# ruubhagat/HP-Assignment-2

Hardware: AMD Instinct MI355X
Metric: simulated coherence transactions/sec (whole node) + % HBM roofline, 1/2/4/8 GPU (higher is better)
Workload: dtype u8

## Files before the change

### hp-assignment-2_amd/csrc/dsm_args.h

```cpp
#ifndef DSM_ARGS_H
#define DSM_ARGS_H

#include <hip/hip_runtime.h>
#include <stdint.h>

#include "dsm.h"

struct SimArgs {
    const uint16_t *traces;
    const uint32_t *counts;
    uint32_t stride;
    uint32_t n_instr;
    uint64_t n_sys;
    const unsigned int *d_n;
    const uint32_t *list;
    uint64_t first_sys;
    uint64_t seed;
    int dist;
    dsm_sys_result *results;
    uint4 *recs;
    unsigned long long *counters;
    unsigned int *claim;
    uint32_t *ovf_list;
    unsigned int *ovf_count;
    const uint2 *table;
    uint64_t sched_seed;
    uint32_t sched_thresh;
    uint32_t issue_cap;
    uint32_t *issue;
    uint32_t *issue_n;
    uint32_t rsh;
    uint32_t budget;
    uint32_t resume;
    uint32_t ffsel;
    const uint32_t *scan;
    uint32_t late_rsh;
    uint32_t *susp;
    uint32_t *susp_list;
    unsigned int *susp_count;
    uint32_t *susp_order;
    unsigned int *susp_multi;
    unsigned int *susp_long;
    unsigned int *susp_short;
    uint32_t susp_cap;
    uint32_t lim_rsh;
    uint32_t icap;
    uint32_t susp_ring;
    uint32_t *spill;
    uint32_t thr_ff;
    uint32_t lone;
    uint32_t lone_min;
    uint32_t serfmt;
    uint32_t split;
};
struct SimArgsPack { SimArgs a[3]; };

enum { K_MSGS = 13, K_INSTRS = 14, K_ROUNDS = 15, K_SYSTEMS = 16, K_STATUS = 17, K_DHASH = 22,
       K_FHASH = 23, K_MAXR = 24, K_OVFRERUN = 25, K_WROUNDS = 26, K_RESUMED = 27,
       K_FFPASS = 28, K_FFITER = 29, K_SCANI = 30, K_SCANR = 31, K_N = 32,
       K_SERMAC = 32 ,
       K_SERIT = 33  ,
       K_SERPROBE = 34  };
static_assert(sizeof(dsm_counters) == DSM_NCOUNTERS * 8 && K_SERMAC < DSM_NCOUNTERS, "dsm_counters slots");

#define CTRL_WORDS 2048
#define CTRL_FAST 0
#define CTRL_FB 256
#define CTRL_OVF 512
#define CTRL_RES 1024
#define CTRL_SUSP 1536
#define CTRL_SUSPL 1568
#define CTRL_SUSPS 1600
#define CTRL_SUSPM 1632
#define CTRL_SCAN 1792

#endif
```

### hp-assignment-2_amd/csrc/dsm_internal.h

```cpp
#ifndef DSM_INTERNAL_H
#define DSM_INTERNAL_H

#include <hip/hip_runtime.h>

#include "dsm.h"
#include "dsm_plan.h"
#include "dsm_args.h"

#define DSM_TIMING_RING 64

struct dsm_ctx {
    int device;
    dsm_config cfg;
    int ring;
    hipStream_t stream;
    int cus;
    unsigned int *d_ctrl;
    SimArgs *d_args;
    uint32_t *d_ovf_list;
    size_t ovf_cap;
    uint32_t *d_susp;
    size_t susp_cap;
    uint32_t *d_susp_list;
    size_t susp_list_cap;
    uint32_t *d_susp_order;
    size_t susp_order_cap;
    uint32_t *d_spill;
    size_t spill_cap;
    uint16_t *d_traces;
    size_t traces_cap;
    uint32_t *d_counts;
    size_t counts_cap;
    dsm_sys_result *d_res;
    size_t res_cap;
    dsm_counters *d_cnt;
    uint2 *d_table;
    uint4 *d_recs;
    size_t recs_cap;
    uint64_t recs_n;
    hipEvent_t tev0[DSM_TIMING_RING], tev1[DSM_TIMING_RING];
    uint64_t runs_timed;
    dsmp::Plan plan;
    hipStream_t last_st;
    int last_verdict;
    uint32_t budget_log2, late_log2, round_limit_log2, inbox_limit;
    uint32_t ff_budget_rounds;
    int ff_mode;
    int serial;
    uint32_t lone_rounds;
    uint32_t lone_min;
    int fmt_tile, parse_bpl;
    uint64_t sched_seed;
    uint32_t sched_thresh;
    uint32_t *d_issue;
    size_t issue_cap_total;
    uint32_t *d_issue_n;
    size_t issue_n_cap;
    uint64_t issue_sys;
    uint4 *d_dump_tpl;
    char *d_text_tmp;
    uint32_t *d_len_tmp;
    char *d_parse_buf;
    size_t parse_cap;
    uint64_t *d_parse_off;
    size_t parse_off_cap;
    uint32_t *d_parse_list;
    size_t parse_list_cap;
    uint32_t *d_ev_scratch;
    size_t ev_scratch_cap;
    unsigned char *d_rb_scratch;
    size_t rb_scratch_cap;
    unsigned long long *d_rb_claim;
    uint64_t rb_in_flight;
};

#define HIPCK(x) do { if ((x) != hipSuccess) return DSM_E_DEVICE; } while (0)

extern "C" int dsm_debug_order_state(dsm_ctx *c, uint32_t *counts, uint32_t *list, uint32_t *order,
                                     uint64_t cap, uint64_t sys, uint32_t *rec, uint32_t rec_cap,
                                     uint32_t *rec_words, int *host_long);

extern "C" int dsm_debug_reach_times(double *ms, uint64_t *chunks);

extern "C" int dsm_debug_dist_edges(int np, const uint16_t *trace, const uint32_t *counts, uint32_t stride,
                                    const dsm_reach_opts *opts, uint32_t *src, uint32_t *dst, uint8_t *pk, uint64_t cap,
                                    uint64_t *n);
extern "C" int dsm_debug_dist_edges_device(dsm_ctx *c, const uint16_t *d_trace, const uint32_t *d_counts,
                                           const dsm_reach_opts *opts, uint32_t *src, uint32_t *dst, uint8_t *pk,
                                           uint64_t cap, uint64_t *n, void *stream);
extern "C" int dsm_debug_dist_times(double *ms);
extern "C" int dsm_debug_fate_times(double *ms, uint64_t *sweeps);

extern "C" int dsm_debug_raudit_times(double *ms, uint64_t *bytes);
extern "C" int dsm_debug_raudit_lane(int np, const uint32_t *state, uint32_t cls, uint32_t *word, uint32_t *set);

extern "C" int dsm_debug_reach_batch_state(dsm_ctx *c, uint64_t *in_flight, uint64_t *scratch_bytes);

extern "C" int dsm_debug_exscan_device(dsm_ctx *c, const uint32_t *d_in, uint64_t n, uint64_t *d_out, void *stream);

void dsm_text_release(dsm_ctx *c);
void dsm_events_release(dsm_ctx *c);
void dsm_reach_batch_release(dsm_ctx *c);

#define DSM_LOCAL __attribute__((visibility("hidden")))
typedef void (*sim_fn)(const SimArgs *);
DSM_LOCAL sim_fn dsm_sim_pick(int np, int ring, bool gen, int mode);
DSM_LOCAL sim_fn dsm_sim_pick_rerun(int np, bool gen, int mode);
DSM_LOCAL int dsm_sim_blocks_per_cu(sim_fn f, int threads);
DSM_LOCAL void dsm_sim_launch(sim_fn f, unsigned grid, unsigned threads, hipStream_t st, const SimArgs *a);
DSM_LOCAL int dsm_sim_lds_bytes(int ring, int waves);
DSM_LOCAL void dsm_order_launch(int np, unsigned blocks, hipStream_t st, const SimArgs *a);
DSM_LOCAL void dsm_ser_launch(int np, bool cap, unsigned blocks, hipStream_t st, const SimArgs *a);
DSM_LOCAL void dsm_args_launch(const SimArgsPack &pk, SimArgs *dst, hipStream_t st);
DSM_LOCAL void dsm_scan_launch(int np, unsigned blocks, hipStream_t st, const uint16_t *traces,
                               const uint32_t *counts, uint32_t stride, uint64_t n_sys, uint32_t *scan,
                               unsigned long long *counters);
DSM_LOCAL void dsm_digest_launch(int np, unsigned blocks, hipStream_t st, uint64_t n_sys, const uint4 *recs,
                                 dsm_sys_result *results, unsigned long long *counters);
#define DSM_EXSCAN_TILE 2048
DSM_LOCAL void dsm_exscan_launch(const uint32_t *in, unsigned long long n, unsigned long long *bsum,
                                 unsigned long long *out, hipStream_t st);

static inline int dsm_recs_range(const dsm_ctx *c, uint32_t need, uint64_t first_sys, uint64_t n_sys) {
    if ((c->cfg.flags & need) != need || !c->d_recs) return DSM_E_STATE;
    if (first_sys > c->recs_n || n_sys > c->recs_n - first_sys) return DSM_E_INVAL;
    return DSM_OK;
}

template <typename T>
static inline int dsm_ensure(T **p, size_t *cap, size_t need) {
    if (*cap >= need && *p) return DSM_OK;
    if (*p) { (void)hipFree(*p); *p = nullptr; *cap = 0; }
    if (hipMalloc((void **)p, need * sizeof(T)) != hipSuccess) { *p = nullptr; return DSM_E_NOMEM; }
    *cap = need;
    return DSM_OK;
}

#endif
```

### hp-assignment-2_amd/csrc/dsm_knobs.h

```cpp
#ifndef DSM_KNOBS_H
#define DSM_KNOBS_H

#ifndef TRAFFIC_PROBE
#define TRAFFIC_PROBE 0
#endif
#ifndef REC_PROBE
#define REC_PROBE 0
#endif
#ifndef SIM_TAILPROBE
#define SIM_TAILPROBE 0
#endif
#ifndef SER_PROBE
#define SER_PROBE 0
#endif

#ifndef FF_LONG_U
#define FF_LONG_U 8
#endif

#ifndef SER_HB
#define SER_HB 8
#endif
#ifndef SER_HT
#define SER_HT 32
#endif
#ifndef SER_SOLO_MIN
#define SER_SOLO_MIN 48
#endif
#ifndef SER_SOLO_HW
#define SER_SOLO_HW 2
#endif
#ifndef SER_DEAD_FWD
#define SER_DEAD_FWD 1
#endif
#ifndef SER_NOTICE_HOME
#define SER_NOTICE_HOME 1
#endif
#ifndef SER_DUMP
#define SER_DUMP 0
#endif

#endif
```

### hp-assignment-2_amd/csrc/dsm_runtime.hip

```cpp
#include <hip/hip_runtime.h>

#include <stdint.h>
#include <stdio.h>
#include <stdlib.h>
#include <string.h>

#include "dsm.h"
#include "dsm_knobs.h"
#include "dsm_table.h"
#include "dsm_internal.h"
#include "dsm_serial.h"

using namespace dsmp;


static uint32_t env_u32(const char *name, uint32_t dflt) {
    const char *e = getenv(name);
    if (!e || !*e) return dflt;
    const long v = strtol(e, nullptr, 10);
    return v < 0 ? 0u : (uint32_t)v;
}

extern "C" int dsm_device_count(int *count) {
    if (!count) return DSM_E_INVAL;
    int c = 0;
    if (hipGetDeviceCount(&c) != hipSuccess) c = 0;
    *count = c;
    return DSM_OK;
}

extern "C" int dsm_open(int device, const dsm_config *cfg, dsm_ctx **out) {
    if (!cfg || !out) return DSM_E_INVAL;
    *out = nullptr;
    if (cfg->np != 4 && cfg->np != 8) return DSM_E_INVAL;
    if (cfg->max_instr == 0 || cfg->max_instr > DSM_MAX_INSTR || (cfg->max_instr & 7u)) return DSM_E_INVAL;
    int ring = cfg->ring_cap ? (int)cfg->ring_cap : 12;
    if (ring != 4 && ring != 8 && ring != 12 && ring != 16) return DSM_E_INVAL;
    int ndev = 0;
    if (hipGetDeviceCount(&ndev) != hipSuccess || device < 0 || device >= ndev) return DSM_E_DEVICE;
    hipDeviceProp_t prop;
    if (hipGetDeviceProperties(&prop, device) != hipSuccess) return DSM_E_DEVICE;
    if (strncmp(prop.gcnArchName, "gfx950", 6) != 0) return DSM_E_DEVICE;
    if (hipSetDevice(device) != hipSuccess) return DSM_E_DEVICE;
    dsm_ctx *c = (dsm_ctx *)calloc(1, sizeof(dsm_ctx));
    if (!c) return DSM_E_NOMEM;
    c->device = device;
    c->cfg = *cfg;
    c->sched_thresh = DSM_SCHED_LOCKSTEP;
    c->ring = ring;
    c->cus = prop.multiProcessorCount;
    c->budget_log2 = env_u32("DSM_BUDGET_LOG2", 12);
    if (c->budget_log2 >= RSH_MAX) c->budget_log2 = 0;
    uint32_t ffb_log2 = env_u32("DSM_FF_BUDGET_LOG2", 0);
    if (ffb_log2 >= RSH_MAX) ffb_log2 = 0;
    c->ff_budget_rounds = getenv("DSM_FF_BUDGET_LOG2") ? (ffb_log2 ? 1u << ffb_log2 : 0u)
                                                       : env_u32("DSM_FF_BUDGET_ROUNDS", 448);
    if (c->ff_budget_rounds >= (1u << RSH_MAX)) c->ff_budget_rounds = 0;
    c->late_log2 = env_u32("DSM_LATE_LOG2", 0);
    c->round_limit_log2 = RSH_MAX;
    c->inbox_limit = FB_RING;
    c->ff_mode = DSM_FF_AUTO;
    c->serial = (int)env_u32("DSM_SERIAL", 1);
    c->lone_rounds = env_u32("DSM_LONE", 8);
    c->lone_min = env_u32("DSM_LONE_MIN", 160);

    c->fmt_tile = (int)env_u32("DSM_FMT", 132);
    c->parse_bpl = (int)env_u32("DSM_PARSE_BPL", 32);
    if (hipStreamCreateWithFlags(&c->stream, hipStreamNonBlocking) != hipSuccess ||
        hipMalloc((void **)&c->d_ctrl, CTRL_WORDS * sizeof(unsigned int)) != hipSuccess ||
        hipMalloc((void **)&c->d_args, sizeof(SimArgsPack)) != hipSuccess ||
        hipMalloc((void **)&c->d_cnt, sizeof(dsm_counters)) != hipSuccess ||
        hipMalloc((void **)&c->d_table, DT_TABLE_WORDS * sizeof(uint32_t)) != hipSuccess) {
        dsm_close(c);
        return DSM_E_DEVICE;
    }
    {
        static uint32_t tab[DT_TABLE_WORDS];
        if (dt_build(tab) > DT_ENTRIES || hipMemcpy(c->d_table, tab, sizeof tab, hipMemcpyHostToDevice) != hipSuccess) {
            dsm_close(c);
            return DSM_E_DEVICE;
        }
    }
    if (cfg->flags & DSM_F_TIMING) {
        for (int i = 0; i < DSM_TIMING_RING; ++i)
            if (hipEventCreate(&c->tev0[i]) != hipSuccess || hipEventCreate(&c->tev1[i]) != hipSuccess) {
                dsm_close(c);
                return DSM_E_DEVICE;
            }
    }
    *out = c;
    return DSM_OK;
}

extern "C" void dsm_close(dsm_ctx *c) {
    if (!c) return;
    (void)hipSetDevice(c->device);
    if (c->stream) (void)hipStreamSynchronize(c->stream);
    void *ptrs[] = {c->d_ctrl, c->d_args, c->d_ovf_list, c->d_susp, c->d_susp_list, c->d_susp_order, c->d_spill,
                    c->d_traces, c->d_counts,
                    c->d_res, c->d_cnt, c->d_recs, c->d_table, c->d_issue, c->d_issue_n};
    for (void *p : ptrs) if (p) (void)hipFree(p);
    dsm_text_release(c);
    dsm_events_release(c);
    dsm_reach_batch_release(c);
    for (int i = 0; i < DSM_TIMING_RING; ++i) {
        if (c->tev0[i]) (void)hipEventDestroy(c->tev0[i]);
        if (c->tev1[i]) (void)hipEventDestroy(c->tev1[i]);
    }
    if (c->stream) (void)hipStreamDestroy(c->stream);
    free(c);
}

extern "C" int dsm_launch_info_get(dsm_ctx *c, dsm_launch_info *info) {
    if (!c || !info) return DSM_E_INVAL;
    if (c->plan.pair && c->last_verdict < 0) {
        uint32_t scan[2] = {0, 0};
        HIPCK(hipSetDevice(c->device));
        HIPCK(hipStreamSynchronize(c->last_st));
        HIPCK(hipMemcpy(scan, c->d_ctrl + CTRL_SCAN, sizeof scan, hipMemcpyDeviceToHost));
        c->last_verdict = ff_verdict(scan) ? 1 : 0;
    }
    *info = plan_info(c->plan, c->last_verdict > 0);
    info->lds_bytes_per_block = c->plan.n_launch ? dsm_sim_lds_bytes(c->plan.ring_eff, SIM_WAVES) : 0;
    info->fmt_tile = c->fmt_tile;
    info->parse_bpl = c->parse_bpl;
    return DSM_OK;
}

static const char *build_variant() {
    static char tag[160];
    if (tag[0]) return tag[1] ? tag + 1 : "";
    int n = snprintf(tag, sizeof tag, "#");
    auto add = [&](const char *name, long v, long def) {
        if (v != def && n < (int)sizeof tag) n += snprintf(tag + n, sizeof tag - n, " %s=%ld", name, v);
    };
    add("REC_PROBE", REC_PROBE, 0);
    add("SIM_TAILPROBE", SIM_TAILPROBE, 0);
    add("TRAFFIC_PROBE", TRAFFIC_PROBE, 0);
    add("SER_PROBE", SER_PROBE, 0);
    add("SER_HB", SER_HB, 8);
    add("SER_HT", SER_HT, 32);
    add("SER_SOLO_MIN", SER_SOLO_MIN, 48);
    add("SER_SOLO_HW", SER_SOLO_HW, 2);
    add("FF_LONG_U", FF_LONG_U, 8);
    add("SER_DEAD_FWD", SER_DEAD_FWD, 1);
    add("SER_NOTICE_HOME", SER_NOTICE_HOME, 1);
    add("SER_DUMP", SER_DUMP, 0);
    return tag[1] ? tag + 1 : "";
}

extern "C" int dsm_launch_kernel_names(const dsm_launch_info *info, char *buf, size_t cap) {
    if (!info || !buf) return DSM_E_INVAL;
    char b[2][96];
    auto sim = [&](char *o, int m) {
        snprintf(o, 96, "sim_kernel<%d, %d, %d, %s, %d, %d>", info->np, info->ring_cap,
                 info->block_threads / 64, info->gen ? "true" : "false", m, info->occ);
    };
    int n;
    if (info->budget_mode < 0) {
        n = snprintf(buf, cap, "none");
    } else if (info->resume_form == DSM_RESUME_NONE) {
        sim(b[0], info->budget_mode);
        n = snprintf(buf, cap, "run=%s", b[0]);
    } else {
        sim(b[0], info->budget_mode);
        if (info->resume_mode >= 0) sim(b[1], info->resume_mode);
        else snprintf(b[1], 96, "ser_kernel<%d, %s>", info->np, info->ser_cap ? "true" : "false");
        n = snprintf(buf, cap, "budget=%s resume=%s", b[0], b[1]);
    }
    const char *v = build_variant();
    if (n >= 0 && *v && (size_t)n < cap) n += snprintf(buf + n, cap - n, " [variant:%s]", v);
    return (n < 0 || (size_t)n >= cap) ? DSM_E_INVAL : n;
}

extern "C" int dsm_set_budget(dsm_ctx *c, uint32_t budget_log2, uint32_t late_log2) {
    if (!c || budget_log2 >= RSH_MAX || late_log2 >= RSH_MAX) return DSM_E_INVAL;
    c->budget_log2 = budget_log2;
    c->late_log2 = late_log2;
    return DSM_OK;
}

extern "C" int dsm_set_round_limit(dsm_ctx *c, uint32_t limit_log2) {
    if (!c || limit_log2 > RSH_MAX) return DSM_E_INVAL;
    c->round_limit_log2 = limit_log2 ? limit_log2 : RSH_MAX;
    if (c->round_limit_log2 < 1) return DSM_E_INVAL;
    return DSM_OK;
}

extern "C" int dsm_set_fast_forward(dsm_ctx *c, int mode) {
    if (!c || mode < DSM_FF_OFF || mode > DSM_FF_AUTO) return DSM_E_INVAL;
    c->ff_mode = mode;
    return DSM_OK;
}

extern "C" int dsm_set_inbox_limit(dsm_ctx *c, uint32_t cap) {
    if (!c || cap > (uint32_t)FB_RING) return DSM_E_INVAL;
    c->inbox_limit = cap ? cap : (uint32_t)FB_RING;
    return DSM_OK;
}

namespace {
struct HostRec {
    const uint32_t *p;
    uint32_t ld(uint32_t w) const { return p[w]; }
};
}
extern "C" int dsm_debug_order_state(dsm_ctx *c, uint32_t *counts, uint32_t *list, uint32_t *order,
                                     uint64_t cap, uint64_t sys, uint32_t *rec, uint32_t rec_cap,
                                     uint32_t *rec_words, int *host_long) {
    if (!c || !counts) return DSM_E_INVAL;
    HIPCK(hipSetDevice(c->device));
    HIPCK(hipStreamSynchronize(c->last_st ? c->last_st : c->stream));
    const Plan &pl = c->plan;
    const uint64_t n = pl.in.n_sys;
    counts[0] = counts[1] = counts[2] = counts[3] = 0;
    if (!n || !pl.blog) return 0;
    HIPCK(hipMemcpy(&counts[0], c->d_ctrl + CTRL_SUSP, sizeof(uint32_t), hipMemcpyDeviceToHost));
    HIPCK(hipMemcpy(&counts[1], c->d_ctrl + CTRL_SUSPL, sizeof(uint32_t), hipMemcpyDeviceToHost));
    HIPCK(hipMemcpy(&counts[2], c->d_ctrl + CTRL_SUSPS, sizeof(uint32_t), hipMemcpyDeviceToHost));
    HIPCK(hipMemcpy(&counts[3], c->d_ctrl + CTRL_SUSPM, sizeof(uint32_t), hipMemcpyDeviceToHost));
    counts[1] += counts[3];
    if ((list && cap < n) || (order && cap < 2 * n)) return DSM_E_INVAL;
    if (list) HIPCK(hipMemcpy(list, c->d_susp_list, n * sizeof(uint32_t), hipMemcpyDeviceToHost));
    if (order && pl.order)
        HIPCK(hipMemcpy(order, c->d_susp_order, pl.order_words * sizeof(uint32_t), hipMemcpyDeviceToHost));
    if (rec_words) *rec_words = pl.rec_words;
    if (rec && pl.rec_words) {
        if (sys >= n || rec_cap < pl.rec_words) return DSM_E_INVAL;
        HIPCK(hipMemcpy(rec, c->d_susp + sys * (uint64_t)pl.rec_words,
                        pl.rec_words * sizeof(uint32_t), hipMemcpyDeviceToHost));
        if (host_long) {
            const HostRec m{rec};
            *host_long = (c->cfg.np == 4 ? dsms::ser_long_class<4>(m, rec[121])
                                         : dsms::ser_long_class<8>(m, rec[121])) ? 1 : 0;
        }
    }
    return pl.order ? 1 : 0;
}

static void put_sched(SimArgs &a, const PlanArgs &s) {
    a.rsh = s.rsh; a.budget = s.budget; a.resume = s.resume; a.ffsel = s.ffsel;
    a.late_rsh = s.late_rsh; a.thr_ff = s.thr_ff; a.lone = s.lone; a.lone_min = s.lone_min;
    a.serfmt = s.serfmt; a.split = s.split; a.susp_ring = s.susp_ring; a.lim_rsh = s.lim_rsh;
    a.icap = s.icap;
}

static int run_engine(dsm_ctx *c, bool gen, const dsm_gen *g, uint64_t first_sys,
                      const uint16_t *d_traces, const uint32_t *d_counts, uint64_t n_sys,
                      dsm_sys_result *d_results, dsm_counters *d_counters, hipStream_t st) {
    if (n_sys > 0xFFFFFFFFull) return DSM_E_INVAL;
    const int np = c->cfg.np;
    const bool tr = (c->cfg.flags & DSM_F_ISSUE_TRACE) != 0;
    PlanIn in{};
    in.np = np; in.ring = c->ring; in.gen = gen; in.n_sys = n_sys; in.cus = c->cus;
    in.tc = (c->cfg.flags & DSM_F_TYPE_COUNTS) != 0; in.tr = tr; in.sx = c->sched_thresh < DSM_SCHED_LOCKSTEP;
    in.round_limit_log2 = c->round_limit_log2; in.inbox_limit = c->inbox_limit;
    in.ff_mode = c->ff_mode; in.serial = c->serial; in.ff_budget_rounds = c->ff_budget_rounds;
    in.budget_log2 = c->budget_log2; in.late_log2 = c->late_log2;
    in.lone_rounds = c->lone_rounds; in.lone_min = c->lone_min;
    in.traffic_probe = TRAFFIC_PROBE;
    Plan p = plan_build(in);
    if (n_sys == 0) {
        c->plan = p;
        return DSM_OK;
    }
    HIPCK(hipSetDevice(c->device));
    sim_fn sim[PLAN_MAX_LAUNCHES] = {}, fast = nullptr;
    for (int i = 0; i < p.n_launch; ++i) {
        if (p.launch[i].kernel != PK_SIM) continue;
        if (!(sim[i] = dsm_sim_pick(np, p.ring_eff, gen, p.launch[i].mode))) return DSM_E_INVAL;
        if (!fast) fast = sim[i];
    }
    const sim_fn fb = dsm_sim_pick_rerun(np, gen, p.mode);
    const int nb_fast = dsm_sim_blocks_per_cu(fast, 64 * SIM_WAVES), nb_fb = dsm_sim_blocks_per_cu(fb, 64);
    if (nb_fast < 1 || nb_fb < 1) return DSM_E_DEVICE;
    plan_grids(p, nb_fast, nb_fb);

    int rc;
    if ((rc = dsm_ensure(&c->d_ovf_list, &c->ovf_cap, (size_t)n_sys))) return rc;
    if (p.blog) {
        if ((rc = dsm_ensure(&c->d_susp, &c->susp_cap, (size_t)n_sys * p.susp_words))) return rc;
        if ((rc = dsm_ensure(&c->d_susp_list, &c->susp_list_cap, (size_t)n_sys))) return rc;
    }
    if (p.order && (rc = dsm_ensure(&c->d_susp_order, &c->susp_order_cap, (size_t)p.order_words))) return rc;
    if ((rc = dsm_ensure(&c->d_recs, &c->recs_cap, (size_t)n_sys * np * 8))) return rc;
    if (p.use_ser && (rc = dsm_ensure(&c->d_spill, &c->spill_cap, (size_t)p.spill_lanes * dsms::S_SPILL))) return rc;
    if (!d_results) {
        if ((rc = dsm_ensure(&c->d_res, &c->res_cap, (size_t)n_sys + 1))) return rc;
        d_results = c->d_res;
    }
    if (tr) {
        const size_t cap = (size_t)np * c->cfg.max_instr;
        if ((rc = dsm_ensure(&c->d_issue, &c->issue_cap_total, (size_t)n_sys * cap))) return rc;
        if ((rc = dsm_ensure(&c->d_issue_n, &c->issue_n_cap, (size_t)n_sys))) return rc;
    }
    if (c->cfg.flags & DSM_F_SNAPSHOTS)
        HIPCK(hipMemsetAsync(c->d_recs, 0, (size_t)n_sys * np * 128, st));
    c->recs_n = n_sys;
    HIPCK(hipMemsetAsync(c->d_ctrl, 0, CTRL_WORDS * sizeof(unsigned int), st));

    SimArgsPack pk;
    memset(&pk, 0, sizeof pk);
    SimArgs &A = pk.a[ARGS_FAST];
    A.traces = d_traces;
    A.counts = d_counts;
    A.stride = c->cfg.max_instr;
    A.n_instr = gen ? g->n_instr : 0;
    A.n_sys = n_sys;
    A.first_sys = first_sys;
    A.seed = gen ? g->seed : 0;
    A.dist = gen ? g->dist : 0;
    A.results = d_results;
    A.recs = c->d_recs;
    A.counters = reinterpret_cast<unsigned long long *>(d_counters);
    A.claim = c->d_ctrl + CTRL_FAST;
    A.ovf_list = c->d_ovf_list;
    A.ovf_count = c->d_ctrl + CTRL_OVF;
    A.table = c->d_table;
    A.sched_seed = c->sched_seed;
    A.sched_thresh = c->sched_thresh;
    A.susp = c->d_susp;
    A.susp_list = c->d_susp_list;
    A.susp_count = c->d_ctrl + CTRL_SUSP;
    A.susp_order = p.order ? c->d_susp_order : nullptr;
    A.susp_multi = c->d_ctrl + CTRL_SUSPM;
    A.susp_long = c->d_ctrl + CTRL_SUSPL;
    A.susp_short = c->d_ctrl + CTRL_SUSPS;
    A.susp_cap = (uint32_t)n_sys;
    A.spill = c->d_spill;
    if (tr) {
        A.issue = c->d_issue;
        A.issue_n = c->d_issue_n;
        A.issue_cap = (uint32_t)((size_t)np * c->cfg.max_instr);
        c->issue_sys = n_sys;
    }
    SimArgs &B = pk.a[ARGS_RERUN];
    B = A;
    B.d_n = c->d_ctrl + CTRL_OVF;
    B.list = c->d_ovf_list;
    B.claim = c->d_ctrl + CTRL_FB;
    B.ovf_list = nullptr;
    B.ovf_count = nullptr;
    SimArgs &C = pk.a[ARGS_RESUME];
    C = A;
    C.n_sys = 0;
    C.d_n = c->d_ctrl + CTRL_SUSP;
    C.list = c->d_susp_list;
    C.claim = c->d_ctrl + CTRL_RES;
    A.scan = C.scan = c->d_ctrl + CTRL_SCAN;
    for (int i = 0; i < 3; ++i) put_sched(pk.a[i], p.args[i]);
    dsm_args_launch(pk, c->d_args, st);
    HIPCK(hipGetLastError());

    const bool timed = (c->cfg.flags & DSM_F_TIMING) != 0;
    const int slot = (int)(c->runs_timed % DSM_TIMING_RING);
    if (timed) HIPCK(hipEventRecord(c->tev0[slot], st));
    unsigned long long *dcnt = reinterpret_cast<unsigned long long *>(d_counters);
    for (int i = 0; i < p.n_launch; ++i) {
        const PlanLaunch &L = p.launch[i];
        const SimArgs *a = (const SimArgs *)(c->d_args + L.args);
        switch (L.kernel) {
        case PK_SCAN:
            dsm_scan_launch(np, p.scan_blocks, st, d_traces, d_counts, (uint32_t)c->cfg.max_instr, n_sys,
                            c->d_ctrl + CTRL_SCAN, dcnt);
            break;
        case PK_SIM:
            dsm_sim_launch(sim[i], p.grid_fast, 64 * SIM_WAVES, st, a);
            break;
        case PK_ORDER:
            dsm_order_launch(np, p.order_blocks, st, a);
            break;
        case PK_SER:
            dsm_ser_launch(np, L.mode != 0, p.ser_blocks, st, a);
            break;
        case PK_RERUN:
            if (timed) {
                HIPCK(hipEventRecord(c->tev1[slot], st));
                c->runs_timed++;
            }
            dsm_sim_launch(fb, p.grid_fb, 64, st, a);
            break;
        case PK_DIGEST:
            if (REC_PROBE) break;
            dsm_digest_launch(np, p.digest_blocks, st, n_sys, (const uint4 *)c->d_recs, d_results, dcnt);
            break;
        }
        HIPCK(hipGetLastError());
    }
    c->plan = p;
    c->last_st = st;
    c->last_verdict = -1;
    return DSM_OK;
}


static int validate_host_traces(const dsm_ctx *c, const uint16_t *traces, const uint32_t *counts,
                                 uint64_t n_sys) {
    const int np = c->cfg.np;
    const uint32_t stride = c->cfg.max_instr;
    for (uint64_t s = 0; s < n_sys; ++s)
        for (int nd = 0; nd < np; ++nd) {
            const uint32_t cnt = counts[s * np + nd];
            if (cnt > stride) return DSM_E_INVAL;
            const uint16_t *t = traces + (s * np + nd) * (uint64_t)stride;
            for (uint32_t i = 0; i < cnt; ++i)
                if ((uint32_t)((t[i] >> 12) & 7u) >= (uint32_t)np) return DSM_E_RANGE;
        }
    return DSM_OK;
}

extern "C" int dsm_run_packed_device(dsm_ctx *c, const uint16_t *d_traces, const uint32_t *d_counts,
                                     uint64_t n_sys, dsm_sys_result *d_results,
                                     dsm_counters *d_counters, void *stream) {
    if (!c || (n_sys && (!d_traces || !d_counts)) || !d_counters) return DSM_E_INVAL;
    return run_engine(c, false, nullptr, 0, d_traces, d_counts, n_sys, d_results, d_counters,
                      (hipStream_t)stream);
}

extern "C" int dsm_run_generated_device(dsm_ctx *c, const dsm_gen *g, uint64_t first_sys,
                                        uint64_t n_sys, dsm_sys_result *d_results,
                                        dsm_counters *d_counters, void *stream) {
    if (!c || !g || !d_counters) return DSM_E_INVAL;
    if (g->n_instr > DSM_MAX_INSTR || g->dist < 0 || g->dist > 2) return DSM_E_INVAL;
    return run_engine(c, true, g, first_sys, nullptr, nullptr, n_sys, d_results, d_counters,
                      (hipStream_t)stream);
}

static int finish_host(dsm_ctx *c, uint64_t n_sys, dsm_sys_result *per_sys, dsm_counters *out) {
    if (per_sys && n_sys)
        HIPCK(hipMemcpyAsync(per_sys, c->d_res, n_sys * sizeof(dsm_sys_result), hipMemcpyDeviceToHost, c->stream));
    if (out) HIPCK(hipMemcpyAsync(out, c->d_cnt, sizeof(dsm_counters), hipMemcpyDeviceToHost, c->stream));
    HIPCK(hipStreamSynchronize(c->stream));
    return DSM_OK;
}

extern "C" int dsm_run_packed(dsm_ctx *c, const uint16_t *traces, const uint32_t *counts,
                              uint64_t n_sys, dsm_sys_result *per_sys, dsm_counters *out) {
    if (!c || (n_sys && (!traces || !counts))) return DSM_E_INVAL;
    int rc = validate_host_traces(c, traces, counts, n_sys);
    if (rc) return rc;
    HIPCK(hipSetDevice(c->device));
    const size_t slots = (size_t)n_sys * c->cfg.np;
    if ((rc = dsm_ensure(&c->d_traces, &c->traces_cap, slots * c->cfg.max_instr + 8))) return rc;
    if ((rc = dsm_ensure(&c->d_counts, &c->counts_cap, slots + 1))) return rc;
    if ((rc = dsm_ensure(&c->d_res, &c->res_cap, (size_t)n_sys + 1))) return rc;
    if (n_sys) {
        HIPCK(hipMemcpyAsync(c->d_traces, traces, slots * c->cfg.max_instr * sizeof(uint16_t), hipMemcpyHostToDevice, c->stream));
        HIPCK(hipMemcpyAsync(c->d_counts, counts, slots * sizeof(uint32_t), hipMemcpyHostToDevice, c->stream));
    }
    HIPCK(hipMemsetAsync(c->d_cnt, 0, sizeof(dsm_counters), c->stream));
    if ((rc = run_engine(c, false, nullptr, 0, c->d_traces, c->d_counts, n_sys, c->d_res, c->d_cnt, c->stream))) return rc;
    return finish_host(c, n_sys, per_sys, out);
}

extern "C" int dsm_run_generated(dsm_ctx *c, const dsm_gen *g, uint64_t first_sys, uint64_t n_sys,
                                 dsm_sys_result *per_sys, dsm_counters *out) {
    if (!c || !g) return DSM_E_INVAL;
    int rc;
    HIPCK(hipSetDevice(c->device));
    if ((rc = dsm_ensure(&c->d_res, &c->res_cap, (size_t)n_sys + 1))) return rc;
    HIPCK(hipMemsetAsync(c->d_cnt, 0, sizeof(dsm_counters), c->stream));
    if ((rc = dsm_run_generated_device(c, g, first_sys, n_sys, c->d_res, c->d_cnt, c->stream))) return rc;
    return finish_host(c, n_sys, per_sys, out);
}

extern "C" int dsm_kernel_ms_history(dsm_ctx *c, float *ms, uint32_t cap, uint32_t *n) {
    if (!c || !n || (cap && !ms)) return DSM_E_INVAL;
    if (!(c->cfg.flags & DSM_F_TIMING)) return DSM_E_STATE;
    HIPCK(hipSetDevice(c->device));
    uint64_t k = c->runs_timed < DSM_TIMING_RING ? c->runs_timed : DSM_TIMING_RING;
    if (k > cap) k = cap;
    for (uint64_t i = 0; i < k; ++i) {
        const int slot = (int)((c->runs_timed - k + i) % DSM_TIMING_RING);
        HIPCK(hipEventSynchronize(c->tev1[slot]));
        HIPCK(hipEventElapsedTime(&ms[i], c->tev0[slot], c->tev1[slot]));
    }
    *n = (uint32_t)k;
    return DSM_OK;
}

extern "C" int dsm_last_kernel_ms(dsm_ctx *c, float *ms) {
    if (!c || !ms) return DSM_E_INVAL;
    if (!(c->cfg.flags & DSM_F_TIMING) || c->runs_timed == 0) return DSM_E_STATE;
    uint32_t n = 0;
    return dsm_kernel_ms_history(c, ms, 1, &n);
}

extern "C" int dsm_get_node_state(dsm_ctx *c, uint64_t sys, int node, dsm_node_state *dump,
                                  dsm_node_state *final_state) {
    if (!c || node < 0 || node >= c->cfg.np) return DSM_E_INVAL;
    if (int rc = dsm_recs_range(c, DSM_F_SNAPSHOTS, sys, 1)) return rc;
    HIPCK(hipSetDevice(c->device));
    HIPCK(hipStreamSynchronize(c->stream));
    HIPCK(hipDeviceSynchronize());
    const size_t i = ((size_t)sys * c->cfg.np + node) * 8;
    if (dump) HIPCK(hipMemcpy(dump, c->d_recs + i, sizeof *dump, hipMemcpyDeviceToHost));
    if (final_state) HIPCK(hipMemcpy(final_state, c->d_recs + i + 4, sizeof *final_state, hipMemcpyDeviceToHost));
    return DSM_OK;
}

extern "C" int dsm_set_schedule(dsm_ctx *c, uint64_t seed, uint32_t act_thresh) {
    if (!c) return DSM_E_INVAL;
    c->sched_seed = seed;
    c->sched_thresh = act_thresh >= DSM_SCHED_LOCKSTEP ? DSM_SCHED_LOCKSTEP : act_thresh;
    return DSM_OK;
}

extern "C" int dsm_get_issue_trace(dsm_ctx *c, uint64_t sys, uint32_t *events, uint32_t cap,
                                   uint32_t *n) {
    if (!c || !n || (cap && !events)) return DSM_E_INVAL;
    if (!(c->cfg.flags & DSM_F_ISSUE_TRACE) || !c->d_issue) return DSM_E_STATE;
    if (sys >= c->issue_sys) return DSM_E_INVAL;
    HIPCK(hipSetDevice(c->device));
    HIPCK(hipStreamSynchronize(c->stream));
    HIPCK(hipDeviceSynchronize());
    uint32_t k = 0;
    HIPCK(hipMemcpy(&k, c->d_issue_n + sys, sizeof k, hipMemcpyDeviceToHost));
    const uint32_t per = (uint32_t)(c->cfg.np * c->cfg.max_instr);
    const uint32_t m = k < cap ? k : cap;
    if (m) HIPCK(hipMemcpy(events, c->d_issue + sys * per, m * sizeof(uint32_t), hipMemcpyDeviceToHost));
    *n = k;
    return DSM_OK;
}
```

### hp-assignment-2_amd/csrc/dsm_ser.hip

```cpp
#include <hip/hip_runtime.h>

#include <stdint.h>

#include "dsm.h"
#include "dsm_knobs.h"
#include "dsm_table.h"
#include "dsm_internal.h"
#include "dsm_device.h"
#include "dsm_serial.h"

namespace {

using namespace dsmp;

constexpr int SER_RF = 8;
constexpr int SER_MACRO = 1;
template <int W>
struct LdsCol {
    uint32_t (&s)[W][dsms::S_WORDS][64];
    uint32_t *dum;
    uint32_t wv, lane;
    GU32 *sp;
    DEVI uint32_t ld(uint32_t w) const { return s[wv][w][lane]; }
    DEVI void st(uint32_t w, uint32_t v) const { s[wv][w][lane] = v; }
    DEVI void st_if(bool en, uint32_t w, uint32_t v) const { *(en ? &s[wv][w][lane] : dum) = v; }
    DEVI uint32_t ld8(uint32_t w, uint32_t b) const {
        return reinterpret_cast<const uint8_t *>(&s[wv][w][lane])[b];
    }
    DEVI void st8(uint32_t w, uint32_t b, uint32_t v) const {
        reinterpret_cast<uint8_t *>(&s[wv][w][lane])[b] = (uint8_t)v;
    }
    DEVI uint32_t ld16(uint32_t w, uint32_t h) const {
        return reinterpret_cast<const uint16_t *>(&s[wv][w][lane])[h];
    }
    DEVI void st16(uint32_t w, uint32_t h, uint32_t v) const {
        reinterpret_cast<uint16_t *>(&s[wv][w][lane])[h] = (uint16_t)v;
    }
    DEVI uint32_t sp_ld(uint32_t i) const { return sp[i]; }
    DEVI void sp_st(uint32_t i, uint32_t v) const { sp[i] = v; }
};
struct LdsTab {
    const uint2 (&t)[DT_TABLE_WORDS / 2];
    DEVI uint32_t hdr(uint32_t i) const { return reinterpret_cast<const uint32_t *>(&t[DT_ENTRIES])[i]; }
    DEVI void row(uint32_t i, uint32_t &w0, uint32_t &w1) const {
        const uint2 e = t[i];
        w0 = e.x;
        w1 = e.y;
    }
};

template <int NP, bool CAP>
__global__ void __launch_bounds__(64 * SER_WAVES) __attribute__((amdgpu_waves_per_eu(2)))
ser_kernel(const SimArgs *Ap) {
    using namespace dsms;
    constexpr uint32_t NPM = (1u << NP) - 1u;
    constexpr bool SOLO = !CAP;
    if (DSM_SER_EXITS(Ap)) return;

    __shared__ uint32_t s_ser[SER_WAVES][S_WORDS][64];
    __shared__ uint2 s_tab[DT_TABLE_WORDS / 2];
    __shared__ unsigned long long s_cnt[K_N];
    __shared__ uint32_t s_dum[64];
    const uint32_t lane = threadIdx.x & 63u, wv = threadIdx.x >> 6;
    if (threadIdx.x < K_N) s_cnt[threadIdx.x] = 0;
    for (uint32_t i = threadIdx.x; i < DT_TABLE_WORDS / 2; i += 64 * SER_WAVES) s_tab[i] = Ap->table[i];
    __syncthreads();
#if SIM_TAILPROBE
    const uint64_t tprobe0 = __builtin_amdgcn_s_memrealtime();
#endif

    const LdsCol<SER_WAVES> m{s_ser, &s_dum[lane], wv, lane,
                              (GU32 *)(Ap->spill + ((uint64_t)blockIdx.x * (64 * SER_WAVES) + threadIdx.x) * S_SPILL)};
    const LdsTab T{s_tab};
    const bool ordered = Ap->serfmt != 0u && Ap->susp_order != nullptr;
    const uint32_t nmulti = ordered ? *Ap->susp_multi : 0u;
    const uint32_t nlong = nmulti + (ordered ? *Ap->susp_long : 0u);
    const uint32_t n = uni32(*Ap->d_n);
    const uint32_t lcap = Ap->susp_cap;
    const uint32_t *const list = ordered ? Ap->susp_order : Ap->list;
    auto sel = [&](uint32_t k) -> uint32_t {
        return ((const GU32 *)list)[k < nmulti ? lcap + k : k < nlong ? lcap - 1u - (k - nmulti) : n - 1u - k];
    };

    const uint32_t stride = Ap->stride, lim_rsh = Ap->lim_rsh, SR = Ap->susp_ring;
    const uint32_t cap = Ap->icap;
    const uint16_t *const traces = Ap->traces;

    uint4 *const recs = Ap->recs;
    dsm_sys_result *const results = Ap->results;
    const uint32_t *const susp = Ap->susp;
    uint32_t *const ovf_list = Ap->ovf_list;
    unsigned int *const ovf_count = Ap->ovf_count, *const claim_ctr = Ap->claim;

    SReg r;
    SCache cc;
    ser_cache_clear(cc);
    uint64_t sys = 0;
    uint32_t tn = 0xFFu, tci = 0, pfc = 0;
    bool nxv = false, pfv = false;
    uint4 cur = make_uint4(0, 0, 0, 0), nx = cur, pf = cur;
    auto slot_of = [&](uint32_t nd) { return traces + (sys * NP + nd) * (uint64_t)stride; };

    auto claim_next = [&]() -> uint32_t {
        return gatomic_add((GU32 *)claim_ctr, 1u);
    };


    auto start_ls = [&]() {
        const GU32 *sp = (const GU32 *)(susp + sys * ((uint64_t)susp_words((int)SR) * NP));
        r.rounds = sp[(12u + SR + 6u) * NP];
        for (uint32_t nd = 0; nd < (uint32_t)NP; ++nd) {
            const GU32 *b = sp + nd;
#pragma unroll
            for (uint32_t i = 0; i < 8; ++i) m.st(S_MB + 8u * nd + i, b[i * NP]);
            uint32_t la = 0, lv = 0, ls = 0;
#pragma unroll
            for (uint32_t i = 0; i < 4; ++i) {
                const uint32_t l = b[(8u + i) * NP];
                la |= (l & 0xFFu) << (8 * i);
                lv |= ((l >> 8) & 0xFFu) << (8 * i);
                ls |= ((l >> 16) & 3u) << (2 * i);
            }
            m.st(S_LA + nd, la);
            m.st(S_LV + nd, lv);
            const GU32 *q = b + (12u + SR) * NP;
            const uint32_t ctl = q[NP], ip = q[2 * NP], rh = q[4 * NP];
            m.st(S_DS + nd, q[0]);
            m.st(S_CT + nd, (ctl & 0x3FFu) | (ls << SC_LS) | (ip << SC_IP));
            s_set_ni(r, nd, q[3 * NP]);
            const uint32_t h = rh & 0xFFu, c = rh >> 8;
            for (uint32_t j = 0; j < c; ++j) {
                uint32_t sl = h + j;
                sl = sl >= SR ? sl - SR : sl;
                ser_enqueue<S_QN>(m, r, nd, b[(12u + sl) * NP]);
            }
            s_byte_add(r.cnt0, r.cnt1, nd, c);
            r.nz |= (c ? 1u : 0u) << nd;
            r.msgs += q[5 * NP] - c;
            r.iss |= ((ctl & (C_WAIT | C_DUMPED)) == 0u ? 1u : 0u) << nd;
            r.dmp |= ((ctl & C_DUMPED) ? 1u : 0u) << nd;
        }
    };
    const bool serfmt = Ap->serfmt != 0u;
    v4u32 rr[33];
    auto load_rec = [&](uint64_t s_) {
        const GV4 *sv = (const GV4 *)(susp + s_ * (uint64_t)ssusp_words((int)SR));
#pragma unroll
        for (uint32_t i = 0; i < 33; ++i) rr[i] = sv[i];
    };
    auto start = [&]() -> uint32_t {
        ser_clear(r);
        tn = 0xFFu;
        nxv = pfv = false;
        if (!serfmt) {
            start_ls();
        } else {
        const GU32 *sp = (const GU32 *)(susp + sys * (uint64_t)ssusp_words((int)SR));
#pragma unroll
        for (uint32_t i = 0; i < 24; ++i) {
            const uint32_t w = 4u * i;
            m.st(w, rr[i].x); m.st(w + 1u, rr[i].y); m.st(w + 2u, rr[i].z); m.st(w + 3u, rr[i].w);
        }
        const v4u32 *const hd = rr + 24;
        r.rounds = hd[6].x;
        auto hw = [&](uint32_t k) -> uint32_t {
            const v4u32 &v = hd[k >> 2];
            return (k & 3u) == 0u ? v.x : (k & 3u) == 1u ? v.y : (k & 3u) == 2u ? v.z : v.w;
        };
#pragma unroll
        for (uint32_t nd = 0; nd < (uint32_t)NP; ++nd) {
            const uint32_t rh = hw(nd), c = rh >> 8, ctl = m.ld(S_CT + nd);
            s_set_ni(r, nd, hw(8u + nd));
            for (uint32_t j = 0; j < c; ++j)
                ser_enqueue<S_QN>(m, r, nd, sp[SSUSP_HDR + nd * SR + j]);
            s_byte_add(r.cnt0, r.cnt1, nd, c);
            r.nz |= (c ? 1u : 0u) << nd;
            r.msgs += hw(16u + nd) - c;
            r.iss |= ((ctl & (SC_WAIT | SC_DUMPED)) == 0u ? 1u : 0u) << nd;
            r.dmp |= ((ctl & SC_DUMPED) ? 1u : 0u) << nd;
        }
        if (hd[6].y & 0x100u) {
            tn = hd[6].y & 0xFFu;
            const uint32_t ip0 = m.ld(S_CT + tn) >> SC_IP, j0 = ip0 & 7u;
            const uint32_t rw[4] = {hd[7].x, hd[7].y, hd[7].z, hd[7].w};
            uint32_t al[4] = {0u, 0u, 0u, 0u};
#pragma unroll
            for (uint32_t k = 0; k < 8u; ++k) {
                uint32_t hv = 0u;
#pragma unroll
                for (uint32_t q = 0; q < 8u; ++q)
                    hv = (k >= j0 && k - j0 == q) ? ((rw[q >> 1] >> (16u * (q & 1u))) & 0xFFFFu) : hv;
                al[k >> 1] |= hv << (16u * (k & 1u));
            }
            cur = make_uint4(al[0], al[1], al[2], al[3]);
            nx = make_uint4(hd[8].x, hd[8].y, hd[8].z, hd[8].w);
            tci = ip0 >> 3;
            nxv = true;
            pfc = tci + 2u;
            pfv = pfc * 8u < stride;
            if (pfv) pf = ld16(slot_of(tn) + pfc * 8u);
        }
        }
        r.E = r.nz;
        r.A = r.nz | r.iss;
        ser_cache_clear(cc);
        if (SOLO && serfmt && tn != 0xFFu) {
            cc.ct = m.ld(S_CT + tn); cc.la = m.ld(S_LA + tn); cc.lv = m.ld(S_LV + tn);
            cc.node = tn;
        }
        if (r.A == 0u) {
            r.st = (r.dmp == NPM) ? SS_COMPLETED : SS_DEADLOCKED;
            return SR_DONE;
        }
        return SR_RUN;
    };
    auto store_rec = [&](uint32_t nd, uint32_t flags, uint32_t which) {
        if (REC_PROBE) return;
        GV4 *dst = (GV4 *)(recs + (sys * NP + nd) * 8 + 4u * which);
#pragma unroll
        for (int q = 0; q < 4; ++q) {
            v4u32 x;
            x.x = ser_rec_word(m, nd, flags, 4 * q);
            x.y = ser_rec_word(m, nd, flags, 4 * q + 1);
            x.z = ser_rec_word(m, nd, flags, 4 * q + 2);
            x.w = ser_rec_word(m, nd, flags, 4 * q + 3);
            dst[q] = x;
        }
    };
    auto fetch = [&](uint32_t nd, uint32_t ip, bool iss) -> uint32_t {
        const uint32_t c = ip >> 3;
        const bool tnd = tn == nd;
        const bool rot = iss & tnd & (tci + 1u == c) & nxv;
        const bool miss = iss & !rot & (!tnd | (tci != c));
        cur.x = rot ? nx.x : cur.x; cur.y = rot ? nx.y : cur.y;
        cur.z = rot ? nx.z : cur.z; cur.w = rot ? nx.w : cur.w;
        nxv = nxv & !rot;
        tci = rot ? c : tci;
        if (__ballot(miss)) {
            if (SER_PROBE && lane == 0) atomicAdd(&s_cnt[3], 1ull);
            if (miss) {
                const uint16_t *sl = slot_of(nd);
                cur = ld16(sl + 8u * c);
                nxv = (c + 1u) * 8u < stride;
                nx = ld16(sl + (nxv ? 8u * (c + 1u) : 8u * c));
                pfv = false;
                tn = nd;
                tci = c;
            }
            wait_vmcnt0();
        }
        const uint32_t j = ip & 7u;
        const uint32_t m2 = 0u - ((j >> 1) & 1u), m4 = 0u - ((j >> 2) & 1u);
        const uint32_t lo = (cur.x & ~m2) | (cur.y & m2), hi = (cur.z & ~m2) | (cur.w & m2);
        const uint32_t wd = (lo & ~m4) | (hi & m4);
        return (wd >> (16u * (j & 1u))) & 0xFFFFu;
    };
    auto fetch_reg = [&](uint32_t nd, uint32_t ip, uint32_t &ins) -> bool {
        const uint32_t c = ip >> 3;
        const bool tnd = tn == nd;
        const bool rot = tnd & (tci + 1u == c) & nxv;
        const bool have = tnd & ((tci == c) | rot);
        cur.x = rot ? nx.x : cur.x; cur.y = rot ? nx.y : cur.y;
        cur.z = rot ? nx.z : cur.z; cur.w = rot ? nx.w : cur.w;
        nxv = nxv & !rot;
        tci = rot ? c : tci;
        const uint32_t j = ip & 7u;
        const uint32_t m2 = 0u - ((j >> 1) & 1u), m4 = 0u - ((j >> 2) & 1u);
        const uint32_t lo = (cur.x & ~m2) | (cur.y & m2), hi = (cur.z & ~m2) | (cur.w & m2);
        const uint32_t wd = (lo & ~m4) | (hi & m4);
        ins = (wd >> (16u * (j & 1u))) & 0xFFFFu;
        return have;
    };
    bool live = false;
    uint32_t v = SR_RUN;
    auto refill = [&]() {
        if (pfv && !nxv && pfc == tci + 1u) {
            nx = pf;
            nxv = true;
            pfv = false;
        }
        if (pfv && (pfc <= tci || pfc > tci + 2u)) pfv = false;
        const uint32_t want = nxv ? tci + 2u : tci + 1u;
        if (tn != 0xFFu && !pfv && want * 8u < stride && v == SR_RUN) {
            pf = ld16(slot_of(tn) + want * 8u);
            pfc = want;
            pfv = true;
        }
    };
    auto on_dump = [&](uint32_t nd) { store_rec(nd, 2u, 0u); };
    auto finish = [&](uint32_t v) {
        if (v == SR_OVF) {
            const uint32_t pos = gatomic_add((GU32 *)ovf_count, 1u);
            ((GU32 *)ovf_list)[pos] = (uint32_t)sys;
            atomicAdd(&s_cnt[K_OVFRERUN], 1ull);
            return;
        }
        uint32_t ins = 0;
#pragma unroll
        for (uint32_t nd = 0; nd < (uint32_t)NP; ++nd) {
            ins += m.ld(S_CT + nd) >> SC_IP;
            store_rec(nd, ser_final_flags(m, nd), 1u);
        }
        v4u32 res;
        res.x = r.st | (r.dmp << 8); res.y = r.rounds; res.z = r.msgs; res.w = ins;
        ((GV4 *)results)[2 * sys] = res;
        atomicAdd(&s_cnt[K_MSGS], (unsigned long long)r.msgs);
        atomicAdd(&s_cnt[K_INSTRS], (unsigned long long)ins);
        atomicAdd(&s_cnt[K_ROUNDS], (unsigned long long)r.rounds);
        atomicAdd(&s_cnt[K_SYSTEMS], 1ull);
        atomicAdd(&s_cnt[K_STATUS + r.st], 1ull);
        atomicMax(&s_cnt[K_MAXR], (unsigned long long)r.rounds);
    };

    {
        const uint32_t k = claim_next();
        live = k < n;
        if (live) sys = sel(k);
        if (live && serfmt) load_rec(sys);
    }
    v = live ? start() : SR_RUN;
    uint32_t iters = 0, nmac = 0;
    uint32_t tclaim = 0, now_it = 0;
    bool lone0 = false;
    [[maybe_unused]] uint64_t pr_long = 0, pr_last = 0, pr_n4k = 0, pr_nl_it = 0, pr_it = 0, pr_nl_n = 0;
    if constexpr (SIM_TAILPROBE == 2) lone0 = live && serfmt && (rr[30].y & 0x100u);
    uint32_t hwait = 0;
    uint64_t pb_runs = 0, pb_steps = 0, pb_idle = 0, pb_cyc = 0;
    for (;;) {
        bool taken = false, rest = false;
#pragma unroll 1
        for (int k = 0; k < SER_RF; ++k) {
            bool ran_now = false, gen = true;
            if (SOLO) {
                if (k == 0) {
                    uint64_t ts0 = 0;
                    if (SER_PROBE >= 2) ts0 = __builtin_amdgcn_s_memtime();
                    const bool run = live && v == SR_RUN;
                    const bool ql = run && ser_quiet_lone(r, lim_rsh);
                    const uint32_t sn = ql ? dsms::s_ctz(r.A) : 0xFEu;
                    const uint32_t c = cc.ct >> (SC_IP + 3u);
                    const bool hotq = ql & (cc.node == sn) & (tn == sn);
                    const bool rot = hotq & (tci + 1u == c) & nxv;
                    cur.x = rot ? nx.x : cur.x; cur.y = rot ? nx.y : cur.y;
                    cur.z = rot ? nx.z : cur.z; cur.w = rot ? nx.w : cur.w;
                    nxv = nxv & !rot;
                    tci = rot ? c : tci;
                    const bool elig = hotq & (tci == c);
                    const uint32_t ne = (uint32_t)__builtin_popcountll(__ballot(elig));
                    const uint32_t nr = (uint32_t)__builtin_popcountll(__ballot(run));
                    if (ne != 0u && ne * 64u >= nr * (uint32_t)SER_SOLO_MIN) {
                        uint32_t ns = 0;
                        if (elig) ns = ser_solo<NP>(m, r, cc, cur.x, cur.y, cur.z, cur.w, lim_rsh);
                        nmac += ns;
                        taken = ran_now = true;
                        rest = elig & (ns != 0u) & (((cc.ct >> SC_IP) & 7u) == 0u);
                        iters += 1u;
                        if (SER_PROBE) {
                            uint32_t t = ns;
                            for (int o = 1; o < 64; o <<= 1) t += __shfl_xor(t, o, 64);
                            pb_runs += 1u; pb_steps += t; pb_idle += 8u * nr - t;
                            if (SER_PROBE >= 2) pb_cyc += __builtin_amdgcn_s_memtime() - ts0;
                        }
                    }
                }
                if (taken) {
                    gen = __ballot(live && v == SR_RUN && !rest) != 0ull;
                    if (!gen && !ran_now) break;
                }
                iters += gen ? 1u : 0u;
            }
            bool mac = false;
            uint64_t tp0 = 0, tp1 = 0, tp2 = 0;
            if (SER_PROBE >= 2) tp0 = __builtin_amdgcn_s_memtime();
            if (!CAP && gen) {
#pragma unroll
                for (int j = 0; j < SER_MACRO; ++j) {
                    const bool q = live && v == SR_RUN && !rest && ser_quiet_lone(r, lim_rsh) && (j == 0 || mac);
                    bool did = false;
                    bool nohave = false;
                    if (SER_PROBE && q) {
                        const uint32_t n0 = dsms::s_ctz(r.A), ip0 = m.ld(S_CT + n0) >> SC_IP, c0 = ip0 >> 3;
                        nohave = !((tn == n0) & ((tci == c0) | ((tci + 1u == c0) & nxv)));
                    }
                    if (SER_PROBE >= 4) {
                        uint64_t ts[5] = {0, 0, 0, 0, 0};
                        auto stamp = [&](int i) { __builtin_amdgcn_s_waitcnt(0); ts[i + 1] = __builtin_amdgcn_s_memtime(); };
                        __builtin_amdgcn_s_waitcnt(0);
                        ts[0] = __builtin_amdgcn_s_memtime();
                        if (__ballot(q) && q) did = ser_macro<NP>(m, r, cc, fetch_reg, on_dump, stamp);
                        const uint64_t okb = __ballot(did);
                        if (okb && lane == (uint32_t)__builtin_ctzll(okb)) {
                            atomicAdd(&s_cnt[13], ts[1] - ts[0]);
                            atomicAdd(&s_cnt[14], ts[2] - ts[1]);
                            atomicAdd(&s_cnt[15], ts[3] - ts[2]);
                            atomicAdd(&s_cnt[16], ts[4] - ts[3]);
                        }
                    } else if (__ballot(q) && q) {
                        did = ser_macro<NP>(m, r, cc, fetch_reg, on_dump, [](int) {});
                    }
                    if (SER_PROBE && j == 0) {
                        const uint64_t nh = __ballot(nohave);
                        if (lane == 0) atomicAdd(&s_cnt[8 + 3], 0ull + __builtin_popcountll(nh));
                    }
                    if (SER_PROBE && j == 0) {
                        const bool nq_ = live && v == SR_RUN && !q;
                        const uint64_t nq = __ballot(nq_), qn = __ballot(q && !did);
                        const uint64_t mi = __ballot(nq_ && (r.iss & (r.iss - 1u)) != 0u);
                        if (lane == 0) {
                            atomicAdd(&s_cnt[9], (unsigned long long)__builtin_popcountll(nq));
                            atomicAdd(&s_cnt[10], (unsigned long long)__builtin_popcountll(qn));
                            (void)mi;
                        }
                    }
                    mac = mac || did;
                    nmac += did ? 1u : 0u;
                }
                if (mac && r.A == 0u) v = SR_DONE;
                if (SOLO) rest = rest | (taken & mac);
            }
            if (SER_PROBE) {
                const uint64_t gm = __ballot(live && v == SR_RUN && !mac), mm = __ballot(mac);
                const uint64_t lv = __ballot(live);
                if (lane == 0) {
                    atomicAdd(&s_cnt[8], (unsigned long long)__builtin_popcountll(lv));
                    if (__builtin_popcountll(lv) < 32) atomicAdd(&s_cnt[12], 1ull);
                    atomicAdd(&s_cnt[0], 1ull);
                    if (mm) atomicAdd(&s_cnt[1], 1ull);
                    if (gm) atomicAdd(&s_cnt[2], 1ull);
                }
            }
            if (SER_PROBE >= 2) tp1 = __builtin_amdgcn_s_memtime();
            if (live && v == SR_RUN && !mac && gen && !rest) {
                v = ser_step<NP, S_QN, CAP>(m, r, T, fetch, on_dump, lim_rsh, cap);
                ser_cache_clear(cc);
            }
            if (SER_PROBE >= 2) tp2 = __builtin_amdgcn_s_memtime();
            if (SER_PROBE) {
                const uint64_t hm = __ballot(live && v != SR_RUN);
                if (lane == 0 && hm) atomicAdd(&s_cnt[4], 1ull);
            }
            bool hgo = false;
            const uint64_t fin = __ballot(live && v != SR_RUN);
            if (fin) {
                hgo = (uint32_t)__builtin_popcountll(fin) >= (uint32_t)SER_HB ||
                      hwait >= (uint32_t)SER_HT || fin == __ballot(live);
                hwait = hgo ? 0u : hwait + (gen ? 1u : 0u) + (ran_now ? (uint32_t)SER_SOLO_HW : 0u);
            }
            if (hgo && live && v != SR_RUN) {
                if constexpr (SIM_TAILPROBE == 2) now_it = iters + (uint32_t)k;
                uint64_t th0 = 0, th1 = 0, th2 = 0;
                if (SER_PROBE >= 3) th0 = __builtin_amdgcn_s_memtime();
                wait_vmcnt0();
                const uint32_t k = claim_next();
                const bool nl = k < n;
                const uint32_t ns = nl ? sel(k) : 0u;
                if (nl && serfmt) load_rec(ns);
                if (SER_PROBE >= 3) { __builtin_amdgcn_s_waitcnt(0); th1 = __builtin_amdgcn_s_memtime(); }
                if constexpr (SIM_TAILPROBE == 2) {
                    const uint64_t dur = (uint64_t)(now_it - tclaim);
                    const uint64_t a = (dur << 32) | (uint64_t)sys;
                    const uint64_t b = ((uint64_t)now_it << 32) | ((uint64_t)lone0 << 31) | dur;
                    pr_long = a > pr_long ? a : pr_long;
                    pr_last = b > pr_last ? b : pr_last;
                    pr_n4k += dur > 4000u ? 1u : 0u;
                    pr_nl_it += lone0 ? 0u : dur;
                    pr_it += dur;
                    pr_nl_n += lone0 ? 0u : 1u;
                    tclaim = now_it;
                    lone0 = nl && serfmt && (rr[30].y & 0x100u);
                }
                finish(v);
                if (SER_PROBE >= 3) { __builtin_amdgcn_s_waitcnt(0); th2 = __builtin_amdgcn_s_memtime(); }
                live = nl;
                sys = ns;
                rest = false;
                v = live ? start() : SR_RUN;
                if (SER_PROBE >= 3) {
                    __builtin_amdgcn_s_waitcnt(0);
                    const uint64_t th3 = __builtin_amdgcn_s_memtime();
                    const uint64_t fl = __ballot(true);
                    if (lane == (uint32_t)__builtin_ctzll(fl)) {
                        atomicAdd(&s_cnt[13], th1 - th0);
                        atomicAdd(&s_cnt[14], th2 - th1);
                        atomicAdd(&s_cnt[15], th3 - th2);
                    }
                }
            }
            if (SER_PROBE >= 2 && lane == 0) {
                const uint64_t tp3 = __builtin_amdgcn_s_memtime();
                atomicAdd(&s_cnt[5], tp1 - tp0);
                atomicAdd(&s_cnt[6], tp2 - tp1);
                atomicAdd(&s_cnt[7], tp3 - tp2);
            }
            if (!gen) break;
        }
        uint64_t tr0 = 0;
        if (SER_PROBE >= 2) tr0 = __builtin_amdgcn_s_memtime();
        refill();
        (void)tr0;
        if (!SOLO) iters += SER_RF;
        if (__ballot(live) == 0) break;
    }
#if SIM_TAILPROBE == 2
    {
        uint64_t v6[6] = {pr_long, pr_last, pr_n4k, pr_nl_it, pr_it, pr_nl_n};
#pragma unroll
        for (int q = 0; q < 6; ++q) {
            uint64_t x = v6[q];
            for (int o = 1; o < 64; o <<= 1) {
                const uint32_t lo = __shfl_xor((uint32_t)x, o, 64), hi = __shfl_xor((uint32_t)(x >> 32), o, 64);
                const uint64_t y = ((uint64_t)hi << 32) | lo;
                x = q < 2 ? (y > x ? y : x) : x + y;
            }
            if (lane == 0) {
                if (q < 2) atomicMax(&Ap->counters[q], (unsigned long long)x);
                else atomicAdd(&Ap->counters[q], (unsigned long long)x);
            }
        }
    }
#endif
    if (lane == 0) {
        atomicAdd(&s_cnt[K_WROUNDS], (unsigned long long)iters);
        atomicAdd(&Ap->counters[K_SERIT], (unsigned long long)iters);
        if (SER_PROBE && SOLO && !SIM_TAILPROBE) {
            atomicAdd(&Ap->counters[K_SERPROBE], (unsigned long long)pb_runs);
            atomicAdd(&Ap->counters[K_SERPROBE + 1], (unsigned long long)pb_steps);
            atomicAdd(&Ap->counters[K_SERPROBE + 2], (unsigned long long)pb_idle);
            atomicAdd(&Ap->counters[K_SERPROBE + 3], (unsigned long long)pb_cyc);
        }
#if SIM_TAILPROBE
        const uint64_t ms = (__builtin_amdgcn_s_memrealtime() - tprobe0) / 100000u;
        atomicAdd(&Ap->counters[K_SERPROBE + (ms < 11u ? 0u : (ms - 10u < 5u ? ms - 10u : 5u))], 1ull);
#endif
    }
    if (!CAP) {
        uint32_t t = nmac;
        for (int o = 1; o < 64; o <<= 1) t += __shfl_xor(t, o, 64);
        if (lane == 0 && t) atomicAdd(&Ap->counters[K_SERMAC], (unsigned long long)t);
    }
    __syncthreads();
    if (threadIdx.x < K_N) {
        const unsigned long long x = s_cnt[threadIdx.x];
        if (x) {
            if (threadIdx.x == K_MAXR) atomicMax(&Ap->counters[K_MAXR], x);
            else atomicAdd(&Ap->counters[threadIdx.x], x);
        }
    }
}

struct RecCol {
    const GU32 *sp;
    DEVI uint32_t ld(uint32_t w) const { return sp[w]; }
};
template <int NP>
__global__ void __launch_bounds__(ORD_THREADS) order_kernel(const SimArgs *Ap) {
    constexpr uint32_t SPB = ORD_THREADS / NP, NW = ORD_THREADS / 64;
    constexpr uint64_t NPM = (1ull << NP) - 1ull;
    if (DSM_SER_EXITS(Ap)) return;
    const uint32_t n = *Ap->d_n, first = blockIdx.x * SPB;
    if (first >= n) return;
    __shared__ uint32_t s_nm[NW], s_nl[NW], s_ns[NW], s_base[3];
    const uint32_t lane = threadIdx.x & 63u, wv = threadIdx.x >> 6;
    const uint32_t h = lane & (uint32_t)(NP - 1), gbase = lane & ~(uint32_t)(NP - 1);
    const uint32_t k = first + threadIdx.x / NP;
    const bool have = k < n;
    uint32_t sys = 0;
    bool lone = false, stale = false;
    if (have) {
        sys = ((const GU32 *)Ap->list)[k];
        const RecCol m{(const GU32 *)(Ap->susp + sys * (uint64_t)ssusp_words((int)Ap->susp_ring))};
        const uint32_t hd = m.sp[121];
        lone = (hd & 0x100u) != 0u;
        stale = dsms::ser_stale_home(m, h, hd & 7u);
    }
    const bool gstale = ((__ballot(stale) >> gbase) & NPM) != 0ull;
    const bool lead = have && h == 0u;
    const uint32_t cls = !lone ? 0u : (gstale ? 2u : 1u);
    const uint64_t mb = __ballot(lead && cls == 0u), lb = __ballot(lead && cls == 1u), sb = __ballot(lead && cls == 2u);
    if (lane == 0) {
        s_nm[wv] = (uint32_t)__builtin_popcountll(mb);
        s_nl[wv] = (uint32_t)__builtin_popcountll(lb);
        s_ns[wv] = (uint32_t)__builtin_popcountll(sb);
    }
    __syncthreads();
    if (threadIdx.x == 0) {
        uint32_t nm = 0, nl = 0, ns = 0;
        for (uint32_t w = 0; w < NW; ++w) { nm += s_nm[w]; nl += s_nl[w]; ns += s_ns[w]; }
        s_base[0] = nm ? atomicAdd(Ap->susp_multi, nm) : 0u;
        s_base[1] = nl ? atomicAdd(Ap->susp_long, nl) : 0u;
        s_base[2] = ns ? atomicAdd(Ap->susp_short, ns) : 0u;
    }
    __syncthreads();
    if (lead) {
        const uint64_t below = (1ull << lane) - 1ull;
        const uint32_t *const cw = cls == 0u ? s_nm : (cls == 1u ? s_nl : s_ns);
        uint32_t r = s_base[cls] + (uint32_t)__builtin_popcountll((cls == 0u ? mb : (cls == 1u ? lb : sb)) & below);
        for (uint32_t w = 0; w < wv; ++w) r += cw[w];
        const uint32_t cap = Ap->susp_cap;
        Ap->susp_order[cls == 0u ? cap + r : (cls == 1u ? cap - 1u - r : r)] = sys;
    }
}

}

void dsm_order_launch(int np, unsigned blocks, hipStream_t st, const SimArgs *a) {
    hipLaunchKernelGGL(np == 4 ? order_kernel<4> : order_kernel<8>, dim3(blocks), dim3(ORD_THREADS), 0, st, a);
}
void dsm_ser_launch(int np, bool cap, unsigned blocks, hipStream_t st, const SimArgs *a) {
    hipLaunchKernelGGL(np == 4 ? (cap ? ser_kernel<4, true> : ser_kernel<4, false>)
                               : (cap ? ser_kernel<8, true> : ser_kernel<8, false>),
                       dim3(blocks), dim3(64 * SER_WAVES), 0, st, a);
}
```

### hp-assignment-2_amd/pydsm.py

```python
import ctypes
import os

import numpy as np

HERE = os.path.dirname(os.path.abspath(__file__))
LIB_PATH = os.environ.get("DSM_LIB") or os.path.join(HERE, "libdsm.so")
CLI_PATH = os.path.join(HERE, "cache_simulator")

NTYPES = 13
TYPE_NAMES = ["READ_REQUEST", "WRITE_REQUEST", "REPLY_RD", "REPLY_WR", "REPLY_ID", "INV",
              "UPGRADE", "WRITEBACK_INV", "WRITEBACK_INT", "FLUSH", "FLUSH_INVACK",
              "EVICT_SHARED", "EVICT_MODIFIED"]
STATUS_NAMES = ["COMPLETED", "DEADLOCKED", "RING_OVERFLOW", "ASSERT_FAILED", "ROUND_LIMIT"]
DIST = {"uniform": 0, "hot": 1, "evict": 2}
FF_OFF, FF_ON, FF_AUTO = 0, 1, 2
F_SNAPSHOTS = 1
F_TIMING = 2
F_TYPE_COUNTS = 4
F_ISSUE_TRACE = 8
SCHED_LOCKSTEP = 0x10000

RESULT_DTYPE = np.dtype([("status", "<u4"), ("rounds", "<u4"), ("msgs", "<u4"),
                         ("instrs", "<u4"), ("dump_hash", "<u8"), ("final_hash", "<u8")])
COUNTER_FIELDS = ([f"msgs_{t}" for t in TYPE_NAMES] +
                  ["msgs", "instrs", "rounds", "systems"] +
                  [f"status_{s}" for s in STATUS_NAMES] +
                  ["sum_dump_hash", "sum_final_hash", "max_rounds", "overflow_reruns",
                   "wave_rounds", "resumed", "ff_passes", "ff_steps", "ff_sample_instrs",
                   "ff_sample_runs", "ser_macro_steps", "ser_iterations"] +
                  [f"reserved_{i}" for i in range(6)])
NCOUNTERS = 40
assert len(COUNTER_FIELDS) == NCOUNTERS
MAX_SLOT = COUNTER_FIELDS.index("max_rounds")

DUMP_BASE, DUMP_MAX, DUMP_SLOT = 1954, 1958, 1968
DUMP_ABSENT = 1
VIEW_DUMP, VIEW_FINAL = 0, 1
E_INVAL, E_DEVICE, E_NOMEM, E_IO, E_FORMAT, E_STATE, E_RANGE = -1, -2, -3, -4, -5, -6, -7


class DsmError(RuntimeError):
    def __init__(self, code, what):
        self.code = code
        super().__init__(f"{what}: {strerror(code)} ({code})")


class Config(ctypes.Structure):
    _fields_ = [("np", ctypes.c_int), ("max_instr", ctypes.c_uint32),
                ("ring_cap", ctypes.c_uint32), ("flags", ctypes.c_uint32)]


class Gen(ctypes.Structure):
    _fields_ = [("seed", ctypes.c_uint64), ("dist", ctypes.c_int), ("n_instr", ctypes.c_uint32)]


class LaunchInfo(ctypes.Structure):
    _fields_ = [("grid_blocks", ctypes.c_int), ("block_threads", ctypes.c_int),
                ("waves_per_cu", ctypes.c_int), ("cus", ctypes.c_int),
                ("ring_cap", ctypes.c_int), ("lds_bytes_per_block", ctypes.c_int),
                ("resume_blocks", ctypes.c_int), ("budget_log2", ctypes.c_int),
                ("late_log2", ctypes.c_int), ("round_limit_log2", ctypes.c_int),
                ("fmt_tile", ctypes.c_int), ("parse_bpl", ctypes.c_int),
                ("resume_form", ctypes.c_int), ("budget_rounds", ctypes.c_int),
                ("ff_picked", ctypes.c_int), ("np", ctypes.c_int), ("gen", ctypes.c_int),
                ("occ", ctypes.c_int), ("budget_mode", ctypes.c_int),
                ("resume_mode", ctypes.c_int), ("ser_cap", ctypes.c_int)]


class EventOpts(ctypes.Structure):
    _fields_ = [("sched_seed", ctypes.c_uint64), ("sched_thresh", ctypes.c_uint32),
                ("round_limit_log2", ctypes.c_uint32), ("inbox_limit", ctypes.c_uint32)]


class ReachOpts(ctypes.Structure):
    _fields_ = [("inbox_limit", ctypes.c_uint32), ("kind", ctypes.c_uint32),
                ("max_states", ctypes.c_uint64), ("max_depth", ctypes.c_uint32),
                ("chunk", ctypes.c_uint32)]


class FateOpts(ctypes.Structure):
    _fields_ = [("status_mask", ctypes.c_uint32), ("max_sweeps", ctypes.c_uint32), ("key", ctypes.c_uint64)]


RESUME_FORMS = {0: "none", 1: "lock-step", 2: "serial", 3: "fast-forward lock-step"}


_lib = None


def lib():
    global _lib
    if _lib is None:
        if not os.path.exists(LIB_PATH):
            raise OSError(f"{LIB_PATH} not built (run `make -C hp-assignment-2_amd`)")
        try:
            import torch
        except ImportError:
            pass
        L = ctypes.CDLL(LIB_PATH)
        vp, u64, u32, i32 = ctypes.c_void_p, ctypes.c_uint64, ctypes.c_uint32, ctypes.c_int
        sig = {
            "dsm_abi_version": (i32, []),
            "dsm_strerror": (ctypes.c_char_p, [i32]),
            "dsm_device_count": (i32, [ctypes.POINTER(i32)]),
            "dsm_open": (i32, [i32, ctypes.POINTER(Config), ctypes.POINTER(vp)]),
            "dsm_close": (None, [vp]),
            "dsm_launch_info_get": (i32, [vp, ctypes.POINTER(LaunchInfo)]),
            "dsm_launch_kernel_names": (i32, [ctypes.POINTER(LaunchInfo), ctypes.c_char_p,
                                              ctypes.c_size_t]),
            "dsm_run_packed": (i32, [vp, vp, vp, u64, vp, vp]),
            "dsm_run_packed_device": (i32, [vp, vp, vp, u64, vp, vp, vp]),
            "dsm_generate_device": (i32, [vp, ctypes.POINTER(Gen), u64, u64, vp, vp, vp]),
            "dsm_run_generated_device": (i32, [vp, ctypes.POINTER(Gen), u64, u64, vp, vp, vp]),
            "dsm_run_generated": (i32, [vp, ctypes.POINTER(Gen), u64, u64, vp, vp]),
            "dsm_get_node_state": (i32, [vp, u64, i32, vp, vp]),
            "dsm_last_kernel_ms": (i32, [vp, ctypes.POINTER(ctypes.c_float)]),
            "dsm_kernel_ms_history": (i32, [vp, vp, u32, ctypes.POINTER(u32)]),
            "dsm_set_budget": (i32, [vp, u32, u32]),
            "dsm_set_round_limit": (i32, [vp, u32]),
            "dsm_set_inbox_limit": (i32, [vp, u32]),
            "dsm_set_fast_forward": (i32, [vp, i32]),
            "dsm_parse_trace_file": (i32, [ctypes.c_char_p, vp, u32, ctypes.POINTER(u32)]),
            "dsm_load_test_dir": (i32, [ctypes.c_char_p, i32, u32, vp, u32, vp]),
            "dsm_format_dump": (i32, [i32, vp, ctypes.c_char_p, ctypes.c_size_t]),
            "dsm_write_dump": (i32, [i32, vp, ctypes.c_char_p]),
            "dsm_node_hash": (u64, [i32, vp, i32]),
            "dsm_format_dumps_device": (i32, [vp, vp, u32, u64, vp, vp, vp]),
            "dsm_format_run_dumps_device": (i32, [vp, i32, u64, u64, vp, vp, vp]),
            "dsm_write_run_dumps": (i32, [vp, u64, u32, ctypes.c_char_p]),
            "dsm_set_schedule": (i32, [vp, u64, u32]),
            "dsm_get_issue_trace": (i32, [vp, u64, vp, u32, ctypes.POINTER(u32)]),
            "dsm_format_issue_trace": (i32, [vp, u32, ctypes.c_char_p, ctypes.c_size_t]),
            "dsm_parse_traces_device": (i32, [vp, vp, vp, u64, u32, vp, vp, vp, vp]),
            "dsm_parse_traces": (i32, [vp, vp, vp, u64, u32, vp, vp, vp]),
            "dsm_generate_text_device": (i32, [vp, ctypes.POINTER(Gen), u64, u64, vp, vp, vp]),
            "dsm_aggregate_device": (i32, [vp, vp, u64, u64, vp, vp]),
            "dsm_aggregate_results": (i32, [vp, u64, u64, vp]),
            "dsm_result_digest": (u64, [u64, vp]),
            "dsm_group_unique_id": (i32, [vp]),
            "dsm_group_init_rank": (i32, [i32, i32, i32, vp, ctypes.POINTER(vp)]),
            "dsm_group_init_all": (i32, [i32, vp, vp]),
            "dsm_group_info": (i32, [vp, ctypes.POINTER(i32), ctypes.POINTER(i32), ctypes.POINTER(i32)]),
            "dsm_group_close": (i32, [vp]),
            "dsm_group_allreduce": (i32, [vp, vp, ctypes.c_size_t, i32, vp]),
            "dsm_group_allreduce_counters": (i32, [vp, vp, vp]),
            "dsm_group_allreduce_aggregate": (i32, [vp, vp, vp]),
            "dsm_group_barrier": (i32, [vp, vp]),
            "dsm_outcome_key": (u64, [i32, vp]),
            "dsm_census_device": (i32, [vp, vp, u64, u64, i32, vp, u32, vp]),
            "dsm_census_run_nodes_device": (i32, [vp, u64, u64, vp, u32, vp]),
            "dsm_census_results": (i32, [vp, u64, u64, i32, vp, u32]),
            "dsm_census_merge": (i32, [vp, vp, u32]),
            "dsm_census_sorted": (i32, [vp, u32, vp, u64, ctypes.POINTER(u64)]),
            "dsm_audit_states_device": (i32, [vp, vp, u32, u64, u64, vp, vp, vp]),
            "dsm_audit_run_device": (i32, [vp, u64, u64, vp, vp, vp]),
            "dsm_audit_states": (i32, [i32, vp, u32, u64, u64, vp, vp]),
            "dsm_audit_merge": (i32, [vp, vp]),
            "dsm_audit_class_name": (ctypes.c_char_p, [i32]),
            "dsm_parse_dump": (i32, [vp, ctypes.c_size_t, ctypes.POINTER(i32), vp]),
            "dsm_read_dump": (i32, [i32, ctypes.c_char_p, vp]),
            "dsm_census_find": (i32, [vp, u32, u64, vp]),
            "dsm_parse_dumps_device": (i32, [vp, vp, vp, u64, vp, u32, vp, vp]),
            "dsm_trace_events_device": (i32, [vp, vp, vp, u64, vp, u64, vp, u32, vp, vp, vp, vp]),
            "dsm_trace_events": (i32, [i32, vp, vp, u32, u64, vp, u64, ctypes.POINTER(EventOpts), vp, u32,
                                       vp, vp, vp]),
            "dsm_event_trace_hash": (u64, [vp, u64]),
            "dsm_format_event_trace": (i32, [vp, u64, i32, ctypes.c_char_p, ctypes.c_size_t]),
            "dsm_reach": (i32, [i32, vp, vp, u32, ctypes.POINTER(ReachOpts), vp, vp, vp, vp, vp, vp, u64]),
            "dsm_reach_device": (i32, [vp, vp, vp, ctypes.POINTER(ReachOpts), vp, vp, vp, vp, vp, vp, u64, vp]),
            "dsm_reach_batch_slab_bytes": (u64, [i32, ctypes.POINTER(ReachOpts)]),
            "dsm_reach_batch": (i32, [i32, vp, vp, u32, u64, ctypes.POINTER(ReachOpts), vp, vp, u64, vp, vp]),
            "dsm_reach_batch_device": (i32, [vp, vp, vp, u64, ctypes.POINTER(ReachOpts), u64, vp, vp, u64, vp, vp, vp]),
            "dsm_debug_reach_batch_state": (i32, [vp, ctypes.POINTER(u64), ctypes.POINTER(u64)]),
            "dsm_reach_path": (i32, [vp, vp, u64, vp, u64, ctypes.POINTER(u64)]),
            "dsm_reach_replay": (i32, [i32, vp, vp, u32, u32, vp, u64, vp, vp, vp]),
            "dsm_census_insert": (i32, [vp, u32, u64, u64]),
            "dsm_sched_prob": (u64, [u32, u32, u32]),
            "dsm_reach_dist": (i32, [i32, vp, vp, u32, ctypes.POINTER(ReachOpts), vp, u32, u32, vp, vp, vp, vp, u64, vp]),
            "dsm_reach_dist_device": (i32, [vp, vp, vp, ctypes.POINTER(ReachOpts), vp, u32, u32, vp, vp, vp, vp, u64,
                                            vp, vp]),
            "dsm_reach_fate": (i32, [i32, vp, vp, u32, ctypes.POINTER(ReachOpts), ctypes.POINTER(FateOpts), vp, u32,
                                     vp, vp, vp, vp, vp, vp, vp, u64, vp, vp, vp]),
            "dsm_reach_fate_device": (i32, [vp, vp, vp, ctypes.POINTER(ReachOpts), ctypes.POINTER(FateOpts), vp, u32,
                                            vp, vp, vp, vp, vp, vp, vp, u64, vp, vp, vp, vp]),
            "dsm_fate_seal_point": (i32, [vp, vp, u64, ctypes.POINTER(u64), ctypes.POINTER(u64)]),
            "dsm_reach_audit": (i32, [i32, vp, vp, u32, ctypes.POINTER(ReachOpts), vp, vp, vp, vp, vp, vp, u64, vp, vp,
                                      vp]),
            "dsm_reach_audit_device": (i32, [vp, vp, vp, ctypes.POINTER(ReachOpts), vp, vp, vp, vp, vp, vp, u64, vp, vp,
                                             vp, vp]),
            "dsm_debug_raudit_times": (i32, [vp, ctypes.POINTER(u64)]),
            "dsm_debug_raudit_lane": (i32, [i32, vp, u32, ctypes.POINTER(u32), ctypes.POINTER(u32)]),
            "dsm_debug_fate_times": (i32, [vp, vp]),
            "dsm_debug_dist_edges": (i32, [i32, vp, vp, u32, ctypes.POINTER(ReachOpts), vp, vp, vp, u64,
                                           ctypes.POINTER(u64)]),
            "dsm_debug_dist_edges_device": (i32, [vp, vp, vp, ctypes.POINTER(ReachOpts), vp, vp, vp, u64,
                                                  ctypes.POINTER(u64), vp]),
            "dsm_debug_dist_times": (i32, [vp]),
            "dsm_debug_reach_times": (i32, [vp, ctypes.POINTER(u64)]),
            "dsm_debug_exscan_device": (i32, [vp, vp, u64, vp, vp]),
            "dsm_debug_order_state": (i32, [vp, vp, vp, vp, u64, u64, vp, u32, ctypes.POINTER(u32),
                                            ctypes.POINTER(i32)]),
        }
        for name, (res, args) in sig.items():
            if os.environ.get("DSM_LIB") and not hasattr(L, name):
                continue
            f = getattr(L, name)
            f.restype, f.argtypes = res, args
        _lib = L
    return _lib


def strerror(code):
    try:
        return lib().dsm_strerror(code).decode()
    except OSError:
        return "libdsm.so unavailable"


def _check(rc, what):
    if rc != 0:
        raise DsmError(rc, what)


def _ptr(a):
    return ctypes.c_void_p(a.ctypes.data) if a is not None else None


COUNTERS_BYTES = NCOUNTERS * 8
NAGG = 16
AGG_FIELDS = ("systems", "msgs", "instrs", "rounds", "max_rounds", "st0", "st1", "st2", "st3",
              "st4", "sum_dump_hash", "sum_final_hash", "result_digest", "reserved0",
              "reserved1", "reserved2")
assert len(AGG_FIELDS) == NAGG
RED_SUM, RED_MAX = 0, 1


def _dptr(x, min_bytes=0):
    if x is None:
        return None
    if hasattr(x, "data_ptr"):
        nb = x.numel() * x.element_size()
        if nb < min_bytes:
            raise DsmError(-1, f"device buffer of {nb} bytes, needs {min_bytes}")
        return ctypes.c_void_p(x.data_ptr())
    return ctypes.c_void_p(x)


def agg_vec_to_dict(v):
    v = [int(x) for x in np.asarray(v, dtype=np.uint64).reshape(-1)]
    a = dict(zip(AGG_FIELDS, v))
    out = {k: a[k] for k in ("systems", "msgs", "instrs", "rounds", "max_rounds")}
    out["status"] = [a[f"st{i}"] for i in range(5)]
    out.update({k: "0x%016x" % a[k] for k in ("sum_dump_hash", "sum_final_hash", "result_digest")})
    return out


def aggregate_results_c(res, first_idx=0):
    res = np.ascontiguousarray(res).view(RESULT_DTYPE).reshape(-1)
    out = np.zeros(NAGG, dtype=np.uint64)
    _check(lib().dsm_aggregate_results(_ptr(res), len(res), first_idx, _ptr(out)),
           "dsm_aggregate_results")
    return agg_vec_to_dict(out)


CENSUS_DUMPS, CENSUS_FINAL, CENSUS_FULL = 0, 1, 2
CENSUS_KINDS = {"dumps": CENSUS_DUMPS, "final": CENSUS_FINAL, "full": CENSUS_FULL}
CENSUS_MIN_CAP, CENSUS_MAX_CAP = 16, 1 << 20
OUTCOME_MISSING = 1
OUTCOME_DTYPE = np.dtype([("key", "<u8"), ("count", "<u8"), ("first_sys", "<u8")])


def _census_cap_ok(cap):
    return CENSUS_MIN_CAP <= cap <= CENSUS_MAX_CAP and cap & (cap - 1) == 0


def CENSUS_WORDS(cap):
    return 4 + 4 * cap


def outcome_key(kind, res):
    rec = np.ascontiguousarray(res).view(RESULT_DTYPE).reshape(-1)[:1].copy()
    return int(lib().dsm_outcome_key(CENSUS_KINDS.get(kind, kind), _ptr(rec)))


def census_results(res, kind=CENSUS_DUMPS, cap=256, first_sys=0):
    res = np.ascontiguousarray(res).view(RESULT_DTYPE).reshape(-1)
    out = np.zeros(CENSUS_WORDS(cap) if _census_cap_ok(cap) else 4, dtype=np.uint64)
    _check(lib().dsm_census_results(_ptr(res), len(res), first_sys, CENSUS_KINDS.get(kind, kind),
                                    _ptr(out), cap), "dsm_census_results")
    return out


def census_merge(dst, src, cap):
    assert dst.dtype == np.uint64 and dst.flags.c_contiguous and dst.size >= 4
    src = np.ascontiguousarray(src, dtype=np.uint64)
    if _census_cap_ok(cap):
        assert dst.size == src.size == CENSUS_WORDS(cap)
    _check(lib().dsm_census_merge(_ptr(dst), _ptr(src), cap), "dsm_census_merge")
    return dst


def census_header(census):
    c = np.asarray(census, dtype=np.uint64).reshape(-1)
    return {"systems": int(c[0]), "distinct": int(c[1]), "dropped": int(c[2])}


def census_sorted(census, cap):
    census = np.ascontiguousarray(census, dtype=np.uint64).reshape(-1)
    if _census_cap_ok(cap):
        assert census.size == CENSUS_WORDS(cap)
    n = ctypes.c_uint64(0)
    _check(lib().dsm_census_sorted(_ptr(census), cap, None, 0, ctypes.byref(n)), "dsm_census_sorted")
    out = np.zeros(n.value, dtype=OUTCOME_DTYPE)
    _check(lib().dsm_census_sorted(_ptr(census), cap, _ptr(out), n.value, ctypes.byref(n)),
           "dsm_census_sorted")
    return out


def census_find(census, cap, key):
    census = np.ascontiguousarray(census, dtype=np.uint64).reshape(-1)
    if _census_cap_ok(cap):
        assert census.size == CENSUS_WORDS(cap)
    out = np.zeros(1, dtype=OUTCOME_DTYPE)
    rc = lib().dsm_census_find(_ptr(census), cap, key, _ptr(out))
    if rc < 0:
        raise DsmError(rc, "dsm_census_find")
    return (int(out[0]["count"]), int(out[0]["first_sys"])) if rc else None


(AUDIT_MULTI_OWNER, AUDIT_OWNER_AND_SHARER, AUDIT_DIR_EM, AUDIT_DIR_S, AUDIT_DIR_U,
 AUDIT_STALE_VALUE, AUDIT_BAD_RECORD) = range(7)
AUDIT_NCLASS = 7
AUDIT_CLASS_NAMES = ["MULTI_OWNER", "OWNER_AND_SHARER", "DIR_EM", "DIR_S", "DIR_U", "STALE_VALUE",
                     "BAD_RECORD"]
AUDIT_COHERENT = 0x00FF0000
NAUDIT = 32
AUDIT_DTYPE = np.dtype([("systems", "<u8"), ("violating", "<u8"), ("lines", "<u8"),
                        ("bad_items", "<u8"), ("by_class", "<u8", (8,)), ("inv_first", "<u8", (8,)),
                        ("reserved", "<u8", (12,))])
assert AUDIT_DTYPE.itemsize == 8 * NAUDIT


def audit_class_name(bit):
    s = lib().dsm_audit_class_name(bit)
    return s.decode() if s is not None else None


def audit_word_fields(word):
    w = int(word)
    return w & 0xFF, (w >> 8) & 0xFF, (w >> 16) & 0xFF, w >> 24


def audit_states(np_, states, state_stride=1, first_sys=0, n_sys=None, words=True, summary=True):
    st = np.ascontiguousarray(states).view(np.uint8).reshape(-1)
    if n_sys is None:
        n_sys = st.size // (64 * np_ * state_stride) if np_ > 0 and state_stride > 0 else 0
    w = np.zeros(n_sys, dtype=np.uint32) if words else None
    a = np.zeros(1, dtype=AUDIT_DTYPE) if summary else None
    _check(lib().dsm_audit_states(np_, _ptr(st) if st.size else None, state_stride, n_sys, first_sys,
                                  _ptr(w), _ptr(a)), "dsm_audit_states")
    return w, (a[0] if summary else None)


def audit_merge(dst, src):
    assert dst.dtype == AUDIT_DTYPE and dst.size == 1 and dst.flags.c_contiguous
    src = np.ascontiguousarray(src, dtype=AUDIT_DTYPE).reshape(1)
    _check(lib().dsm_audit_merge(_ptr(dst), _ptr(src)), "dsm_audit_merge")
    return dst


def audit_to_dict(a):
    v = [int(x) for x in np.ascontiguousarray(a).view(np.uint64).reshape(-1)]
    assert len(v) == NAUDIT
    inv = lambda x: (~x) & 0xFFFFFFFFFFFFFFFF
    return {"systems": v[0], "violating": v[1], "lines": v[2], "bad_items": v[3],
            "first": inv(v[19]) if v[19] else None,
            "classes": {AUDIT_CLASS_NAMES[b]: (v[4 + b], inv(v[12 + b]))
                        for b in range(AUDIT_NCLASS) if v[4 + b]}}


EV_RECV, EV_SEND, EV_ISSUE, EV_ACCESS, EV_REPLACE, EV_FINISHED = range(6)
EV_KIND_NAMES = ["RECV", "SEND", "ISSUE", "ACCESS", "REPLACE", "FINISHED"]
EV_FMT_INSTR, EV_FMT_MSG = 1, 2
EV_FMT_ALL = EV_FMT_INSTR | EV_FMT_MSG
EV_FMT = {"instr": EV_FMT_INSTR, "msg": EV_FMT_MSG, "all": EV_FMT_ALL}
EVENTS_MAX_LANES = 65536


def event_fields(events):
    e = np.asarray(events, dtype=np.uint64)
    f = lambda lo, w: ((e >> np.uint64(lo)) & np.uint64((1 << w) - 1)).astype(np.int64)
    return {"addr": f(0, 8), "value": f(8, 8), "type": f(16, 4), "node": f(20, 3), "peer": f(23, 3),
            "aux": f(26, 3), "kind": f(29, 3), "round": f(32, 23), "flag": f(55, 1)}


def trace_events(np_, traces, counts, ids=None, cap=0, sched=(0, SCHED_LOCKSTEP), round_limit_log2=0,
                 inbox_limit=0):
    traces = np.ascontiguousarray(traces, dtype=np.uint16)
    counts = np.ascontiguousarray(counts, dtype=np.uint32)
    n_sys, _, stride = traces.shape
    assert traces.shape[1] == np_ and counts.shape == (n_sys, np_)
    if ids is not None:
        ids = np.ascontiguousarray(ids, dtype=np.uint64)
    n = n_sys if ids is None else len(ids)
    ev = np.zeros((n, cap), dtype=np.uint64) if cap else None
    cnt = np.zeros(n, dtype=np.uint32)
    hs = np.zeros(n, dtype=np.uint64)
    res = np.zeros(n, dtype=RESULT_DTYPE)
    opts = EventOpts(sched[0], sched[1], round_limit_log2, inbox_limit)
    _check(lib().dsm_trace_events(np_, _ptr(traces), _ptr(counts), stride, n_sys, _ptr(ids), n,
                                  ctypes.byref(opts), _ptr(ev), cap, _ptr(cnt), _ptr(hs), _ptr(res)),
           "dsm_trace_events")
    return ev, cnt, hs, res


def event_trace_hash(events):
    events = np.ascontiguousarray(events, dtype=np.uint64).reshape(-1)
    return int(lib().dsm_event_trace_hash(_ptr(events) if events.size else None, events.size))


def format_event_trace_rc(events, what=EV_FMT_ALL, cap=None):
    events = np.ascontiguousarray(events, dtype=np.uint64).reshape(-1)
    if cap is None:
        cap = 160 * max(events.size, 1) + 1
    buf = ctypes.create_string_buffer(max(cap, 1))
    n = lib().dsm_format_event_trace(_ptr(events) if events.size else None, events.size,
                                     EV_FMT.get(what, what), buf, cap)
    return n, (buf.raw[:n] if n >= 0 else b"")


def format_event_trace(events, what=EV_FMT_ALL):
    n, text = format_event_trace_rc(events, what)
    if n < 0:
        raise DsmError(n, "dsm_format_event_trace")
    return text


REACH_F_STATES, REACH_F_DEPTH, REACH_F_COLLISION = 1, 2, 4
REACH_MAX_LEVELS = 4096
REACH_INFO_FIELDS = ("states", "transitions", "terminals", "levels", "max_frontier", "max_fill",
                     "st0", "st1", "st2", "st3", "st4", "fp_collisions", "flags", "reserved")
REACH_TERMINAL_DTYPE = np.dtype([("state", "<u8"), ("status", "<u4"), ("rounds", "<u4"), ("msgs", "<u4"),
                                 ("instrs", "<u4"), ("dump_hash", "<u8"), ("final_hash", "<u8")])
assert REACH_TERMINAL_DTYPE.itemsize == 40


def reach_info_to_dict(v):
    a = dict(zip(REACH_INFO_FIELDS, (int(x) for x in v)))
    out = {k: a[k] for k in REACH_INFO_FIELDS if not k.startswith("st") or k == "states"}
    out["by_status"] = [a[f"st{i}"] for i in range(5)]
    return out


def reach_census(terminals, kind=CENSUS_DUMPS, cap=None):
    terminals = np.ascontiguousarray(terminals).view(REACH_TERMINAL_DTYPE).reshape(-1)
    if cap is None:
        cap = min(CENSUS_MAX_CAP, max(CENSUS_MIN_CAP, 1 << (2 * max(len(terminals), 1) - 1).bit_length()))
    table = np.zeros(CENSUS_WORDS(cap), dtype=np.uint64)
    res = np.zeros(1, dtype=RESULT_DTYPE)
    for t in terminals:
        for f in RESULT_DTYPE.names:
            res[0][f] = t[f]
        key = int(lib().dsm_outcome_key(CENSUS_KINDS.get(kind, kind), _ptr(res)))
        _check(lib().dsm_census_insert(_ptr(table), cap, key, int(t["state"])), "dsm_census_insert")
    return table, cap


def _reach_result(info, parents, masks, fps, level_off, terms, kind):
    d = reach_info_to_dict(info)
    n, nt = d["states"], min(d["terminals"], len(terms))
    table, cap = reach_census(terms[:nt], kind)
    return {"info": d, "parents": parents[:n], "masks": masks[:n], "fps": fps[:n],
            "level_off": level_off[:d["levels"] + 1], "terminals": terms[:nt], "census": table,
            "census_cap": cap, "outcomes": census_sorted(table, cap)}


def reach(np_, traces, counts, inbox_limit=16, kind=CENSUS_DUMPS, max_states=1 << 22, max_depth=0, term_cap=None):
    traces = np.ascontiguousarray(traces, dtype=np.uint16)
    counts = np.ascontiguousarray(counts, dtype=np.uint32).reshape(-1)
    assert traces.ndim == 2 and traces.shape[0] == np_ and counts.shape == (np_,)
    kind = CENSUS_KINDS.get(kind, kind)
    opts = ReachOpts(inbox_limit, kind, max_states, max_depth, 0)
    ok = 0 < max_states <= 1 << 31
    n = max_states if ok else 1
    term_cap = min(n, 1 << 20) if term_cap is None else term_cap
    info = np.zeros(len(REACH_INFO_FIELDS), dtype=np.uint64)
    parents, masks, fps = np.zeros(n, np.uint32), np.zeros(n, np.uint8), np.zeros(n, np.uint64)
    level_off = np.zeros(REACH_MAX_LEVELS + 1, dtype=np.uint64)
    terms = np.zeros(max(term_cap, 1), dtype=REACH_TERMINAL_DTYPE)
    _check(lib().dsm_reach(np_, _ptr(traces), _ptr(counts), traces.shape[1], ctypes.byref(opts), _ptr(info),
                           _ptr(parents), _ptr(masks), _ptr(fps), _ptr(level_off), _ptr(terms), term_cap),
           "dsm_reach")
    return _reach_result(info, parents, masks, fps, level_off, terms, kind)


REACH_BATCH_MAX_STATES = 1 << 20
REACH_BATCH_MAX_CHUNK = 1 << 16
REACH_INFO_DTYPE = np.dtype([("states", "<u8"), ("transitions", "<u8"), ("terminals", "<u8"), ("levels", "<u8"),
                             ("max_frontier", "<u8"), ("max_fill", "<u8"), ("by_status", "<u8", (5,)),
                             ("fp_collisions", "<u8"), ("flags", "<u8"), ("reserved", "<u8")])
assert REACH_INFO_DTYPE.itemsize == 8 * len(REACH_INFO_FIELDS)


def reach_batch_slab_bytes(np_, inbox_limit=16, kind=CENSUS_DUMPS, max_states=1 << 16, max_depth=0, chunk=0):
    opts = ReachOpts(inbox_limit, CENSUS_KINDS.get(kind, kind), max_states, max_depth, chunk)
    return int(lib().dsm_reach_batch_slab_bytes(np_, ctypes.byref(opts)))


def _reach_many_result(info, terms, term_cap, parents, masks, max_states):
    n = len(info)
    terms = terms[:n * term_cap].reshape(n, term_cap)
    out = {"info": info,
           "terminals": [terms[s, :min(term_cap, int(info["terminals"][s]))] for s in range(n)],
           "can_deadlock": info["by_status"][:, 1] > 0 if n else np.zeros(0, bool),
           "exhaustive": (info["flags"] & (REACH_F_STATES | REACH_F_DEPTH)) == 0}
    if parents is not None:
        out["parents"] = [parents[s * max_states: s * max_states + int(info["states"][s])] for s in range(n)]
        out["masks"] = [masks[s * max_states: s * max_states + int(info["states"][s])] for s in range(n)]
    return out


def reach_many(np_, traces, counts, inbox_limit=16, kind=CENSUS_DUMPS, max_states=1 << 16, max_depth=0, term_cap=None,
               witnesses=False):
    traces = np.ascontiguousarray(traces, dtype=np.uint16)
    counts = np.ascontiguousarray(counts, dtype=np.uint32)
    assert traces.ndim == 3 and traces.shape[1] == np_ and counts.shape == traces.shape[:2]
    n = traces.shape[0]
    opts = ReachOpts(inbox_limit, CENSUS_KINDS.get(kind, kind), max_states, max_depth, 0)
    ok = 0 < max_states <= REACH_BATCH_MAX_STATES
    cap = max_states if ok else 1
    term_cap = min(cap, 4096) if term_cap is None else term_cap
    info = np.zeros(n, dtype=REACH_INFO_DTYPE)
    terms = np.zeros(max(n * term_cap, 1), dtype=REACH_TERMINAL_DTYPE)
    parents = np.zeros(max(n * cap, 1), np.uint32) if witnesses else None
    masks = np.zeros(max(n * cap, 1), np.uint8) if witnesses else None
    _check(lib().dsm_reach_batch(np_, _ptr(traces), _ptr(counts), traces.shape[2], n, ctypes.byref(opts), _ptr(info),
                                 _ptr(terms), term_cap, _ptr(parents), _ptr(masks)), "dsm_reach_batch")
    return _reach_many_result(info, terms[:n * term_cap], term_cap, parents, masks, cap)


def reach_path(parents, masks, state):
    parents = np.ascontiguousarray(parents, dtype=np.uint32)
    masks = np.ascontiguousarray(masks, dtype=np.uint8)
    if not 0 <= state < len(parents):
        raise DsmError(E_INVAL, "reach_path: state")
    out = np.zeros(REACH_MAX_LEVELS, dtype=np.uint8)
    n = ctypes.c_uint64(0)
    _check(lib().dsm_reach_path(_ptr(parents), _ptr(masks), state, _ptr(out), len(out), ctypes.byref(n)),
           "dsm_reach_path")
    return out[:n.value].copy()


def reach_replay(np_, traces, counts, masks, inbox_limit=16):
    traces = np.ascontiguousarray(traces, dtype=np.uint16)
    counts = np.ascontiguousarray(counts, dtype=np.uint32).reshape(-1)
    masks = np.ascontiguousarray(masks, dtype=np.uint8).reshape(-1)
    assert traces.ndim == 2 and traces.shape[0] == np_ and counts.shape == (np_,)
    dump, fin = np.zeros((np_, 64), np.uint8), np.zeros((np_, 64), np.uint8)
    res = np.zeros(1, dtype=RESULT_DTYPE)
    _check(lib().dsm_reach_replay(np_, _ptr(traces), _ptr(counts), traces.shape[1], inbox_limit,
                                  _ptr(masks) if masks.size else None, masks.size, _ptr(dump), _ptr(fin), _ptr(res)),
           "dsm_reach_replay")
    return dump, fin, res[0]


DIST_ONE = 1 << 63
DIST_MAX_THRESH, DIST_MAX_ROUNDS = 16, 65536
DIST_F_RESIDUAL, DIST_F_ESCAPED, DIST_F_INEXACT = 1, 2, 4
DIST_INFO_FIELDS = ("thresh", "rounds", "absorbed", "escaped", "residual", "lost", "st0", "st1", "st2", "st3",
                    "st4", "edges", "missing_edges", "flags", "reserved0", "reserved1")


def sched_prob(thresh, k, m):
    if not all(0 <= x < 1 << 32 for x in (thresh, k, m)):
        return 0
    return int(lib().dsm_sched_prob(thresh, k, m))


def dist_info_to_dict(v):
    a = dict(zip(DIST_INFO_FIELDS, (int(x) for x in v)))
    out = {k: a[k] for k in DIST_INFO_FIELDS if not (k.startswith("st") or k.startswith("reserved"))}
    out["by_status"] = [a[f"st{i}"] for i in range(5)]
    out["reserved"] = [a["reserved0"], a["reserved1"]]
    return out


def _dist_rounds(max_rounds):
    return max_rounds if 0 < max_rounds <= DIST_MAX_ROUNDS else 4096


def _dist_result(r, kind, dinfo, term_mass, round_mass):
    terms = r["terminals"]
    res = np.zeros(1, dtype=RESULT_DTYPE)
    keys = []
    for t in terms:
        for f in RESULT_DTYPE.names:
            res[0][f] = t[f]
        keys.append(int(lib().dsm_outcome_key(kind, _ptr(res))))
    r["dist"] = []
    for j in range(len(dinfo)):
        d = dist_info_to_dict(dinfo[j])
        tm = term_mass[j, :len(terms)].copy()
        by_key = {}
        for k, v in zip(keys, tm):
            by_key[k] = by_key.get(k, 0) + int(v)
        d["term_mass"] = tm
        d["round_mass"] = round_mass[j, :d["rounds"] + 1].copy()
        d["outcomes"] = [{"key": int(o["key"]), "count": int(o["count"]), "first_sys": int(o["first_sys"]),
                          "mass": by_key.get(int(o["key"]), 0), "p": by_key.get(int(o["key"]), 0) / DIST_ONE}
                         for o in r["outcomes"]]
        r["dist"].append(d)
    return r


def reach_dist(np_, traces, counts, thresh=(0x8000,), max_rounds=0, inbox_limit=16, kind=CENSUS_DUMPS,
               max_states=1 << 22, max_depth=0, term_cap=None):
    traces = np.ascontiguousarray(traces, dtype=np.uint16)
    counts = np.ascontiguousarray(counts, dtype=np.uint32).reshape(-1)
    assert traces.ndim == 2 and traces.shape[0] == np_ and counts.shape == (np_,)
    kind = CENSUS_KINDS.get(kind, kind)
    th = np.ascontiguousarray(thresh, dtype=np.uint32).reshape(-1)
    opts = ReachOpts(inbox_limit, kind, max_states, max_depth, 0)
    n = max_states if 0 < max_states <= 1 << 31 else 1
    term_cap = min(n, 1 << 20) if term_cap is None else term_cap
    R = _dist_rounds(max_rounds)
    info = np.zeros(len(REACH_INFO_FIELDS), dtype=np.uint64)
    dinfo = np.zeros((max(len(th), 1), len(DIST_INFO_FIELDS)), dtype=np.uint64)
    terms = np.zeros(max(term_cap, 1), dtype=REACH_TERMINAL_DTYPE)
    term_mass = np.zeros((max(len(th), 1), max(term_cap, 1)), dtype=np.uint64)
    round_mass = np.zeros((max(len(th), 1), R + 1), dtype=np.uint64)
    _check(lib().dsm_reach_dist(np_, _ptr(traces), _ptr(counts), traces.shape[1], ctypes.byref(opts), _ptr(th), len(th),
                                max_rounds, _ptr(info), _ptr(dinfo), _ptr(terms), _ptr(term_mass), max(term_cap, 1),
                                _ptr(round_mass)), "dsm_reach_dist")
    return _dist_result(_reach_terminals_result(info, terms, kind), kind, dinfo, term_mass, round_mass)


FATE_CAN_TARGET, FATE_CAN_OTHER = 1, 2
FATE_NONE, FATE_DOOMED, FATE_SAFE, FATE_OPEN = 0, 1, 2, 3
FATE_CLASS_NAMES = ["NONE", "DOOMED", "SAFE", "OPEN"]
FATE_F_TRUNCATED, FATE_F_INEXACT, FATE_F_UNCONVERGED = 1, 2, 4
FATE_STATUS_ALL = 0x1F
FATE_NO_EDGE = (1 << 64) - 1
FATE_INFO_FIELDS = ("targets", "cls0", "cls1", "cls2", "cls3", "seal_edges", "avert_edges",
                    "seal_src", "seal_rank", "seal_mask", "seal_dst", "avert_src", "avert_rank", "avert_mask",
                    "avert_dst", "edges", "missing_edges", "sweeps", "flags", "reserved0", "reserved1")
FATE_VALUE_FIELDS = ("thresh", "root_lo", "root_hi", "max_slack", "sweeps", "flags", "reserved0", "reserved1")


def fate_info_to_dict(v):
    a = dict(zip(FATE_INFO_FIELDS, (int(x) for x in v)))
    out = {k: a[k] for k in ("targets", "seal_edges", "avert_edges", "edges", "missing_edges", "sweeps", "flags")}
    out["by_class"] = [a[f"cls{i}"] for i in range(4)]
    for kind in ("seal", "avert"):
        out[f"first_{kind}"] = {f: a[f"{kind}_{f}"] for f in ("src", "rank", "mask", "dst")}
    out["reserved"] = [a["reserved0"], a["reserved1"]]
    return out


def fate_value_to_dict(v):
    a = dict(zip(FATE_VALUE_FIELDS, (int(x) for x in v)))
    a["reserved"] = [a.pop("reserved0"), a.pop("reserved1")]
    return a


def fate_target(target):
    if isinstance(target, str):
        return 1 << [n.lower() for n in STATUS_NAMES].index(target.lower()), 0
    if isinstance(target, int):
        return target, 0
    if len(target) and target[0] == "key":
        return (target[2] if len(target) > 2 else FATE_STATUS_ALL), int(target[1])
    m = 0
    for t in target:
        m |= fate_target(t)[0]
    return m, 0


def _fate_result(info, finfo, values, parents, masks, level_off, terms, kind, cls, lo, hi, nth):
    d = reach_info_to_dict(info)
    n, nt = d["states"], min(d["terminals"], len(terms))
    return {"info": d, "fate": fate_info_to_dict(finfo), "values": [fate_value_to_dict(values[j]) for j in range(nth)],
            "parents": parents[:n], "masks": masks[:n], "level_off": level_off[:d["levels"] + 1], "terminals": terms[:nt],
            "cls": cls[:n], "lo": lo[:nth, :n], "hi": hi[:nth, :n]}


def reach_fate(np_, traces, counts, target="deadlocked", thresh=(0x8000,), max_sweeps=0, inbox_limit=16,
               kind=CENSUS_DUMPS, max_states=1 << 22, max_depth=0, term_cap=None):
    traces = np.ascontiguousarray(traces, dtype=np.uint16)
    counts = np.ascontiguousarray(counts, dtype=np.uint32).reshape(-1)
    assert traces.ndim == 2 and traces.shape[0] == np_ and counts.shape == (np_,)
    kind = CENSUS_KINDS.get(kind, kind)
    th = np.ascontiguousarray(thresh, dtype=np.uint32).reshape(-1)
    mask, key = fate_target(target)
    opts = ReachOpts(inbox_limit, kind, max_states, max_depth, 0)
    fopts = FateOpts(mask, max_sweeps, key)
    n = max_states if 0 < max_states <= 1 << 31 else 1
    term_cap = min(n, 1 << 20) if term_cap is None else term_cap
    nth = len(th)
    info = np.zeros(len(REACH_INFO_FIELDS), dtype=np.uint64)
    finfo = np.zeros(len(FATE_INFO_FIELDS), dtype=np.uint64)
    values = np.zeros((max(nth, 1), len(FATE_VALUE_FIELDS)), dtype=np.uint64)
    parents, masks, cls = np.zeros(n, np.uint32), np.zeros(n, np.uint8), np.zeros(n, np.uint8)
    level_off = np.zeros(REACH_MAX_LEVELS + 1, dtype=np.uint64)
    terms = np.zeros(max(term_cap, 1), dtype=REACH_TERMINAL_DTYPE)
    lo, hi = np.zeros((max(nth, 1), n), np.uint64), np.zeros((max(nth, 1), n), np.uint64)
    _check(lib().dsm_reach_fate(np_, _ptr(traces), _ptr(counts), traces.shape[1], ctypes.byref(opts), ctypes.byref(fopts),
                                _ptr(th) if nth else None, nth, _ptr(info), _ptr(finfo), _ptr(values), _ptr(parents),
                                _ptr(masks), _ptr(level_off), _ptr(terms), term_cap, _ptr(cls), _ptr(lo), _ptr(hi)),
           "dsm_reach_fate")
    return _fate_result(info, finfo, values, parents, masks, level_off, terms, kind, cls, lo, hi, nth)


def fate_seal_point(parents, cls, state):
    parents = np.ascontiguousarray(parents, dtype=np.uint32)
    cls = np.ascontiguousarray(cls, dtype=np.uint8)
    if not 0 <= state < min(len(parents), len(cls)):
        raise DsmError(E_INVAL, "fate_seal_point: state")
    s, d = ctypes.c_uint64(0), ctypes.c_uint64(0)
    _check(lib().dsm_fate_seal_point(_ptr(parents), _ptr(cls), state, ctypes.byref(s), ctypes.byref(d)),
           "dsm_fate_seal_point")
    return (None if s.value == FATE_NO_EDGE else s.value), d.value


RAUDIT_ALL, RAUDIT_QUIESCENT, RAUDIT_TERMINAL, RAUDIT_COMPLETED = range(4)
RAUDIT_NSETS = 4
RAUDIT_SET_NAMES = ["all", "quiescent", "terminal", "completed"]
RAUDIT_F_TRUNCATED, RAUDIT_F_INEXACT = 1, 2
RAUDIT_NONE = (1 << 64) - 1
RAUDIT_INFO_DTYPE = np.dtype([("set", AUDIT_DTYPE, (RAUDIT_NSETS,)), ("first_depth", "<u8", (RAUDIT_NSETS, 8)),
                              ("flags", "<u8"), ("reserved", "<u8", (3,))])
assert RAUDIT_INFO_DTYPE.itemsize == RAUDIT_NSETS * NAUDIT * 8 + RAUDIT_NSETS * 64 + 32


def _raudit_result(info, ainfo, parents, masks, level_off, terms, words, sets, term_words, term_cap):
    d = reach_info_to_dict(info)
    n, nt = d["states"], min(d["terminals"], term_cap)
    a = ainfo[0]
    return {"info": d, "parents": parents[:n], "masks": masks[:n], "level_off": level_off[:d["levels"] + 1],
            "terminals": terms[:nt], "words": words[:n], "sets": sets[:n], "term_words": term_words[:nt],
            "audit": a["set"].copy(), "flags": int(a["flags"]), "reserved": [int(x) for x in a["reserved"]],
            "first_depth": a["first_depth"].copy(),
            **{name: audit_to_dict(a["set"][k]) for k, name in enumerate(RAUDIT_SET_NAMES)}}


def reach_audit(np_, traces, counts, inbox_limit=16, kind=CENSUS_DUMPS, max_states=1 << 22, max_depth=0, term_cap=None):
    traces = np.ascontiguousarray(traces, dtype=np.uint16)
    counts = np.ascontiguousarray(counts, dtype=np.uint32).reshape(-1)
    assert traces.ndim == 2 and traces.shape[0] == np_ and counts.shape == (np_,)
    kind = CENSUS_KINDS.get(kind, kind)
    opts = ReachOpts(inbox_limit, kind, max_states, max_depth, 0)
    n = max_states if 0 < max_states <= 1 << 31 else 1
    term_cap = min(n, 1 << 20) if term_cap is None else term_cap
    info = np.zeros(len(REACH_INFO_FIELDS), dtype=np.uint64)
    ainfo = np.zeros(1, dtype=RAUDIT_INFO_DTYPE)
    parents, masks = np.zeros(n, np.uint32), np.zeros(n, np.uint8)
    words, sets = np.zeros(n, np.uint32), np.zeros(n, np.uint8)
    level_off = np.zeros(REACH_MAX_LEVELS + 1, dtype=np.uint64)
    terms = np.zeros(max(term_cap, 1), dtype=REACH_TERMINAL_DTYPE)
    term_words = np.zeros(max(term_cap, 1), np.uint32)
    _check(lib().dsm_reach_audit(np_, _ptr(traces), _ptr(counts), traces.shape[1], ctypes.byref(opts), _ptr(info),
                                 _ptr(ainfo), _ptr(parents), _ptr(masks), _ptr(level_off), _ptr(terms), term_cap,
                                 _ptr(words), _ptr(sets), _ptr(term_words)), "dsm_reach_audit")
    return _raudit_result(info, ainfo, parents, masks, level_off, terms, words, sets, term_words, term_cap)


def _reach_terminals_result(info, terms, kind):
    d = reach_info_to_dict(info)
    nt = min(d["terminals"], len(terms))
    table, cap = reach_census(terms[:nt], kind)
    return {"info": d, "terminals": terms[:nt], "census": table, "census_cap": cap, "outcomes": census_sorted(table, cap)}


class Group:

    @staticmethod
    def unique_id():
        b = (ctypes.c_ubyte * 128)()
        _check(lib().dsm_group_unique_id(b), "dsm_group_unique_id")
        return bytes(b)

    def __init__(self, device, nranks, rank, uid):
        assert len(uid) == 128
        self.g = ctypes.c_void_p()
        b = (ctypes.c_ubyte * 128).from_buffer_copy(uid)
        _check(lib().dsm_group_init_rank(device, nranks, rank, b, ctypes.byref(self.g)),
               "dsm_group_init_rank")

    def info(self):
        r, n, d = ctypes.c_int(), ctypes.c_int(), ctypes.c_int()
        _check(lib().dsm_group_info(self.g, ctypes.byref(r), ctypes.byref(n), ctypes.byref(d)),
               "dsm_group_info")
        return r.value, n.value, d.value

    def allreduce(self, d_buf, n, op=RED_SUM, stream=0):
        _check(lib().dsm_group_allreduce(self.g, _dptr(d_buf, 8 * n), n, op, ctypes.c_void_p(stream)),
               "dsm_group_allreduce")

    def allreduce_counters(self, d_counters, stream=0):
        _check(lib().dsm_group_allreduce_counters(self.g, _dptr(d_counters, COUNTERS_BYTES),
                                                  ctypes.c_void_p(stream)),
               "dsm_group_allreduce_counters")

    def allreduce_aggregate(self, d_agg, stream=0):
        _check(lib().dsm_group_allreduce_aggregate(self.g, _dptr(d_agg, NAGG * 8),
                                                   ctypes.c_void_p(stream)),
               "dsm_group_allreduce_aggregate")

    def barrier(self, stream=0):
        _check(lib().dsm_group_barrier(self.g, ctypes.c_void_p(stream)), "dsm_group_barrier")

    def close(self):
        if self.g:
            lib().dsm_group_close(self.g)
            self.g = ctypes.c_void_p()

    def __del__(self):
        try:
            self.close()
        except Exception:
            pass


def counters_to_dict(c):
    c = np.asarray(c, dtype=np.uint64).reshape(-1)
    return {k: int(v) for k, v in zip(COUNTER_FIELDS, c) if not k.startswith("reserved")}


def device_count():
    n = ctypes.c_int(0)
    _check(lib().dsm_device_count(ctypes.byref(n)), "dsm_device_count")
    return n.value


class Engine:

    def __init__(self, np_=8, max_instr=4096, ring_cap=0, snapshots=False, device=0, timing=False,
                 type_counts=False, issue_trace=False):
        self.np = np_
        self.max_instr = max_instr
        self.device = device
        self._sched = (0, SCHED_LOCKSTEP)
        self.cfg = Config(np_, max_instr, ring_cap,
                          (F_SNAPSHOTS if snapshots else 0) | (F_TIMING if timing else 0) |
                          (F_TYPE_COUNTS if type_counts else 0) |
                          (F_ISSUE_TRACE if issue_trace else 0))
        self.ctx = ctypes.c_void_p()
        _check(lib().dsm_open(device, ctypes.byref(self.cfg), ctypes.byref(self.ctx)), "dsm_open")

    def close(self):
        if self.ctx:
            lib().dsm_close(self.ctx)
            self.ctx = ctypes.c_void_p()

    def __enter__(self):
        return self

    def __exit__(self, *a):
        self.close()

    def __del__(self):
        try:
            self.close()
        except Exception:
            pass

    def run_packed(self, traces, counts):
        traces = np.ascontiguousarray(traces, dtype=np.uint16)
        counts = np.ascontiguousarray(counts, dtype=np.uint32)
        n = counts.shape[0]
        assert traces.shape == (n, self.np, self.max_instr), traces.shape
        assert counts.shape == (n, self.np)
        res = np.zeros(n, dtype=RESULT_DTYPE)
        cnt = np.zeros(NCOUNTERS, dtype=np.uint64)
        _check(lib().dsm_run_packed(self.ctx, _ptr(traces), _ptr(counts), n, _ptr(res), _ptr(cnt)),
               "dsm_run_packed")
        return res, counters_to_dict(cnt)

    def run_generated(self, dist, seed, n_instr, first_sys, n_sys):
        g = Gen(seed, DIST.get(dist, dist), n_instr)
        res = np.zeros(n_sys, dtype=RESULT_DTYPE)
        cnt = np.zeros(NCOUNTERS, dtype=np.uint64)
        _check(lib().dsm_run_generated(self.ctx, ctypes.byref(g), first_sys, n_sys, _ptr(res),
                                       _ptr(cnt)), "dsm_run_generated")
        return res, counters_to_dict(cnt)

    def generate_device(self, dist, seed, n_instr, first_sys, n_sys, d_traces, d_counts, stream=0):
        g = Gen(seed, DIST.get(dist, dist), n_instr)
        _check(lib().dsm_generate_device(self.ctx, ctypes.byref(g), first_sys, n_sys,
                                         ctypes.c_void_p(d_traces), ctypes.c_void_p(d_counts),
                                         ctypes.c_void_p(stream)), "dsm_generate_device")

    def run_packed_device(self, d_traces, d_counts, n_sys, d_results, d_counters, stream=0):
        _check(lib().dsm_run_packed_device(self.ctx, _dptr(d_traces), _dptr(d_counts), n_sys,
                                           _dptr(d_results), _dptr(d_counters, COUNTERS_BYTES),
                                           ctypes.c_void_p(stream)), "dsm_run_packed_device")

    def run_generated_device(self, dist, seed, n_instr, first_sys, n_sys, d_results, d_counters,
                             stream=0):
        g = Gen(seed, DIST.get(dist, dist), n_instr)
        _check(lib().dsm_run_generated_device(self.ctx, ctypes.byref(g), first_sys, n_sys,
                                              _dptr(d_results), _dptr(d_counters, COUNTERS_BYTES),
                                              ctypes.c_void_p(stream)), "dsm_run_generated_device")

    def aggregate_device(self, d_results, n_sys, first_sys, d_agg, stream=0):
        _check(lib().dsm_aggregate_device(self.ctx, _dptr(d_results), n_sys, first_sys,
                                          _dptr(d_agg, NAGG * 8), ctypes.c_void_p(stream)),
               "dsm_aggregate_device")

    def census_device(self, d_results, n_sys, first_sys, kind, d_census, cap, stream=0):
        nb = 8 * CENSUS_WORDS(cap) if _census_cap_ok(cap) else 0
        _check(lib().dsm_census_device(self.ctx, _dptr(d_results, 32 * n_sys), n_sys, first_sys,
                                       CENSUS_KINDS.get(kind, kind), _dptr(d_census, nb), cap,
                                       ctypes.c_void_p(stream)), "dsm_census_device")

    def census_run_nodes_device(self, first_sys, n_sys, d_census, cap, stream=0):
        nb = 8 * self.np * CENSUS_WORDS(cap) if _census_cap_ok(cap) else 0
        _check(lib().dsm_census_run_nodes_device(self.ctx, first_sys, n_sys, _dptr(d_census, nb),
                                                 cap, ctypes.c_void_p(stream)),
               "dsm_census_run_nodes_device")

    def audit_states_device(self, d_states, n_sys, first_sys, d_words, d_audit, state_stride=1,
                            stream=0):
        _check(lib().dsm_audit_states_device(self.ctx, _dptr(d_states), state_stride, n_sys,
                                             first_sys, _dptr(d_words, 4 * n_sys),
                                             _dptr(d_audit, 8 * NAUDIT), ctypes.c_void_p(stream)),
               "dsm_audit_states_device")

    def audit_run_device(self, first_sys, n_sys, d_words, d_audit, stream=0):
        _check(lib().dsm_audit_run_device(self.ctx, first_sys, n_sys, _dptr(d_words, 4 * n_sys),
                                          _dptr(d_audit, 8 * NAUDIT), ctypes.c_void_p(stream)),
               "dsm_audit_run_device")

    def debug_exscan_device(self, d_in, n, d_out, stream=0):
        _check(lib().dsm_debug_exscan_device(self.ctx, _dptr(d_in, 4 * n), n, _dptr(d_out, 8 * (n + 1)),
                                             ctypes.c_void_p(stream)), "dsm_debug_exscan_device")

    def trace_events_device(self, d_traces, d_counts, n_sys, d_ids, n_ids, d_events, event_cap,
                            d_n_events, d_hash, d_results, stream=0):
        _check(lib().dsm_trace_events_device(self.ctx, _dptr(d_traces), _dptr(d_counts), n_sys,
                                             _dptr(d_ids, 8 * n_ids), n_ids,
                                             _dptr(d_events, 8 * n_ids * event_cap), event_cap,
                                             _dptr(d_n_events, 4 * n_ids), _dptr(d_hash, 8 * n_ids),
                                             _dptr(d_results, 32 * n_ids), ctypes.c_void_p(stream)),
               "dsm_trace_events_device")

    def event_trace(self, traces, counts, ids=None, cap=0):
        import torch
        traces = np.ascontiguousarray(traces, dtype=np.uint16)
        counts = np.ascontiguousarray(counts, dtype=np.uint32)
        n_sys = counts.shape[0]
        assert traces.shape == (n_sys, self.np, self.max_instr), traces.shape
        assert counts.shape == (n_sys, self.np)
        dev = torch.device("cuda", self.device)
        d_tr = torch.from_numpy(traces.view(np.int16).reshape(-1)).to(dev)
        d_cn = torch.from_numpy(counts.view(np.int32).reshape(-1)).to(dev)
        d_ids = None
        if ids is not None:
            ids = np.ascontiguousarray(ids, dtype=np.uint64)
            d_ids = torch.from_numpy(ids.view(np.int64)).to(dev)
        n = n_sys if ids is None else len(ids)
        d_ev = torch.zeros(max(n * cap, 1), dtype=torch.int64, device=dev) if cap else None
        d_n = torch.zeros(max(n, 1), dtype=torch.int32, device=dev)
        d_h = torch.zeros(max(n, 1), dtype=torch.int64, device=dev)
        d_res = torch.zeros(4 * max(n, 1), dtype=torch.int64, device=dev)
        st = torch.cuda.current_stream(dev).cuda_stream
        self.trace_events_device(d_tr, d_cn, n_sys, d_ids, n, d_ev, cap, d_n, d_h, d_res, st)
        torch.cuda.synchronize(dev)
        ev = d_ev.cpu().numpy().view(np.uint64)[:n * cap].reshape(n, cap) if cap else None
        return (ev, d_n.cpu().numpy().view(np.uint32)[:n], d_h.cpu().numpy().view(np.uint64)[:n],
                d_res.cpu().numpy().view(RESULT_DTYPE)[:n])

    def reach_device(self, d_trace, d_counts, opts, info, d_parents, d_masks, d_fps, level_off, d_terminals,
                     term_cap, stream=0):
        return lib().dsm_reach_device(self.ctx, _dptr(d_trace), _dptr(d_counts), ctypes.byref(opts), _ptr(info),
                                      _dptr(d_parents), _dptr(d_masks), _dptr(d_fps), _ptr(level_off),
                                      _dptr(d_terminals), term_cap, ctypes.c_void_p(stream))

    def reach(self, traces, counts, inbox_limit=16, kind=CENSUS_DUMPS, max_states=1 << 22, max_depth=0, chunk=0,
              term_cap=None):
        import torch
        tr, cn = np.array(traces, dtype=np.uint16), np.array(counts, dtype=np.uint32)
        if tr.shape != (self.np, self.max_instr) or cn.shape != (self.np,):
            raise DsmError(E_INVAL, "reach: one system of the engine's np and max_instr")
        kind = CENSUS_KINDS.get(kind, kind)
        dev = torch.device("cuda", self.device)
        d_tr = torch.from_numpy(tr.view(np.int16).reshape(-1)).to(dev)
        d_cn = torch.from_numpy(cn.view(np.int32)).to(dev)
        ok = 0 < max_states <= 1 << 31
        n = max_states if ok else 1
        term_cap = min(n, 1 << 20) if term_cap is None else term_cap
        d_par = torch.zeros(n, dtype=torch.int32, device=dev)
        d_msk = torch.zeros(n, dtype=torch.uint8, device=dev)
        d_fps = torch.zeros(n, dtype=torch.int64, device=dev)
        d_term = torch.zeros(5 * max(term_cap, 1), dtype=torch.int64, device=dev)
        info = np.zeros(len(REACH_INFO_FIELDS), dtype=np.uint64)
        level_off = np.zeros(REACH_MAX_LEVELS + 1, dtype=np.uint64)
        opts = ReachOpts(inbox_limit, kind, max_states, max_depth, chunk)
        st = torch.cuda.current_stream(dev).cuda_stream
        _check(self.reach_device(d_tr, d_cn, opts, info, d_par, d_msk, d_fps, level_off, d_term, term_cap, st),
               "dsm_reach_device")
        return _reach_result(info, d_par.cpu().numpy().view(np.uint32), d_msk.cpu().numpy(),
                             d_fps.cpu().numpy().view(np.uint64),
                             level_off, d_term.cpu().numpy().view(REACH_TERMINAL_DTYPE), kind)

    def reach_batch_device(self, d_traces, d_counts, n_sys, opts, d_info, d_terminals, term_cap, d_parents, d_masks,
                           scratch_bytes=0, stream=0):
        return lib().dsm_reach_batch_device(self.ctx, _dptr(d_traces), _dptr(d_counts), n_sys, ctypes.byref(opts),
                                            scratch_bytes, _dptr(d_info), _dptr(d_terminals), term_cap,
                                            _dptr(d_parents), _dptr(d_masks), ctypes.c_void_p(stream))

    def reach_batch_state(self):
        w, b = ctypes.c_uint64(0), ctypes.c_uint64(0)
        _check(lib().dsm_debug_reach_batch_state(self.ctx, ctypes.byref(w), ctypes.byref(b)), "dsm_debug_reach_batch_state")
        return w.value, b.value

    def reach_many(self, traces, counts, inbox_limit=16, kind=CENSUS_DUMPS, max_states=1 << 16, max_depth=0, chunk=0,
                   term_cap=None, witnesses=False, scratch_bytes=0):
        import torch
        tr, cn = np.ascontiguousarray(traces, dtype=np.uint16), np.ascontiguousarray(counts, dtype=np.uint32)
        if tr.ndim != 3 or tr.shape[1:] != (self.np, self.max_instr) or cn.shape != tr.shape[:2]:
            raise DsmError(E_INVAL, "reach_many: systems of the engine's np and max_instr")
        n = tr.shape[0]
        dev = torch.device("cuda", self.device)
        d_tr = torch.from_numpy(tr.view(np.int16).reshape(-1)).to(dev)
        d_cn = torch.from_numpy(cn.view(np.int32).reshape(-1)).to(dev)
        ok = 0 < max_states <= REACH_BATCH_MAX_STATES
        cap = max_states if ok else 1
        term_cap = min(cap, 4096) if term_cap is None else term_cap
        nw = len(REACH_INFO_FIELDS)
        d_info = torch.zeros(max(n, 1) * nw, dtype=torch.int64, device=dev)
        d_term = torch.zeros(5 * max(n * term_cap, 1), dtype=torch.int64, device=dev)
        d_par = torch.zeros(max(n * cap, 1), dtype=torch.int32, device=dev) if witnesses else None
        d_msk = torch.zeros(max(n * cap, 1), dtype=torch.uint8, device=dev) if witnesses else None
        opts = ReachOpts(inbox_limit, CENSUS_KINDS.get(kind, kind), max_states, max_depth, chunk)
        st = torch.cuda.current_stream(dev).cuda_stream
        _check(self.reach_batch_device(d_tr, d_cn, n, opts, d_info, d_term, term_cap, d_par, d_msk, scratch_bytes, st),
               "dsm_reach_batch_device")
        info = d_info.cpu().numpy().view(REACH_INFO_DTYPE)[:n]
        terms = d_term.cpu().numpy().view(REACH_TERMINAL_DTYPE)[:n * term_cap]
        return _reach_many_result(info, terms, term_cap,
                                  d_par.cpu().numpy().view(np.uint32) if witnesses else None,
                                  d_msk.cpu().numpy() if witnesses else None, cap)

    def reach_dist_device(self, d_trace, d_counts, opts, thresh, max_rounds, rinfo, dinfo, d_terminals, d_term_mass,
                          term_cap, round_mass, stream=0):
        n = 0 if thresh is None else len(thresh)
        return lib().dsm_reach_dist_device(self.ctx, _dptr(d_trace), _dptr(d_counts), ctypes.byref(opts), _ptr(thresh), n,
                                           max_rounds, _ptr(rinfo), _ptr(dinfo), _dptr(d_terminals), _dptr(d_term_mass),
                                           term_cap, _ptr(round_mass), ctypes.c_void_p(stream))

    def reach_dist(self, traces, counts, thresh=(0x8000,), max_rounds=0, inbox_limit=16, kind=CENSUS_DUMPS,
                   max_states=1 << 22, max_depth=0, chunk=0, term_cap=None):
        import torch
        tr, cn = np.array(traces, dtype=np.uint16), np.array(counts, dtype=np.uint32)
        if tr.shape != (self.np, self.max_instr) or cn.shape != (self.np,):
            raise DsmError(E_INVAL, "reach_dist: one system of the engine's np and max_instr")
        kind = CENSUS_KINDS.get(kind, kind)
        th = np.ascontiguousarray(thresh, dtype=np.uint32).reshape(-1)
        dev = torch.device("cuda", self.device)
        d_tr = torch.from_numpy(tr.view(np.int16).reshape(-1)).to(dev)
        d_cn = torch.from_numpy(cn.view(np.int32)).to(dev)
        n = max_states if 0 < max_states <= 1 << 31 else 1
        term_cap = max(min(n, 1 << 20) if term_cap is None else term_cap, 1)
        R, nth = _dist_rounds(max_rounds), max(len(th), 1)
        d_term = torch.zeros(5 * term_cap, dtype=torch.int64, device=dev)
        d_tm = torch.zeros(nth * term_cap, dtype=torch.int64, device=dev)
        info = np.zeros(len(REACH_INFO_FIELDS), dtype=np.uint64)
        dinfo = np.zeros((nth, len(DIST_INFO_FIELDS)), dtype=np.uint64)
        round_mass = np.zeros((nth, R + 1), dtype=np.uint64)
        opts = ReachOpts(inbox_limit, kind, max_states, max_depth, chunk)
        st = torch.cuda.current_stream(dev).cuda_stream
        _check(self.reach_dist_device(d_tr, d_cn, opts, th, max_rounds, info, dinfo, d_term, d_tm, term_cap, round_mass, st),
               "dsm_reach_dist_device")
        terms = d_term.cpu().numpy().view(REACH_TERMINAL_DTYPE)
        term_mass = d_tm.cpu().numpy().view(np.uint64).reshape(nth, term_cap)
        return _dist_result(_reach_terminals_result(info, terms, kind), kind, dinfo, term_mass, round_mass)

    def reach_fate_device(self, d_trace, d_counts, opts, fopts, thresh, rinfo, finfo, values, d_parents, d_masks,
                          level_off, d_terminals, term_cap, d_cls, d_lo, d_hi, stream=0):
        n = 0 if thresh is None else len(thresh)
        return lib().dsm_reach_fate_device(self.ctx, _dptr(d_trace), _dptr(d_counts),
                                           None if opts is None else ctypes.byref(opts),
                                           None if fopts is None else ctypes.byref(fopts),
                                           _ptr(thresh) if n else None, n, _ptr(rinfo), _ptr(finfo),
                                           _ptr(values), _dptr(d_parents), _dptr(d_masks), _ptr(level_off),
                                           _dptr(d_terminals), term_cap, _dptr(d_cls), _dptr(d_lo), _dptr(d_hi),
                                           ctypes.c_void_p(stream))

    def reach_fate(self, traces, counts, target="deadlocked", thresh=(0x8000,), max_sweeps=0, inbox_limit=16,
                   kind=CENSUS_DUMPS, max_states=1 << 22, max_depth=0, chunk=0, term_cap=None):
        import torch
        tr, cn = np.array(traces, dtype=np.uint16), np.array(counts, dtype=np.uint32)
        if tr.shape != (self.np, self.max_instr) or cn.shape != (self.np,):
            raise DsmError(E_INVAL, "reach_fate: one system of the engine's np and max_instr")
        kind = CENSUS_KINDS.get(kind, kind)
        th = np.ascontiguousarray(thresh, dtype=np.uint32).reshape(-1)
        mask, key = fate_target(target)
        dev = torch.device("cuda", self.device)
        d_tr = torch.from_numpy(tr.view(np.int16).reshape(-1)).to(dev)
        d_cn = torch.from_numpy(cn.view(np.int32)).to(dev)
        n = max_states if 0 < max_states <= 1 << 31 else 1
        term_cap = max(min(n, 1 << 20) if term_cap is None else term_cap, 1)
        nth = len(th)
        d_par = torch.zeros(n, dtype=torch.int32, device=dev)
        d_msk = torch.zeros(n, dtype=torch.uint8, device=dev)
        d_cls = torch.zeros(n, dtype=torch.uint8, device=dev)
        d_lo = torch.zeros(max(nth, 1) * n, dtype=torch.int64, device=dev)
        d_hi = torch.zeros(max(nth, 1) * n, dtype=torch.int64, device=dev)
        d_term = torch.zeros(5 * term_cap, dtype=torch.int64, device=dev)
        info = np.zeros(len(REACH_INFO_FIELDS), dtype=np.uint64)
        finfo = np.zeros(len(FATE_INFO_FIELDS), dtype=np.uint64)
        values = np.zeros((max(nth, 1), len(FATE_VALUE_FIELDS)), dtype=np.uint64)
        level_off = np.zeros(REACH_MAX_LEVELS + 1, dtype=np.uint64)
        opts = ReachOpts(inbox_limit, kind, max_states, max_depth, chunk)
        fopts = FateOpts(mask, max_sweeps, key)
        st = torch.cuda.current_stream(dev).cuda_stream
        _check(self.reach_fate_device(d_tr, d_cn, opts, fopts, th, info, finfo, values, d_par, d_msk, level_off, d_term,
                                      term_cap, d_cls, d_lo, d_hi, st), "dsm_reach_fate_device")
        return _fate_result(info, finfo, values, d_par.cpu().numpy().view(np.uint32), d_msk.cpu().numpy(), level_off,
                            d_term.cpu().numpy().view(REACH_TERMINAL_DTYPE), kind, d_cls.cpu().numpy(),
                            d_lo.cpu().numpy().view(np.uint64).reshape(max(nth, 1), n),
                            d_hi.cpu().numpy().view(np.uint64).reshape(max(nth, 1), n), nth)

    def reach_audit_device(self, d_trace, d_counts, opts, rinfo, ainfo, d_parents, d_masks, level_off, d_terminals,
                           term_cap, d_words, d_sets, d_term_words, stream=0):
        return lib().dsm_reach_audit_device(self.ctx, _dptr(d_trace), _dptr(d_counts),
                                            None if opts is None else ctypes.byref(opts), _ptr(rinfo), _ptr(ainfo),
                                            _dptr(d_parents), _dptr(d_masks), _ptr(level_off), _dptr(d_terminals),
                                            term_cap, _dptr(d_words), _dptr(d_sets), _dptr(d_term_words),
                                            ctypes.c_void_p(stream))

    def reach_audit(self, traces, counts, inbox_limit=16, kind=CENSUS_DUMPS, max_states=1 << 22, max_depth=0, chunk=0,
                    term_cap=None):
        import torch
        tr, cn = np.array(traces, dtype=np.uint16), np.array(counts, dtype=np.uint32)
        if tr.shape != (self.np, self.max_instr) or cn.shape != (self.np,):
            raise DsmError(E_INVAL, "reach_audit: one system of the engine's np and max_instr")
        kind = CENSUS_KINDS.get(kind, kind)
        dev = torch.device("cuda", self.device)
        d_tr = torch.from_numpy(tr.view(np.int16).reshape(-1)).to(dev)
        d_cn = torch.from_numpy(cn.view(np.int32)).to(dev)
        n = max_states if 0 < max_states <= 1 << 31 else 1
        term_cap = min(n, 1 << 20) if term_cap is None else term_cap
        d_par = torch.zeros(n, dtype=torch.int32, device=dev)
        d_msk = torch.zeros(n, dtype=torch.uint8, device=dev)
        d_words = torch.zeros(n, dtype=torch.int32, device=dev)
        d_sets = torch.zeros(n, dtype=torch.uint8, device=dev)
        d_term = torch.zeros(5 * max(term_cap, 1), dtype=torch.int64, device=dev)
        d_tw = torch.zeros(max(term_cap, 1), dtype=torch.int32, device=dev)
        info = np.zeros(len(REACH_INFO_FIELDS), dtype=np.uint64)
        ainfo = np.zeros(1, dtype=RAUDIT_INFO_DTYPE)
        level_off = np.zeros(REACH_MAX_LEVELS + 1, dtype=np.uint64)
        opts = ReachOpts(inbox_limit, kind, max_states, max_depth, chunk)
        st = torch.cuda.current_stream(dev).cuda_stream
        _check(self.reach_audit_device(d_tr, d_cn, opts, info, ainfo, d_par, d_msk, level_off, d_term, term_cap, d_words,
                                       d_sets, d_tw, st), "dsm_reach_audit_device")
        return _raudit_result(info, ainfo, d_par.cpu().numpy().view(np.uint32), d_msk.cpu().numpy(), level_off,
                              d_term.cpu().numpy().view(REACH_TERMINAL_DTYPE), d_words.cpu().numpy().view(np.uint32),
                              d_sets.cpu().numpy(), d_tw.cpu().numpy().view(np.uint32), term_cap)

    def explore(self, traces, counts, k, seed, thresh=0x8000, kind=CENSUS_DUMPS, audit=False):
        import torch
        if not 1 <= k <= CENSUS_MAX_CAP:
            raise DsmError(E_INVAL, "explore: k")
        if audit and not self.cfg.flags & F_SNAPSHOTS:
            raise DsmError(E_STATE, "explore: audit needs an engine with snapshots")
        cap, dev, d_tr, d_cn, d_res, d_cnt, st = self._stage_variants(traces, counts, k)
        d_cen = torch.zeros(CENSUS_WORDS(cap), dtype=torch.int64, device=dev)
        prev = self._sched
        self.set_schedule(seed, thresh)
        try:
            self.run_packed_device(d_tr, d_cn, k, d_res, d_cnt, st)
            self.census_device(d_res, k, 0, kind, d_cen, cap, st)
            if audit:
                d_words = torch.zeros(k, dtype=torch.int32, device=dev)
                d_aud = torch.zeros(NAUDIT, dtype=torch.int64, device=dev)
                self.audit_run_device(0, k, d_words, d_aud, st)
            table = d_cen.cpu().numpy().view(np.uint64)
        finally:
            self.set_schedule(*prev)
        outcomes = census_sorted(table, cap)
        if not audit:
            return outcomes
        words = d_words.cpu().numpy().view(np.uint32)[outcomes["first_sys"].astype(np.int64)]
        return outcomes, words, d_aud.cpu().numpy().view(AUDIT_DTYPE)[0]

    def _stage_variants(self, traces, counts, k):
        import torch
        tr = np.ascontiguousarray(traces, dtype=np.uint16).reshape(1, self.np, self.max_instr)
        cn = np.ascontiguousarray(counts, dtype=np.uint32).reshape(1, self.np)
        cap = max(CENSUS_MIN_CAP, 1 << (k - 1).bit_length())
        dev = torch.device("cuda", self.device)
        d_tr = torch.zeros(k * tr.size + 8, dtype=torch.int16, device=dev)
        d_tr[:k * tr.size].view(k, tr.size)[:] = torch.from_numpy(tr.view(np.int16).reshape(-1)).to(dev)
        d_cn = torch.zeros(k * self.np + 1, dtype=torch.int32, device=dev)
        d_cn[:k * self.np].view(k, self.np)[:] = torch.from_numpy(cn.view(np.int32).reshape(-1)).to(dev)
        d_res = torch.zeros(4 * k, dtype=torch.int64, device=dev)
        d_cnt = torch.zeros(NCOUNTERS, dtype=torch.int64, device=dev)
        return cap, dev, d_tr, d_cn, d_res, d_cnt, torch.cuda.current_stream(dev).cuda_stream

    def check_dumps(self, traces, counts, k, seed, thresh, dumps):
        import torch
        if not 1 <= k <= CENSUS_MAX_CAP:
            raise DsmError(E_INVAL, "check_dumps: k")
        if not self.cfg.flags & F_SNAPSHOTS:
            raise DsmError(E_STATE, "check_dumps: needs an engine with snapshots")
        if len(dumps) != self.np:
            raise DsmError(E_INVAL, "check_dumps: one item per core")
        target, keys = [], []
        for c, text in enumerate(dumps):
            if text is None:
                target.append(None)
                keys.append(OUTCOME_MISSING)
                continue
            node, rec = parse_dump(text)
            if node != c:
                raise DsmError(E_FORMAT, f"check_dumps: core {c}'s text prints node {node}")
            target.append(rec[:60].tobytes())
            keys.append(max(node_hash(c, rec, 15), 2))
        cap, dev, d_tr, d_cn, d_res, d_cnt, st = self._stage_variants(traces, counts, k)
        words = CENSUS_WORDS(cap)
        d_cen = torch.zeros((1 + self.np) * words, dtype=torch.int64, device=dev)
        prev = self._sched
        self.set_schedule(seed, thresh)
        try:
            self.run_packed_device(d_tr, d_cn, k, d_res, d_cnt, st)
            self.census_device(d_res, k, 0, CENSUS_DUMPS, d_cen[:words], cap, st)
            self.census_run_nodes_device(0, k, d_cen[words:], cap, st)
            tables = d_cen.cpu().numpy().view(np.uint64).reshape(1 + self.np, words)
        finally:
            self.set_schedule(*prev)
        out = {"k": k, "cores": [], "dropped": int(tables[:, 2].sum())}
        for c in range(self.np):
            hit = census_find(tables[1 + c], cap, keys[c])
            out["cores"].append({"key": keys[c], "count": hit[0] if hit else 0,
                                 "first": hit[1] if hit else None})
        by_agree = {}
        for o in census_sorted(tables[0], cap):
            rep, agree = int(o["first_sys"]), 0
            for c in range(self.np):
                d, f = self.node_state(rep, c)
                mine = d[:60].tobytes() if f[61] & 2 else None
                agree += mine == target[c]
            cnt, first = by_agree.get(agree, (0, rep))
            by_agree[agree] = (cnt + int(o["count"]), min(first, rep))
        cnt, first = by_agree.pop(self.np, (0, None))
        out["joint"] = {"count": cnt, "first": first}
        out["closest"] = None
        if by_agree:
            a = max(by_agree)
            out["closest"] = {"agree": a, "count": by_agree[a][0], "first": by_agree[a][1]}
        return out

    def node_state(self, sys, node):
        d = np.zeros(64, dtype=np.uint8)
        f = np.zeros(64, dtype=np.uint8)
        _check(lib().dsm_get_node_state(self.ctx, sys, node, _ptr(d), _ptr(f)), "dsm_get_node_state")
        return d, f

    def parse_traces(self, files, cap):
        n = len(files)
        assert n % self.np == 0
        text = np.frombuffer(b"".join(files) + b"\0" * 16, dtype=np.uint8)
        off = np.zeros(n + 1, dtype=np.uint64)
        off[1:] = np.cumsum([len(f) for f in files])
        tr = np.zeros((n // self.np, self.np, self.max_instr), dtype=np.uint16)
        cn = np.zeros((n // self.np, self.np), dtype=np.uint32)
        st = np.zeros((n // self.np, self.np), dtype=np.int32)
        _check(lib().dsm_parse_traces(self.ctx, _ptr(text), _ptr(off), n, cap, _ptr(tr), _ptr(cn),
                                      _ptr(st)), "dsm_parse_traces")
        return tr, cn, st

    def parse_traces_device(self, d_text, d_offsets, n_files, cap, d_traces, d_counts, d_status,
                            stream=0):
        _check(lib().dsm_parse_traces_device(self.ctx, ctypes.c_void_p(d_text),
                                             ctypes.c_void_p(d_offsets), n_files, cap,
                                             ctypes.c_void_p(d_traces), ctypes.c_void_p(d_counts),
                                             ctypes.c_void_p(d_status), ctypes.c_void_p(stream)),
               "dsm_parse_traces_device")

    def generate_text_device(self, dist, seed, n_instr, first_sys, n_sys, d_text, d_offsets,
                             stream=0):
        g = Gen(seed, DIST.get(dist, dist), n_instr)
        _check(lib().dsm_generate_text_device(self.ctx, ctypes.byref(g), first_sys, n_sys,
                                              ctypes.c_void_p(d_text), ctypes.c_void_p(d_offsets),
                                              ctypes.c_void_p(stream)), "dsm_generate_text_device")

    def format_dumps_device(self, d_states, n_states, d_text, d_len, state_stride=1, stream=0):
        _check(lib().dsm_format_dumps_device(self.ctx, ctypes.c_void_p(d_states), state_stride,
                                             n_states, ctypes.c_void_p(d_text),
                                             ctypes.c_void_p(d_len), ctypes.c_void_p(stream)),
               "dsm_format_dumps_device")

    def format_run_dumps_device(self, view, first_sys, n_sys, d_text, d_len, stream=0):
        _check(lib().dsm_format_run_dumps_device(self.ctx, view, first_sys, n_sys,
                                                 ctypes.c_void_p(d_text), ctypes.c_void_p(d_len),
                                                 ctypes.c_void_p(stream)),
               "dsm_format_run_dumps_device")

    def parse_dumps_device(self, d_text, d_len, n, d_states, d_status=None, state_stride=1, stream=0):
        _check(lib().dsm_parse_dumps_device(self.ctx, _dptr(d_text, DUMP_SLOT * n), _dptr(d_len, 4 * n), n,
                                            _dptr(d_states, 64 * ((n - 1) * state_stride + 1) if n else 0),
                                            state_stride, _dptr(d_status, 4 * n), ctypes.c_void_p(stream)),
               "dsm_parse_dumps_device")

    def write_run_dumps(self, sys, node_mask, out_dir=None):
        _check(lib().dsm_write_run_dumps(self.ctx, sys, node_mask,
                                         out_dir.encode() if out_dir else None),
               "dsm_write_run_dumps")

    def set_schedule(self, seed, act_thresh=SCHED_LOCKSTEP):
        _check(lib().dsm_set_schedule(self.ctx, seed, act_thresh), "dsm_set_schedule")
        self._sched = (seed, act_thresh)

    def issue_trace(self, sys):
        cap = self.np * self.max_instr
        ev = np.zeros(cap, dtype=np.uint32)
        n = ctypes.c_uint32(0)
        _check(lib().dsm_get_issue_trace(self.ctx, sys, _ptr(ev), cap, ctypes.byref(n)),
               "dsm_get_issue_trace")
        return ev[:min(n.value, cap)].copy()

    def last_kernel_ms(self):
        ms = ctypes.c_float(0)
        _check(lib().dsm_last_kernel_ms(self.ctx, ctypes.byref(ms)), "dsm_last_kernel_ms")
        return float(ms.value)

    def kernel_ms_history(self, cap=64):
        ms = np.zeros(max(cap, 1), dtype=np.float32)
        n = ctypes.c_uint32(0)
        _check(lib().dsm_kernel_ms_history(self.ctx, _ptr(ms), cap, ctypes.byref(n)),
               "dsm_kernel_ms_history")
        return [float(x) for x in ms[:n.value]]

    def set_budget(self, budget_log2, late_log2=9):
        _check(lib().dsm_set_budget(self.ctx, budget_log2, late_log2), "dsm_set_budget")

    def set_round_limit(self, limit_log2):
        _check(lib().dsm_set_round_limit(self.ctx, limit_log2), "dsm_set_round_limit")

    def set_inbox_limit(self, cap):
        _check(lib().dsm_set_inbox_limit(self.ctx, cap), "dsm_set_inbox_limit")

    def set_fast_forward(self, mode):
        _check(lib().dsm_set_fast_forward(self.ctx, mode), "dsm_set_fast_forward")

    def order_state(self, n_sys, sys=None):
        counts = np.zeros(4, dtype=np.uint32)
        rw, hl = ctypes.c_uint32(0), ctypes.c_int(-1)
        if sys is not None:
            rec = np.zeros(512, dtype=np.uint32)
            rc = lib().dsm_debug_order_state(self.ctx, _ptr(counts), None, None, 0, sys, _ptr(rec),
                                             rec.size, ctypes.byref(rw), ctypes.byref(hl))
            _check(min(rc, 0), "dsm_debug_order_state")
            return (rec[:rw.value].copy(), bool(hl.value)) if rw.value else (None, None)
        n = n_sys
        lst = np.zeros(max(n, 1), dtype=np.uint32)
        order = np.zeros(max(2 * n, 1), dtype=np.uint32)
        rc = lib().dsm_debug_order_state(self.ctx, _ptr(counts), _ptr(lst), _ptr(order), order.size,
                                         0, None, 0, ctypes.byref(rw), ctypes.byref(hl))
        _check(min(rc, 0), "dsm_debug_order_state")
        nl, ns, nm = int(counts[1]), int(counts[2]), int(counts[3])
        d = {"launched": rc == 1, "suspended": int(counts[0]), "long": nl, "short": ns, "multi": nm,
             "list": lst[:int(counts[0])].copy(), "order_long": None, "order_short": None}
        if rc == 1:
            d["order_long"] = np.concatenate([order[n:n + nm], order[n - (nl - nm):n][::-1]])
            d["order_short"] = order[:ns][::-1].copy()
        return d

    def launch_info(self):
        li = LaunchInfo()
        _check(lib().dsm_launch_info_get(self.ctx, ctypes.byref(li)), "dsm_launch_info_get")
        d = {k: getattr(li, k) for k, _ in LaunchInfo._fields_}
        buf = ctypes.create_string_buffer(256)
        n = lib().dsm_launch_kernel_names(ctypes.byref(li), buf, 256)
        if n < 0:
            raise DsmError(n, "dsm_launch_kernel_names")
        d["kernels"] = buf.raw[:n].decode()
        return d


def parse_trace_file(path, cap=32):
    out = np.zeros(max(cap, 1), dtype=np.uint16)
    n = ctypes.c_uint32(0)
    rc = lib().dsm_parse_trace_file(path.encode(), _ptr(out), cap, ctypes.byref(n))
    _check(rc, f"dsm_parse_trace_file({path})")
    return out[:n.value].copy()


def format_dump(node, rec):
    rec = np.ascontiguousarray(rec, dtype=np.uint8)
    assert rec.size == 64
    buf = ctypes.create_string_buffer(4096)
    n = lib().dsm_format_dump(node, _ptr(rec), buf, 4096)
    if n < 0:
        raise DsmError(n, "dsm_format_dump")
    return buf.raw[:n].decode()


def parse_dump_rc(text, length=None):
    raw = text.encode("latin-1") if isinstance(text, str) else bytes(text)
    length = len(raw) if length is None else length
    assert 0 <= length <= len(raw)
    buf = np.frombuffer(raw, dtype=np.uint8) if raw else np.zeros(1, dtype=np.uint8)
    rec = np.full(64, 0xEE, dtype=np.uint8)
    node = ctypes.c_int(-2)
    rc = lib().dsm_parse_dump(_ptr(buf), length, ctypes.byref(node), _ptr(rec))
    return rc, node.value, rec


def parse_dump(text):
    rc, node, rec = parse_dump_rc(text)
    _check(rc, "dsm_parse_dump")
    return node, rec


def read_dump(node, dump_dir=None):
    rec = np.zeros(64, dtype=np.uint8)
    _check(lib().dsm_read_dump(node, dump_dir.encode() if dump_dir else None, _ptr(rec)),
           f"dsm_read_dump({node})")
    return rec


def split_dumps(text, lens):
    text = np.asarray(text, dtype=np.uint8).reshape(-1, DUMP_SLOT)
    return [bytes(text[k, :int(n)]).decode() for k, n in enumerate(np.asarray(lens))]


def format_issue_trace(events):
    events = np.ascontiguousarray(events, dtype=np.uint32)
    cap = 64 * max(len(events), 1) + 1
    buf = ctypes.create_string_buffer(cap)
    n = lib().dsm_format_issue_trace(_ptr(events), len(events), buf, cap)
    if n < 0:
        raise DsmError(n, "dsm_format_issue_trace")
    return buf.raw[:n].decode()


def node_hash(node, rec, nwords):
    rec = np.ascontiguousarray(rec, dtype=np.uint8)
    return int(lib().dsm_node_hash(node, _ptr(rec), nwords))


def pack_instr(op, addr, value=0):
    wr = 1 if op in ("W", "WR") else 0
    return (wr << 15) | ((addr & 0x7F) << 8) | ((value & 0xFF) if wr else 0)


_M64 = np.uint64(0xFFFFFFFFFFFFFFFF)


def _fmix64(z):
    z = z ^ (z >> np.uint64(33))
    z = z * np.uint64(0xff51afd7ed558ccd)
    z = z ^ (z >> np.uint64(33))
    z = z * np.uint64(0xc4ceb9fe1a85ec53)
    return z ^ (z >> np.uint64(33))


def result_digest(res, first_idx=0):
    res = np.ascontiguousarray(res).view(RESULT_DTYPE).reshape(-1)
    with np.errstate(over="ignore"):
        idx = np.arange(first_idx, first_idx + len(res), dtype=np.uint64)
        h = _fmix64(idx * np.uint64(0x9E3779B97F4A7C15) + np.uint64(1))
        h = _fmix64(h ^ (res["status"].astype(np.uint64) | (res["rounds"].astype(np.uint64) << np.uint64(32))))
        h = _fmix64(h ^ (res["msgs"].astype(np.uint64) | (res["instrs"].astype(np.uint64) << np.uint64(32))))
        h = _fmix64(h ^ res["dump_hash"])
        h = _fmix64(h ^ res["final_hash"])
        return int(h.sum(dtype=np.uint64))


def aggregate(res, first_idx=0):
    res = np.ascontiguousarray(res).view(RESULT_DTYPE).reshape(-1)
    st = np.bincount((res["status"] & 0xFF).astype(np.int64), minlength=5)
    with np.errstate(over="ignore"):
        return {"systems": int(len(res)), "msgs": int(res["msgs"].sum(dtype=np.uint64)),
                "instrs": int(res["instrs"].sum(dtype=np.uint64)),
                "rounds": int(res["rounds"].sum(dtype=np.uint64)),
                "max_rounds": int(res["rounds"].max()) if len(res) else 0,
                "status": [int(x) for x in st[:5]],
                "sum_dump_hash": "0x%016x" % int(res["dump_hash"].sum(dtype=np.uint64)),
                "sum_final_hash": "0x%016x" % int(res["final_hash"].sum(dtype=np.uint64)),
                "result_digest": "0x%016x" % result_digest(res, first_idx)}


AGG_KEYS = ("systems", "msgs", "instrs", "rounds", "max_rounds", "status", "sum_dump_hash",
            "sum_final_hash", "result_digest")


def aggregate_diff(mine, gold):
    return [k for k in AGG_KEYS if mine.get(k) != gold.get(k)]
```

Before: 105.7 billion.

## Split serial-tail kernel claims across a multi-wave share path with separate args

```diff
diff --git a/hp-assignment-2_amd/csrc/dsm_args.h b/hp-assignment-2_amd/csrc/dsm_args.h
--- a/hp-assignment-2_amd/csrc/dsm_args.h
+++ b/hp-assignment-2_amd/csrc/dsm_args.h
@@ -53,7 +53,8 @@
     uint32_t serfmt;
     uint32_t split;
 };
-struct SimArgsPack { SimArgs a[3]; };
+struct SimArgsPack { SimArgs a[4]; };
+#define ARGS_SERX 3
 
 enum { K_MSGS = 13, K_INSTRS = 14, K_ROUNDS = 15, K_SYSTEMS = 16, K_STATUS = 17, K_DHASH = 22,
        K_FHASH = 23, K_MAXR = 24, K_OVFRERUN = 25, K_WROUNDS = 26, K_RESUMED = 27,
@@ -72,6 +73,7 @@
 #define CTRL_SUSPL 1568
 #define CTRL_SUSPS 1600
 #define CTRL_SUSPM 1632
+#define CTRL_SERX 1664
 #define CTRL_SCAN 1792
 
 #endif
diff --git a/hp-assignment-2_amd/csrc/dsm_internal.h b/hp-assignment-2_amd/csrc/dsm_internal.h
--- a/hp-assignment-2_amd/csrc/dsm_internal.h
+++ b/hp-assignment-2_amd/csrc/dsm_internal.h
@@ -80,6 +80,8 @@
                                      uint64_t cap, uint64_t sys, uint32_t *rec, uint32_t rec_cap,
                                      uint32_t *rec_words, int *host_long);
 
+extern "C" int dsm_debug_ser_claims(dsm_ctx *c, uint32_t *out);
+
 extern "C" int dsm_debug_reach_times(double *ms, uint64_t *chunks);
 
 extern "C" int dsm_debug_dist_edges(int np, const uint16_t *trace, const uint32_t *counts, uint32_t stride,
@@ -110,7 +112,8 @@
 DSM_LOCAL void dsm_sim_launch(sim_fn f, unsigned grid, unsigned threads, hipStream_t st, const SimArgs *a);
 DSM_LOCAL int dsm_sim_lds_bytes(int ring, int waves);
 DSM_LOCAL void dsm_order_launch(int np, unsigned blocks, hipStream_t st, const SimArgs *a);
-DSM_LOCAL void dsm_ser_launch(int np, bool cap, unsigned blocks, hipStream_t st, const SimArgs *a);
+DSM_LOCAL void dsm_ser_launch(int np, bool cap, unsigned blocks, hipStream_t st, const SimArgs *a,
+                              const SimArgs *ax, uint32_t *took);
 DSM_LOCAL void dsm_args_launch(const SimArgsPack &pk, SimArgs *dst, hipStream_t st);
 DSM_LOCAL void dsm_scan_launch(int np, unsigned blocks, hipStream_t st, const uint16_t *traces,
                                const uint32_t *counts, uint32_t stride, uint64_t n_sys, uint32_t *scan,
diff --git a/hp-assignment-2_amd/csrc/dsm_knobs.h b/hp-assignment-2_amd/csrc/dsm_knobs.h
--- a/hp-assignment-2_amd/csrc/dsm_knobs.h
+++ b/hp-assignment-2_amd/csrc/dsm_knobs.h
@@ -30,6 +30,9 @@
 #ifndef SER_SOLO_HW
 #define SER_SOLO_HW 2
 #endif
+#ifndef SER_MW_SHARE
+#define SER_MW_SHARE 8
+#endif
 #ifndef SER_DEAD_FWD
 #define SER_DEAD_FWD 1
 #endif
diff --git a/hp-assignment-2_amd/csrc/dsm_runtime.hip b/hp-assignment-2_amd/csrc/dsm_runtime.hip
--- a/hp-assignment-2_amd/csrc/dsm_runtime.hip
+++ b/hp-assignment-2_amd/csrc/dsm_runtime.hip
@@ -238,6 +238,16 @@
     return pl.order ? 1 : 0;
 }
 
+extern "C" int dsm_debug_ser_claims(dsm_ctx *c, uint32_t *out) {
+    if (!c || !out) return DSM_E_INVAL;
+    HIPCK(hipSetDevice(c->device));
+    HIPCK(hipStreamSynchronize(c->last_st ? c->last_st : c->stream));
+    const unsigned int at[4] = {CTRL_SERX, CTRL_RES, CTRL_RES + 32, CTRL_RES + 64};
+    for (int i = 0; i < 4; ++i)
+        HIPCK(hipMemcpy(&out[i], c->d_ctrl + at[i], sizeof(uint32_t), hipMemcpyDeviceToHost));
+    return DSM_OK;
+}
+
 static void put_sched(SimArgs &a, const PlanArgs &s) {
     a.rsh = s.rsh; a.budget = s.budget; a.resume = s.resume; a.ffsel = s.ffsel;
     a.late_rsh = s.late_rsh; a.thr_ff = s.thr_ff; a.lone = s.lone; a.lone_min = s.lone_min;
@@ -349,6 +359,10 @@
     C.claim = c->d_ctrl + CTRL_RES;
     A.scan = C.scan = c->d_ctrl + CTRL_SCAN;
     for (int i = 0; i < 3; ++i) put_sched(pk.a[i], p.args[i]);
+    SimArgs &X = pk.a[ARGS_SERX];
+    X = C;
+    X.ffsel = 1;
+    X.scan = c->d_ctrl + CTRL_SERX;
     dsm_args_launch(pk, c->d_args, st);
     HIPCK(hipGetLastError());
 
@@ -371,7 +385,7 @@
             dsm_order_launch(np, p.order_blocks, st, a);
             break;
         case PK_SER:
-            dsm_ser_launch(np, L.mode != 0, p.ser_blocks, st, a);
+            dsm_ser_launch(np, L.mode != 0, p.ser_blocks, st, a, c->d_args + ARGS_SERX, c->d_ctrl + CTRL_SERX);
             break;
         case PK_RERUN:
             if (timed) {
diff --git a/hp-assignment-2_amd/csrc/dsm_ser.hip b/hp-assignment-2_amd/csrc/dsm_ser.hip
--- a/hp-assignment-2_amd/csrc/dsm_ser.hip
+++ b/hp-assignment-2_amd/csrc/dsm_ser.hip
@@ -52,500 +52,15 @@
 template <int NP, bool CAP>
 __global__ void __launch_bounds__(64 * SER_WAVES) __attribute__((amdgpu_waves_per_eu(2)))
 ser_kernel(const SimArgs *Ap) {
-    using namespace dsms;
-    constexpr uint32_t NPM = (1u << NP) - 1u;
-    constexpr bool SOLO = !CAP;
-    if (DSM_SER_EXITS(Ap)) return;
-
-    __shared__ uint32_t s_ser[SER_WAVES][S_WORDS][64];
-    __shared__ uint2 s_tab[DT_TABLE_WORDS / 2];
-    __shared__ unsigned long long s_cnt[K_N];
-    __shared__ uint32_t s_dum[64];
-    const uint32_t lane = threadIdx.x & 63u, wv = threadIdx.x >> 6;
-    if (threadIdx.x < K_N) s_cnt[threadIdx.x] = 0;
-    for (uint32_t i = threadIdx.x; i < DT_TABLE_WORDS / 2; i += 64 * SER_WAVES) s_tab[i] = Ap->table[i];
-    __syncthreads();
-#if SIM_TAILPROBE
-    const uint64_t tprobe0 = __builtin_amdgcn_s_memrealtime();
-#endif
-
-    const LdsCol<SER_WAVES> m{s_ser, &s_dum[lane], wv, lane,
-                              (GU32 *)(Ap->spill + ((uint64_t)blockIdx.x * (64 * SER_WAVES) + threadIdx.x) * S_SPILL)};
-    const LdsTab T{s_tab};
-    const bool ordered = Ap->serfmt != 0u && Ap->susp_order != nullptr;
-    const uint32_t nmulti = ordered ? *Ap->susp_multi : 0u;
-    const uint32_t nlong = nmulti + (ordered ? *Ap->susp_long : 0u);
-    const uint32_t n = uni32(*Ap->d_n);
-    const uint32_t lcap = Ap->susp_cap;
-    const uint32_t *const list = ordered ? Ap->susp_order : Ap->list;
-    auto sel = [&](uint32_t k) -> uint32_t {
-        return ((const GU32 *)list)[k < nmulti ? lcap + k : k < nlong ? lcap - 1u - (k - nmulti) : n - 1u - k];
-    };
-
-    const uint32_t stride = Ap->stride, lim_rsh = Ap->lim_rsh, SR = Ap->susp_ring;
-    const uint32_t cap = Ap->icap;
-    const uint16_t *const traces = Ap->traces;
-
-    uint4 *const recs = Ap->recs;
-    dsm_sys_result *const results = Ap->results;
-    const uint32_t *const susp = Ap->susp;
-    uint32_t *const ovf_list = Ap->ovf_list;
-    unsigned int *const ovf_count = Ap->ovf_count, *const claim_ctr = Ap->claim;
-
-    SReg r;
-    SCache cc;
-    ser_cache_clear(cc);
-    uint64_t sys = 0;
-    uint32_t tn = 0xFFu, tci = 0, pfc = 0;
-    bool nxv = false, pfv = false;
-    uint4 cur = make_uint4(0, 0, 0, 0), nx = cur, pf = cur;
-    auto slot_of = [&](uint32_t nd) { return traces + (sys * NP + nd) * (uint64_t)stride; };
-
-    auto claim_next = [&]() -> uint32_t {
-        return gatomic_add((GU32 *)claim_ctr, 1u);
-    };
-
-
-    auto start_ls = [&]() {
-        const GU32 *sp = (const GU32 *)(susp + sys * ((uint64_t)susp_words((int)SR) * NP));
-        r.rounds = sp[(12u + SR + 6u) * NP];
-        for (uint32_t nd = 0; nd < (uint32_t)NP; ++nd) {
-            const GU32 *b = sp + nd;
-#pragma unroll
-            for (uint32_t i = 0; i < 8; ++i) m.st(S_MB + 8u * nd + i, b[i * NP]);
-            uint32_t la = 0, lv = 0, ls = 0;
-#pragma unroll
-            for (uint32_t i = 0; i < 4; ++i) {
-                const uint32_t l = b[(8u + i) * NP];
-                la |= (l & 0xFFu) << (8 * i);
-                lv |= ((l >> 8) & 0xFFu) << (8 * i);
-                ls |= ((l >> 16) & 3u) << (2 * i);
-            }
-            m.st(S_LA + nd, la);
-            m.st(S_LV + nd, lv);
-            const GU32 *q = b + (12u + SR) * NP;
-            const uint32_t ctl = q[NP], ip = q[2 * NP], rh = q[4 * NP];
-            m.st(S_DS + nd, q[0]);
-            m.st(S_CT + nd, (ctl & 0x3FFu) | (ls << SC_LS) | (ip << SC_IP));
-            s_set_ni(r, nd, q[3 * NP]);
-            const uint32_t h = rh & 0xFFu, c = rh >> 8;
-            for (uint32_t j = 0; j < c; ++j) {
-                uint32_t sl = h + j;
-                sl = sl >= SR ? sl - SR : sl;
-                ser_enqueue<S_QN>(m, r, nd, b[(12u + sl) * NP]);
-            }
-            s_byte_add(r.cnt0, r.cnt1, nd, c);
-            r.nz |= (c ? 1u : 0u) << nd;
-            r.msgs += q[5 * NP] - c;
-            r.iss |= ((ctl & (C_WAIT | C_DUMPED)) == 0u ? 1u : 0u) << nd;
-            r.dmp |= ((ctl & C_DUMPED) ? 1u : 0u) << nd;
-        }
-    };
-    const bool serfmt = Ap->serfmt != 0u;
-    v4u32 rr[33];
-    auto load_rec = [&](uint64_t s_) {
-        const GV4 *sv = (const GV4 *)(susp + s_ * (uint64_t)ssusp_words((int)SR));
-#pragma unroll
-        for (uint32_t i = 0; i < 33; ++i) rr[i] = sv[i];
-    };
-    auto start = [&]() -> uint32_t {
-        ser_clear(r);
-        tn = 0xFFu;
-        nxv = pfv = false;
-        if (!serfmt) {
-            start_ls();
-        } else {
-        const GU32 *sp = (const GU32 *)(susp + sys * (uint64_t)ssusp_words((int)SR));
-#pragma unroll
-        for (uint32_t i = 0; i < 24; ++i) {
-            const uint32_t w = 4u * i;
-            m.st(w, rr[i].x); m.st(w + 1u, rr[i].y); m.st(w + 2u, rr[i].z); m.st(w + 3u, rr[i].w);
-        }
-        const v4u32 *const hd = rr + 24;
-        r.rounds = hd[6].x;
-        auto hw = [&](uint32_t k) -> uint32_t {
-            const v4u32 &v = hd[k >> 2];
-            return (k & 3u) == 0u ? v.x : (k & 3u) == 1u ? v.y : (k & 3u) == 2u ? v.z : v.w;
-        };
-#pragma unroll
-        for (uint32_t nd = 0; nd < (uint32_t)NP; ++nd) {
-            const uint32_t rh = hw(nd), c = rh >> 8, ctl = m.ld(S_CT + nd);
-            s_set_ni(r, nd, hw(8u + nd));
-            for (uint32_t j = 0; j < c; ++j)
-                ser_enqueue<S_QN>(m, r, nd, sp[SSUSP_HDR + nd * SR + j]);
-            s_byte_add(r.cnt0, r.cnt1, nd, c);
-            r.nz |= (c ? 1u : 0u) << nd;
-            r.msgs += hw(16u + nd) - c;
-            r.iss |= ((ctl & (SC_WAIT | SC_DUMPED)) == 0u ? 1u : 0u) << nd;
-            r.dmp |= ((ctl & SC_DUMPED) ? 1u : 0u) << nd;
-        }
-        if (hd[6].y & 0x100u) {
-            tn = hd[6].y & 0xFFu;
-            const uint32_t ip0 = m.ld(S_CT + tn) >> SC_IP, j0 = ip0 & 7u;
-            const uint32_t rw[4] = {hd[7].x, hd[7].y, hd[7].z, hd[7].w};
-            uint32_t al[4] = {0u, 0u, 0u, 0u};
-#pragma unroll
-            for (uint32_t k = 0; k < 8u; ++k) {
-                uint32_t hv = 0u;
-#pragma unroll
-                for (uint32_t q = 0; q < 8u; ++q)
-                    hv = (k >= j0 && k - j0 == q) ? ((rw[q >> 1] >> (16u * (q & 1u))) & 0xFFFFu) : hv;
-                al[k >> 1] |= hv << (16u * (k & 1u));
-            }
-            cur = make_uint4(al[0], al[1], al[2], al[3]);
-            nx = make_uint4(hd[8].x, hd[8].y, hd[8].z, hd[8].w);
-            tci = ip0 >> 3;
-            nxv = true;
-            pfc = tci + 2u;
-            pfv = pfc * 8u < stride;
-            if (pfv) pf = ld16(slot_of(tn) + pfc * 8u);
-        }
-        }
-        r.E = r.nz;
-        r.A = r.nz | r.iss;
-        ser_cache_clear(cc);
-        if (SOLO && serfmt && tn != 0xFFu) {
-            cc.ct = m.ld(S_CT + tn); cc.la = m.ld(S_LA + tn); cc.lv = m.ld(S_LV + tn);
-            cc.node = tn;
-        }
-        if (r.A == 0u) {
-            r.st = (r.dmp == NPM) ? SS_COMPLETED : SS_DEADLOCKED;
-            return SR_DONE;
-        }
-        return SR_RUN;
-    };
-    auto store_rec = [&](uint32_t nd, uint32_t flags, uint32_t which) {
-        if (REC_PROBE) return;
-        GV4 *dst = (GV4 *)(recs + (sys * NP + nd) * 8 + 4u * which);
-#pragma unroll
-        for (int q = 0; q < 4; ++q) {
-            v4u32 x;
-            x.x = ser_rec_word(m, nd, flags, 4 * q);
-            x.y = ser_rec_word(m, nd, flags, 4 * q + 1);
-            x.z = ser_rec_word(m, nd, flags, 4 * q + 2);
-            x.w = ser_rec_word(m, nd, flags, 4 * q + 3);
-            dst[q] = x;
-        }
-    };
-    auto fetch = [&](uint32_t nd, uint32_t ip, bool iss) -> uint32_t {
-        const uint32_t c = ip >> 3;
-        const bool tnd = tn == nd;
-        const bool rot = iss & tnd & (tci + 1u == c) & nxv;
-        const bool miss = iss & !rot & (!tnd | (tci != c));
-        cur.x = rot ? nx.x : cur.x; cur.y = rot ? nx.y : cur.y;
-        cur.z = rot ? nx.z : cur.z; cur.w = rot ? nx.w : cur.w;
-        nxv = nxv & !rot;
-        tci = rot ? c : tci;
-        if (__ballot(miss)) {
-            if (SER_PROBE && lane == 0) atomicAdd(&s_cnt[3], 1ull);
-            if (miss) {
-                const uint16_t *sl = slot_of(nd);
-                cur = ld16(sl + 8u * c);
-                nxv = (c + 1u) * 8u < stride;
-                nx = ld16(sl + (nxv ? 8u * (c + 1u) : 8u * c));
-                pfv = false;
-                tn = nd;
-                tci = c;
-            }
-            wait_vmcnt0();
-        }
-        const uint32_t j = ip & 7u;
-        const uint32_t m2 = 0u - ((j >> 1) & 1u), m4 = 0u - ((j >> 2) & 1u);
-        const uint32_t lo = (cur.x & ~m2) | (cur.y & m2), hi = (cur.z & ~m2) | (cur.w & m2);
-        const uint32_t wd = (lo & ~m4) | (hi & m4);
-        return (wd >> (16u * (j & 1u))) & 0xFFFFu;
-    };
-    auto fetch_reg = [&](uint32_t nd, uint32_t ip, uint32_t &ins) -> bool {
-        const uint32_t c = ip >> 3;
-        const bool tnd = tn == nd;
-        const bool rot = tnd & (tci + 1u == c) & nxv;
-        const bool have = tnd & ((tci == c) | rot);
-        cur.x = rot ? nx.x : cur.x; cur.y = rot ? nx.y : cur.y;
-        cur.z = rot ? nx.z : cur.z; cur.w = rot ? nx.w : cur.w;
-        nxv = nxv & !rot;
-        tci = rot ? c : tci;
-        const uint32_t j = ip & 7u;
-        const uint32_t m2 = 0u - ((j >> 1) & 1u), m4 = 0u - ((j >> 2) & 1u);
-        const uint32_t lo = (cur.x & ~m2) | (cur.y & m2), hi = (cur.z & ~m2) | (cur.w & m2);
-        const uint32_t wd = (lo & ~m4) | (hi & m4);
-        ins = (wd >> (16u * (j & 1u))) & 0xFFFFu;
-        return have;
-    };
-    bool live = false;
-    uint32_t v = SR_RUN;
-    auto refill = [&]() {
-        if (pfv && !nxv && pfc == tci + 1u) {
-            nx = pf;
-            nxv = true;
-            pfv = false;
-        }
-        if (pfv && (pfc <= tci || pfc > tci + 2u)) pfv = false;
-        const uint32_t want = nxv ? tci + 2u : tci + 1u;
-        if (tn != 0xFFu && !pfv && want * 8u < stride && v == SR_RUN) {
-            pf = ld16(slot_of(tn) + want * 8u);
-            pfc = want;
-            pfv = true;
-        }
-    };
-    auto on_dump = [&](uint32_t nd) { store_rec(nd, 2u, 0u); };
-    auto finish = [&](uint32_t v) {
-        if (v == SR_OVF) {
-            const uint32_t pos = gatomic_add((GU32 *)ovf_count, 1u);
-            ((GU32 *)ovf_list)[pos] = (uint32_t)sys;
-            atomicAdd(&s_cnt[K_OVFRERUN], 1ull);
-            return;
-        }
-        uint32_t ins = 0;
-#pragma unroll
-        for (uint32_t nd = 0; nd < (uint32_t)NP; ++nd) {
-            ins += m.ld(S_CT + nd) >> SC_IP;
-            store_rec(nd, ser_final_flags(m, nd), 1u);
-        }
-        v4u32 res;
-        res.x = r.st | (r.dmp << 8); res.y = r.rounds; res.z = r.msgs; res.w = ins;
-        ((GV4 *)results)[2 * sys] = res;
-        atomicAdd(&s_cnt[K_MSGS], (unsigned long long)r.msgs);
-        atomicAdd(&s_cnt[K_INSTRS], (unsigned long long)ins);
-        atomicAdd(&s_cnt[K_ROUNDS], (unsigned long long)r.rounds);
-        atomicAdd(&s_cnt[K_SYSTEMS], 1ull);
-        atomicAdd(&s_cnt[K_STATUS + r.st], 1ull);
-        atomicMax(&s_cnt[K_MAXR], (unsigned long long)r.rounds);
-    };
-
-    {
-        const uint32_t k = claim_next();
-        live = k < n;
-        if (live) sys = sel(k);
-        if (live && serfmt) load_rec(sys);
-    }
-    v = live ? start() : SR_RUN;
-    uint32_t iters = 0, nmac = 0;
-    uint32_t tclaim = 0, now_it = 0;
-    bool lone0 = false;
-    [[maybe_unused]] uint64_t pr_long = 0, pr_last = 0, pr_n4k = 0, pr_nl_it = 0, pr_it = 0, pr_nl_n = 0;
-    if constexpr (SIM_TAILPROBE == 2) lone0 = live && serfmt && (rr[30].y & 0x100u);
-    uint32_t hwait = 0;
-    uint64_t pb_runs = 0, pb_steps = 0, pb_idle = 0, pb_cyc = 0;
-    for (;;) {
-        bool taken = false, rest = false;
-#pragma unroll 1
-        for (int k = 0; k < SER_RF; ++k) {
-            bool ran_now = false, gen = true;
-            if (SOLO) {
-                if (k == 0) {
-                    uint64_t ts0 = 0;
-                    if (SER_PROBE >= 2) ts0 = __builtin_amdgcn_s_memtime();
-                    const bool run = live && v == SR_RUN;
-                    const bool ql = run && ser_quiet_lone(r, lim_rsh);
-                    const uint32_t sn = ql ? dsms::s_ctz(r.A) : 0xFEu;
-                    const uint32_t c = cc.ct >> (SC_IP + 3u);
-                    const bool hotq = ql & (cc.node == sn) & (tn == sn);
-                    const bool rot = hotq & (tci + 1u == c) & nxv;
-                    cur.x = rot ? nx.x : cur.x; cur.y = rot ? nx.y : cur.y;
-                    cur.z = rot ? nx.z : cur.z; cur.w = rot ? nx.w : cur.w;
-                    nxv = nxv & !rot;
-                    tci = rot ? c : tci;
-                    const bool elig = hotq & (tci == c);
-                    const uint32_t ne = (uint32_t)__builtin_popcountll(__ballot(elig));
-                    const uint32_t nr = (uint32_t)__builtin_popcountll(__ballot(run));
-                    if (ne != 0u && ne * 64u >= nr * (uint32_t)SER_SOLO_MIN) {
-                        uint32_t ns = 0;
-                        if (elig) ns = ser_solo<NP>(m, r, cc, cur.x, cur.y, cur.z, cur.w, lim_rsh);
-                        nmac += ns;
-                        taken = ran_now = true;
-                        rest = elig & (ns != 0u) & (((cc.ct >> SC_IP) & 7u) == 0u);
-                        iters += 1u;
-                        if (SER_PROBE) {
-                            uint32_t t = ns;
-                            for (int o = 1; o < 64; o <<= 1) t += __shfl_xor(t, o, 64);
-                            pb_runs += 1u; pb_steps += t; pb_idle += 8u * nr - t;
-                            if (SER_PROBE >= 2) pb_cyc += __builtin_amdgcn_s_memtime() - ts0;
-                        }
-                    }
-                }
-                if (taken) {
-                    gen = __ballot(live && v == SR_RUN && !rest) != 0ull;
-                    if (!gen && !ran_now) break;
-                }
-                iters += gen ? 1u : 0u;
-            }
-            bool mac = false;
-            uint64_t tp0 = 0, tp1 = 0, tp2 = 0;
-            if (SER_PROBE >= 2) tp0 = __builtin_amdgcn_s_memtime();
-            if (!CAP && gen) {
-#pragma unroll
-                for (int j = 0; j < SER_MACRO; ++j) {
-                    const bool q = live && v == SR_RUN && !rest && ser_quiet_lone(r, lim_rsh) && (j == 0 || mac);
-                    bool did = false;
-                    bool nohave = false;
-                    if (SER_PROBE && q) {
-                        const uint32_t n0 = dsms::s_ctz(r.A), ip0 = m.ld(S_CT + n0) >> SC_IP, c0 = ip0 >> 3;
-                        nohave = !((tn == n0) & ((tci == c0) | ((tci + 1u == c0) & nxv)));
-                    }
-                    if (SER_PROBE >= 4) {
-                        uint64_t ts[5] = {0, 0, 0, 0, 0};
-                        auto stamp = [&](int i) { __builtin_amdgcn_s_waitcnt(0); ts[i + 1] = __builtin_amdgcn_s_memtime(); };
-                        __builtin_amdgcn_s_waitcnt(0);
-                        ts[0] = __builtin_amdgcn_s_memtime();
-                        if (__ballot(q) && q) did = ser_macro<NP>(m, r, cc, fetch_reg, on_dump, stamp);
-                        const uint64_t okb = __ballot(did);
-                        if (okb && lane == (uint32_t)__builtin_ctzll(okb)) {
-                            atomicAdd(&s_cnt[13], ts[1] - ts[0]);
-                            atomicAdd(&s_cnt[14], ts[2] - ts[1]);
-                            atomicAdd(&s_cnt[15], ts[3] - ts[2]);
-                            atomicAdd(&s_cnt[16], ts[4] - ts[3]);
-                        }
-                    } else if (__ballot(q) && q) {
-                        did = ser_macro<NP>(m, r, cc, fetch_reg, on_dump, [](int) {});
-                    }
-                    if (SER_PROBE && j == 0) {
-                        const uint64_t nh = __ballot(nohave);
-                        if (lane == 0) atomicAdd(&s_cnt[8 + 3], 0ull + __builtin_popcountll(nh));
-                    }
-                    if (SER_PROBE && j == 0) {
-                        const bool nq_ = live && v == SR_RUN && !q;
-                        const uint64_t nq = __ballot(nq_), qn = __ballot(q && !did);
-                        const uint64_t mi = __ballot(nq_ && (r.iss & (r.iss - 1u)) != 0u);
-                        if (lane == 0) {
-                            atomicAdd(&s_cnt[9], (unsigned long long)__builtin_popcountll(nq));
-                            atomicAdd(&s_cnt[10], (unsigned long long)__builtin_popcountll(qn));
-                            (void)mi;
-                        }
-                    }
-                    mac = mac || did;
-                    nmac += did ? 1u : 0u;
-                }
-                if (mac && r.A == 0u) v = SR_DONE;
-                if (SOLO) rest = rest | (taken & mac);
-            }
-            if (SER_PROBE) {
-                const uint64_t gm = __ballot(live && v == SR_RUN && !mac), mm = __ballot(mac);
-                const uint64_t lv = __ballot(live);
-                if (lane == 0) {
-                    atomicAdd(&s_cnt[8], (unsigned long long)__builtin_popcountll(lv));
-                    if (__builtin_popcountll(lv) < 32) atomicAdd(&s_cnt[12], 1ull);
-                    atomicAdd(&s_cnt[0], 1ull);
-                    if (mm) atomicAdd(&s_cnt[1], 1ull);
-                    if (gm) atomicAdd(&s_cnt[2], 1ull);
-                }
-            }
-            if (SER_PROBE >= 2) tp1 = __builtin_amdgcn_s_memtime();
-            if (live && v == SR_RUN && !mac && gen && !rest) {
-                v = ser_step<NP, S_QN, CAP>(m, r, T, fetch, on_dump, lim_rsh, cap);
-                ser_cache_clear(cc);
-            }
-            if (SER_PROBE >= 2) tp2 = __builtin_amdgcn_s_memtime();
-            if (SER_PROBE) {
-                const uint64_t hm = __ballot(live && v != SR_RUN);
-                if (lane == 0 && hm) atomicAdd(&s_cnt[4], 1ull);
-            }
-            bool hgo = false;
-            const uint64_t fin = __ballot(live && v != SR_RUN);
-            if (fin) {
-                hgo = (uint32_t)__builtin_popcountll(fin) >= (uint32_t)SER_HB ||
-                      hwait >= (uint32_t)SER_HT || fin == __ballot(live);
-                hwait = hgo ? 0u : hwait + (gen ? 1u : 0u) + (ran_now ? (uint32_t)SER_SOLO_HW : 0u);
-            }
-            if (hgo && live && v != SR_RUN) {
-                if constexpr (SIM_TAILPROBE == 2) now_it = iters + (uint32_t)k;
-                uint64_t th0 = 0, th1 = 0, th2 = 0;
-                if (SER_PROBE >= 3) th0 = __builtin_amdgcn_s_memtime();
-                wait_vmcnt0();
-                const uint32_t k = claim_next();
-                const bool nl = k < n;
-                const uint32_t ns = nl ? sel(k) : 0u;
-                if (nl && serfmt) load_rec(ns);
-                if (SER_PROBE >= 3) { __builtin_amdgcn_s_waitcnt(0); th1 = __builtin_amdgcn_s_memtime(); }
-                if constexpr (SIM_TAILPROBE == 2) {
-                    const uint64_t dur = (uint64_t)(now_it - tclaim);
-                    const uint64_t a = (dur << 32) | (uint64_t)sys;
-                    const uint64_t b = ((uint64_t)now_it << 32) | ((uint64_t)lone0 << 31) | dur;
-                    pr_long = a > pr_long ? a : pr_long;
-                    pr_last = b > pr_last ? b : pr_last;
-                    pr_n4k += dur > 4000u ? 1u : 0u;
-                    pr_nl_it += lone0 ? 0u : dur;
-                    pr_it += dur;
-                    pr_nl_n += lone0 ? 0u : 1u;
-                    tclaim = now_it;
-                    lone0 = nl && serfmt && (rr[30].y & 0x100u);
-                }
-                finish(v);
-                if (SER_PROBE >= 3) { __builtin_amdgcn_s_waitcnt(0); th2 = __builtin_amdgcn_s_memtime(); }
-                live = nl;
-                sys = ns;
-                rest = false;
-                v = live ? start() : SR_RUN;
-                if (SER_PROBE >= 3) {
-                    __builtin_amdgcn_s_waitcnt(0);
-                    const uint64_t th3 = __builtin_amdgcn_s_memtime();
-                    const uint64_t fl = __ballot(true);
-                    if (lane == (uint32_t)__builtin_ctzll(fl)) {
-                        atomicAdd(&s_cnt[13], th1 - th0);
-                        atomicAdd(&s_cnt[14], th2 - th1);
-                        atomicAdd(&s_cnt[15], th3 - th2);
-                    }
-                }
-            }
-            if (SER_PROBE >= 2 && lane == 0) {
-                const uint64_t tp3 = __builtin_amdgcn_s_memtime();
-                atomicAdd(&s_cnt[5], tp1 - tp0);
-                atomicAdd(&s_cnt[6], tp2 - tp1);
-                atomicAdd(&s_cnt[7], tp3 - tp2);
-            }
-            if (!gen) break;
-        }
-        uint64_t tr0 = 0;
-        if (SER_PROBE >= 2) tr0 = __builtin_amdgcn_s_memtime();
-        refill();
-        (void)tr0;
-        if (!SOLO) iters += SER_RF;
-        if (__ballot(live) == 0) break;
-    }
-#if SIM_TAILPROBE == 2
-    {
-        uint64_t v6[6] = {pr_long, pr_last, pr_n4k, pr_nl_it, pr_it, pr_nl_n};
-#pragma unroll
-        for (int q = 0; q < 6; ++q) {
-            uint64_t x = v6[q];
-            for (int o = 1; o < 64; o <<= 1) {
-                const uint32_t lo = __shfl_xor((uint32_t)x, o, 64), hi = __shfl_xor((uint32_t)(x >> 32), o, 64);
-                const uint64_t y = ((uint64_t)hi << 32) | lo;
-                x = q < 2 ? (y > x ? y : x) : x + y;
-            }
-            if (lane == 0) {
-                if (q < 2) atomicMax(&Ap->counters[q], (unsigned long long)x);
-                else atomicAdd(&Ap->counters[q], (unsigned long long)x);
-            }
-        }
-    }
-#endif
-    if (lane == 0) {
-        atomicAdd(&s_cnt[K_WROUNDS], (unsigned long long)iters);
-        atomicAdd(&Ap->counters[K_SERIT], (unsigned long long)iters);
-        if (SER_PROBE && SOLO && !SIM_TAILPROBE) {
-            atomicAdd(&Ap->counters[K_SERPROBE], (unsigned long long)pb_runs);
-            atomicAdd(&Ap->counters[K_SERPROBE + 1], (unsigned long long)pb_steps);
-            atomicAdd(&Ap->counters[K_SERPROBE + 2], (unsigned long long)pb_idle);
-            atomicAdd(&Ap->counters[K_SERPROBE + 3], (unsigned long long)pb_cyc);
-        }
-#if SIM_TAILPROBE
-        const uint64_t ms = (__builtin_amdgcn_s_memrealtime() - tprobe0) / 100000u;
-        atomicAdd(&Ap->counters[K_SERPROBE + (ms < 11u ? 0u : (ms - 10u < 5u ? ms - 10u : 5u))], 1ull);
-#endif
-    }
-    if (!CAP) {
-        uint32_t t = nmac;
-        for (int o = 1; o < 64; o <<= 1) t += __shfl_xor(t, o, 64);
-        if (lane == 0 && t) atomicAdd(&Ap->counters[K_SERMAC], (unsigned long long)t);
-    }
-    __syncthreads();
-    if (threadIdx.x < K_N) {
-        const unsigned long long x = s_cnt[threadIdx.x];
-        if (x) {
-            if (threadIdx.x == K_MAXR) atomicMax(&Ap->counters[K_MAXR], x);
-            else atomicAdd(&Ap->counters[threadIdx.x], x);
-        }
-    }
+    constexpr bool MW = false;
+    [[maybe_unused]] uint32_t *const took = nullptr;
+#include "dsm_ser_body.h"
+}
+template <int NP, bool CAP>
+__global__ void __launch_bounds__(64 * SER_WAVES) __attribute__((amdgpu_waves_per_eu(2)))
+ser_multi_kernel(const SimArgs *Ap, uint32_t *took) {
+    constexpr bool MW = true;
+#include "dsm_ser_body.h"
 }
 
 struct RecCol {
@@ -606,8 +121,12 @@
 void dsm_order_launch(int np, unsigned blocks, hipStream_t st, const SimArgs *a) {
     hipLaunchKernelGGL(np == 4 ? order_kernel<4> : order_kernel<8>, dim3(blocks), dim3(ORD_THREADS), 0, st, a);
 }
-void dsm_ser_launch(int np, bool cap, unsigned blocks, hipStream_t st, const SimArgs *a) {
+void dsm_ser_launch(int np, bool cap, unsigned blocks, hipStream_t st, const SimArgs *a, const SimArgs *ax,
+                    uint32_t *took) {
+    hipLaunchKernelGGL(np == 4 ? (cap ? ser_multi_kernel<4, true> : ser_multi_kernel<4, false>)
+                               : (cap ? ser_multi_kernel<8, true> : ser_multi_kernel<8, false>),
+                       dim3(blocks), dim3(64 * SER_WAVES), 0, st, a, took);
     hipLaunchKernelGGL(np == 4 ? (cap ? ser_kernel<4, true> : ser_kernel<4, false>)
                                : (cap ? ser_kernel<8, true> : ser_kernel<8, false>),
-                       dim3(blocks), dim3(64 * SER_WAVES), 0, st, a);
+                       dim3(blocks), dim3(64 * SER_WAVES), 0, st, ax);
 }
diff --git a/hp-assignment-2_amd/csrc/dsm_ser_body.h b/hp-assignment-2_amd/csrc/dsm_ser_body.h
--- /dev/null
+++ b/hp-assignment-2_amd/csrc/dsm_ser_body.h
@@ -0,0 +1,526 @@
+    using namespace dsms;
+    constexpr uint32_t NPM = (1u << NP) - 1u;
+    constexpr bool SOLO = !CAP;
+    if constexpr (MW) {
+        const bool ffx = DSM_SER_EXITS(Ap);
+        const bool mine = !ffx && Ap->serfmt != 0u && Ap->susp_order != nullptr && *Ap->susp_multi != 0u;
+        if ((ffx || mine) && blockIdx.x == 0 && threadIdx.x == 0) took[0] = took[1] = 1u;
+        if (!mine) return;
+    } else {
+    if (DSM_SER_EXITS(Ap)) return;
+    }
+
+    __shared__ uint32_t s_ser[SER_WAVES][S_WORDS][64];
+    __shared__ uint2 s_tab[DT_TABLE_WORDS / 2];
+    __shared__ unsigned long long s_cnt[K_N];
+    __shared__ uint32_t s_dum[64];
+    const uint32_t lane = threadIdx.x & 63u, wv = threadIdx.x >> 6;
+    if (threadIdx.x < K_N) s_cnt[threadIdx.x] = 0;
+    for (uint32_t i = threadIdx.x; i < DT_TABLE_WORDS / 2; i += 64 * SER_WAVES) s_tab[i] = Ap->table[i];
+    __syncthreads();
+#if SIM_TAILPROBE
+    const uint64_t tprobe0 = __builtin_amdgcn_s_memrealtime();
+#endif
+
+    const LdsCol<SER_WAVES> m{s_ser, &s_dum[lane], wv, lane,
+                              (GU32 *)(Ap->spill + ((uint64_t)blockIdx.x * (64 * SER_WAVES) + threadIdx.x) * S_SPILL)};
+    const LdsTab T{s_tab};
+    const bool ordered = Ap->serfmt != 0u && Ap->susp_order != nullptr;
+    const uint32_t nmulti = ordered ? *Ap->susp_multi : 0u;
+    const uint32_t nlong = nmulti + (ordered ? *Ap->susp_long : 0u);
+    const uint32_t n = uni32(*Ap->d_n);
+    const uint32_t lcap = Ap->susp_cap;
+    const uint32_t *const list = ordered ? Ap->susp_order : Ap->list;
+    auto sel = [&](uint32_t k) -> uint32_t {
+        return ((const GU32 *)list)[k < nmulti ? lcap + k : k < nlong ? lcap - 1u - (k - nmulti) : n - 1u - k];
+    };
+
+    const uint32_t stride = Ap->stride, lim_rsh = Ap->lim_rsh, SR = Ap->susp_ring;
+    const uint32_t cap = Ap->icap;
+    const uint16_t *const traces = Ap->traces;
+
+    uint4 *const recs = Ap->recs;
+    dsm_sys_result *const results = Ap->results;
+    const uint32_t *const susp = Ap->susp;
+    uint32_t *const ovf_list = Ap->ovf_list;
+    unsigned int *const ovf_count = Ap->ovf_count, *const claim_ctr = Ap->claim;
+
+    SReg r;
+    SCache cc;
+    ser_cache_clear(cc);
+    uint64_t sys = 0;
+    uint32_t tn = 0xFFu, tci = 0, pfc = 0;
+    bool nxv = false, pfv = false;
+    uint4 cur = make_uint4(0, 0, 0, 0), nx = cur, pf = cur;
+    auto slot_of = [&](uint32_t nd) { return traces + (sys * NP + nd) * (uint64_t)stride; };
+
+    [[maybe_unused]] const uint32_t nwaves = gridDim.x * (uint32_t)SER_WAVES;
+    [[maybe_unused]] const uint32_t mw_spread = nwaves / (uint32_t)SER_MW_SHARE ? nwaves / (uint32_t)SER_MW_SHARE : 1u;
+    [[maybe_unused]] const uint32_t mw_l0 = (nmulti + mw_spread - 1u) / mw_spread;
+    [[maybe_unused]] const uint32_t mw_lanes = mw_l0 < 64u ? mw_l0 : 64u;
+    [[maybe_unused]] const uint32_t mw_want = (nmulti + mw_lanes - 1u) / (MW ? mw_lanes : 1u);
+    [[maybe_unused]] const bool mwave =
+        MW && blockIdx.x * (uint32_t)SER_WAVES + wv < (mw_want < nwaves / 2u ? mw_want : nwaves / 2u);
+    auto claim_next = [&]() -> uint32_t {
+        if constexpr (MW) {
+            GU32 *const rest_ctr = (GU32 *)claim_ctr + 32, *const multi_ctr = (GU32 *)claim_ctr + 64;
+            if (mwave) {
+                if (lane >= mw_lanes) return n;
+                const uint32_t b = gatomic_add(multi_ctr, 1u);
+                if (b < nmulti) return b;
+                if (gatomic_add(rest_ctr, 0u) < nlong - nmulti) return n;
+            }
+            const uint32_t a = gatomic_add(rest_ctr, 1u);
+            return a < n - nmulti ? nmulti + a : n;
+        }
+        return gatomic_add((GU32 *)claim_ctr, 1u);
+    };
+
+
+    auto start_ls = [&]() {
+        const GU32 *sp = (const GU32 *)(susp + sys * ((uint64_t)susp_words((int)SR) * NP));
+        r.rounds = sp[(12u + SR + 6u) * NP];
+        for (uint32_t nd = 0; nd < (uint32_t)NP; ++nd) {
+            const GU32 *b = sp + nd;
+#pragma unroll
+            for (uint32_t i = 0; i < 8; ++i) m.st(S_MB + 8u * nd + i, b[i * NP]);
+            uint32_t la = 0, lv = 0, ls = 0;
+#pragma unroll
+            for (uint32_t i = 0; i < 4; ++i) {
+                const uint32_t l = b[(8u + i) * NP];
+                la |= (l & 0xFFu) << (8 * i);
+                lv |= ((l >> 8) & 0xFFu) << (8 * i);
+                ls |= ((l >> 16) & 3u) << (2 * i);
+            }
+            m.st(S_LA + nd, la);
+            m.st(S_LV + nd, lv);
+            const GU32 *q = b + (12u + SR) * NP;
+            const uint32_t ctl = q[NP], ip = q[2 * NP], rh = q[4 * NP];
+            m.st(S_DS + nd, q[0]);
+            m.st(S_CT + nd, (ctl & 0x3FFu) | (ls << SC_LS) | (ip << SC_IP));
+            s_set_ni(r, nd, q[3 * NP]);
+            const uint32_t h = rh & 0xFFu, c = rh >> 8;
+            for (uint32_t j = 0; j < c; ++j) {
+                uint32_t sl = h + j;
+                sl = sl >= SR ? sl - SR : sl;
+                ser_enqueue<S_QN>(m, r, nd, b[(12u + sl) * NP]);
+            }
+            s_byte_add(r.cnt0, r.cnt1, nd, c);
+            r.nz |= (c ? 1u : 0u) << nd;
+            r.msgs += q[5 * NP] - c;
+            r.iss |= ((ctl & (C_WAIT | C_DUMPED)) == 0u ? 1u : 0u) << nd;
+            r.dmp |= ((ctl & C_DUMPED) ? 1u : 0u) << nd;
+        }
+    };
+    const bool serfmt = Ap->serfmt != 0u;
+    v4u32 rr[33];
+    auto load_rec = [&](uint64_t s_) {
+        const GV4 *sv = (const GV4 *)(susp + s_ * (uint64_t)ssusp_words((int)SR));
+#pragma unroll
+        for (uint32_t i = 0; i < 33; ++i) rr[i] = sv[i];
+    };
+    auto start = [&]() -> uint32_t {
+        ser_clear(r);
+        tn = 0xFFu;
+        nxv = pfv = false;
+        if (!serfmt) {
+            start_ls();
+        } else {
+        const GU32 *sp = (const GU32 *)(susp + sys * (uint64_t)ssusp_words((int)SR));
+#pragma unroll
+        for (uint32_t i = 0; i < 24; ++i) {
+            const uint32_t w = 4u * i;
+            m.st(w, rr[i].x); m.st(w + 1u, rr[i].y); m.st(w + 2u, rr[i].z); m.st(w + 3u, rr[i].w);
+        }
+        const v4u32 *const hd = rr + 24;
+        r.rounds = hd[6].x;
+        auto hw = [&](uint32_t k) -> uint32_t {
+            const v4u32 &v = hd[k >> 2];
+            return (k & 3u) == 0u ? v.x : (k & 3u) == 1u ? v.y : (k & 3u) == 2u ? v.z : v.w;
+        };
+#pragma unroll
+        for (uint32_t nd = 0; nd < (uint32_t)NP; ++nd) {
+            const uint32_t rh = hw(nd), c = rh >> 8, ctl = m.ld(S_CT + nd);
+            s_set_ni(r, nd, hw(8u + nd));
+            for (uint32_t j = 0; j < c; ++j)
+                ser_enqueue<S_QN>(m, r, nd, sp[SSUSP_HDR + nd * SR + j]);
+            s_byte_add(r.cnt0, r.cnt1, nd, c);
+            r.nz |= (c ? 1u : 0u) << nd;
+            r.msgs += hw(16u + nd) - c;
+            r.iss |= ((ctl & (SC_WAIT | SC_DUMPED)) == 0u ? 1u : 0u) << nd;
+            r.dmp |= ((ctl & SC_DUMPED) ? 1u : 0u) << nd;
+        }
+        if (hd[6].y & 0x100u) {
+            tn = hd[6].y & 0xFFu;
+            const uint32_t ip0 = m.ld(S_CT + tn) >> SC_IP, j0 = ip0 & 7u;
+            const uint32_t rw[4] = {hd[7].x, hd[7].y, hd[7].z, hd[7].w};
+            uint32_t al[4] = {0u, 0u, 0u, 0u};
+#pragma unroll
+            for (uint32_t k = 0; k < 8u; ++k) {
+                uint32_t hv = 0u;
+#pragma unroll
+                for (uint32_t q = 0; q < 8u; ++q)
+                    hv = (k >= j0 && k - j0 == q) ? ((rw[q >> 1] >> (16u * (q & 1u))) & 0xFFFFu) : hv;
+                al[k >> 1] |= hv << (16u * (k & 1u));
+            }
+            cur = make_uint4(al[0], al[1], al[2], al[3]);
+            nx = make_uint4(hd[8].x, hd[8].y, hd[8].z, hd[8].w);
+            tci = ip0 >> 3;
+            nxv = true;
+            pfc = tci + 2u;
+            pfv = pfc * 8u < stride;
+            if (pfv) pf = ld16(slot_of(tn) + pfc * 8u);
+        }
+        }
+        r.E = r.nz;
+        r.A = r.nz | r.iss;
+        ser_cache_clear(cc);
+        if (SOLO && serfmt && tn != 0xFFu) {
+            cc.ct = m.ld(S_CT + tn); cc.la = m.ld(S_LA + tn); cc.lv = m.ld(S_LV + tn);
+            cc.node = tn;
+        }
+        if (r.A == 0u) {
+            r.st = (r.dmp == NPM) ? SS_COMPLETED : SS_DEADLOCKED;
+            return SR_DONE;
+        }
+        return SR_RUN;
+    };
+    auto store_rec = [&](uint32_t nd, uint32_t flags, uint32_t which) {
+        if (REC_PROBE) return;
+        GV4 *dst = (GV4 *)(recs + (sys * NP + nd) * 8 + 4u * which);
+#pragma unroll
+        for (int q = 0; q < 4; ++q) {
+            v4u32 x;
+            x.x = ser_rec_word(m, nd, flags, 4 * q);
+            x.y = ser_rec_word(m, nd, flags, 4 * q + 1);
+            x.z = ser_rec_word(m, nd, flags, 4 * q + 2);
+            x.w = ser_rec_word(m, nd, flags, 4 * q + 3);
+            dst[q] = x;
+        }
+    };
+    auto fetch = [&](uint32_t nd, uint32_t ip, bool iss) -> uint32_t {
+        const uint32_t c = ip >> 3;
+        const bool tnd = tn == nd;
+        const bool rot = iss & tnd & (tci + 1u == c) & nxv;
+        const bool miss = iss & !rot & (!tnd | (tci != c));
+        cur.x = rot ? nx.x : cur.x; cur.y = rot ? nx.y : cur.y;
+        cur.z = rot ? nx.z : cur.z; cur.w = rot ? nx.w : cur.w;
+        nxv = nxv & !rot;
+        tci = rot ? c : tci;
+        if (__ballot(miss)) {
+            if (SER_PROBE && lane == 0) atomicAdd(&s_cnt[3], 1ull);
+            if (miss) {
+                const uint16_t *sl = slot_of(nd);
+                cur = ld16(sl + 8u * c);
+                nxv = (c + 1u) * 8u < stride;
+                nx = ld16(sl + (nxv ? 8u * (c + 1u) : 8u * c));
+                pfv = false;
+                tn = nd;
+                tci = c;
+            }
+            wait_vmcnt0();
+        }
+        const uint32_t j = ip & 7u;
+        const uint32_t m2 = 0u - ((j >> 1) & 1u), m4 = 0u - ((j >> 2) & 1u);
+        const uint32_t lo = (cur.x & ~m2) | (cur.y & m2), hi = (cur.z & ~m2) | (cur.w & m2);
+        const uint32_t wd = (lo & ~m4) | (hi & m4);
+        return (wd >> (16u * (j & 1u))) & 0xFFFFu;
+    };
+    auto fetch_reg = [&](uint32_t nd, uint32_t ip, uint32_t &ins) -> bool {
+        const uint32_t c = ip >> 3;
+        const bool tnd = tn == nd;
+        const bool rot = tnd & (tci + 1u == c) & nxv;
+        const bool have = tnd & ((tci == c) | rot);
+        cur.x = rot ? nx.x : cur.x; cur.y = rot ? nx.y : cur.y;
+        cur.z = rot ? nx.z : cur.z; cur.w = rot ? nx.w : cur.w;
+        nxv = nxv & !rot;
+        tci = rot ? c : tci;
+        const uint32_t j = ip & 7u;
+        const uint32_t m2 = 0u - ((j >> 1) & 1u), m4 = 0u - ((j >> 2) & 1u);
+        const uint32_t lo = (cur.x & ~m2) | (cur.y & m2), hi = (cur.z & ~m2) | (cur.w & m2);
+        const uint32_t wd = (lo & ~m4) | (hi & m4);
+        ins = (wd >> (16u * (j & 1u))) & 0xFFFFu;
+        return have;
+    };
+    bool live = false;
+    uint32_t v = SR_RUN;
+    auto refill = [&]() {
+        if (pfv && !nxv && pfc == tci + 1u) {
+            nx = pf;
+            nxv = true;
+            pfv = false;
+        }
+        if (pfv && (pfc <= tci || pfc > tci + 2u)) pfv = false;
+        const uint32_t want = nxv ? tci + 2u : tci + 1u;
+        if (tn != 0xFFu && !pfv && want * 8u < stride && v == SR_RUN) {
+            pf = ld16(slot_of(tn) + want * 8u);
+            pfc = want;
+            pfv = true;
+        }
+    };
+    auto on_dump = [&](uint32_t nd) { store_rec(nd, 2u, 0u); };
+    auto finish = [&](uint32_t v) {
+        if (v == SR_OVF) {
+            const uint32_t pos = gatomic_add((GU32 *)ovf_count, 1u);
+            ((GU32 *)ovf_list)[pos] = (uint32_t)sys;
+            atomicAdd(&s_cnt[K_OVFRERUN], 1ull);
+            return;
+        }
+        uint32_t ins = 0;
+#pragma unroll
+        for (uint32_t nd = 0; nd < (uint32_t)NP; ++nd) {
+            ins += m.ld(S_CT + nd) >> SC_IP;
+            store_rec(nd, ser_final_flags(m, nd), 1u);
+        }
+        v4u32 res;
+        res.x = r.st | (r.dmp << 8); res.y = r.rounds; res.z = r.msgs; res.w = ins;
+        ((GV4 *)results)[2 * sys] = res;
+        atomicAdd(&s_cnt[K_MSGS], (unsigned long long)r.msgs);
+        atomicAdd(&s_cnt[K_INSTRS], (unsigned long long)ins);
+        atomicAdd(&s_cnt[K_ROUNDS], (unsigned long long)r.rounds);
+        atomicAdd(&s_cnt[K_SYSTEMS], 1ull);
+        atomicAdd(&s_cnt[K_STATUS + r.st], 1ull);
+        atomicMax(&s_cnt[K_MAXR], (unsigned long long)r.rounds);
+    };
+
+    {
+        const uint32_t k = claim_next();
+        live = k < n;
+        if (live) sys = sel(k);
+        if (live && serfmt) load_rec(sys);
+    }
+    v = live ? start() : SR_RUN;
+    uint32_t iters = 0, nmac = 0;
+    uint32_t tclaim = 0, now_it = 0;
+    bool lone0 = false;
+    [[maybe_unused]] uint64_t pr_long = 0, pr_last = 0, pr_n4k = 0, pr_nl_it = 0, pr_it = 0, pr_nl_n = 0;
+    if constexpr (SIM_TAILPROBE == 2) lone0 = live && serfmt && (rr[30].y & 0x100u);
+    uint32_t hwait = 0;
+    uint64_t pb_runs = 0, pb_steps = 0, pb_idle = 0, pb_cyc = 0;
+    for (;;) {
+        bool taken = false, rest = false;
+#pragma unroll 1
+        for (int k = 0; k < SER_RF; ++k) {
+            bool ran_now = false, gen = true;
+            if (SOLO) {
+                if (k == 0) {
+                    uint64_t ts0 = 0;
+                    if (SER_PROBE >= 2) ts0 = __builtin_amdgcn_s_memtime();
+                    const bool run = live && v == SR_RUN;
+                    const bool ql = run && ser_quiet_lone(r, lim_rsh);
+                    const uint32_t sn = ql ? dsms::s_ctz(r.A) : 0xFEu;
+                    const uint32_t c = cc.ct >> (SC_IP + 3u);
+                    const bool hotq = ql & (cc.node == sn) & (tn == sn);
+                    const bool rot = hotq & (tci + 1u == c) & nxv;
+                    cur.x = rot ? nx.x : cur.x; cur.y = rot ? nx.y : cur.y;
+                    cur.z = rot ? nx.z : cur.z; cur.w = rot ? nx.w : cur.w;
+                    nxv = nxv & !rot;
+                    tci = rot ? c : tci;
+                    const bool elig = hotq & (tci == c);
+                    const uint32_t ne = (uint32_t)__builtin_popcountll(__ballot(elig));
+                    const uint32_t nr = (uint32_t)__builtin_popcountll(__ballot(run));
+                    if (ne != 0u && ne * 64u >= nr * (uint32_t)SER_SOLO_MIN) {
+                        uint32_t ns = 0;
+                        if (elig) ns = ser_solo<NP>(m, r, cc, cur.x, cur.y, cur.z, cur.w, lim_rsh);
+                        nmac += ns;
+                        taken = ran_now = true;
+                        rest = elig & (ns != 0u) & (((cc.ct >> SC_IP) & 7u) == 0u);
+                        iters += 1u;
+                        if (SER_PROBE) {
+                            uint32_t t = ns;
+                            for (int o = 1; o < 64; o <<= 1) t += __shfl_xor(t, o, 64);
+                            pb_runs += 1u; pb_steps += t; pb_idle += 8u * nr - t;
+                            if (SER_PROBE >= 2) pb_cyc += __builtin_amdgcn_s_memtime() - ts0;
+                        }
+                    }
+                }
+                if (taken) {
+                    gen = __ballot(live && v == SR_RUN && !rest) != 0ull;
+                    if (!gen && !ran_now) break;
+                }
+                iters += gen ? 1u : 0u;
+            }
+            bool mac = false;
+            uint64_t tp0 = 0, tp1 = 0, tp2 = 0;
+            if (SER_PROBE >= 2) tp0 = __builtin_amdgcn_s_memtime();
+            if (!CAP && gen) {
+#pragma unroll
+                for (int j = 0; j < SER_MACRO; ++j) {
+                    const bool q = live && v == SR_RUN && !rest && ser_quiet_lone(r, lim_rsh) && (j == 0 || mac);
+                    bool did = false;
+                    bool nohave = false;
+                    if (SER_PROBE && q) {
+                        const uint32_t n0 = dsms::s_ctz(r.A), ip0 = m.ld(S_CT + n0) >> SC_IP, c0 = ip0 >> 3;
+                        nohave = !((tn == n0) & ((tci == c0) | ((tci + 1u == c0) & nxv)));
+                    }
+                    if (SER_PROBE >= 4) {
+                        uint64_t ts[5] = {0, 0, 0, 0, 0};
+                        auto stamp = [&](int i) { __builtin_amdgcn_s_waitcnt(0); ts[i + 1] = __builtin_amdgcn_s_memtime(); };
+                        __builtin_amdgcn_s_waitcnt(0);
+                        ts[0] = __builtin_amdgcn_s_memtime();
+                        if (__ballot(q) && q) did = ser_macro<NP>(m, r, cc, fetch_reg, on_dump, stamp);
+                        const uint64_t okb = __ballot(did);
+                        if (okb && lane == (uint32_t)__builtin_ctzll(okb)) {
+                            atomicAdd(&s_cnt[13], ts[1] - ts[0]);
+                            atomicAdd(&s_cnt[14], ts[2] - ts[1]);
+                            atomicAdd(&s_cnt[15], ts[3] - ts[2]);
+                            atomicAdd(&s_cnt[16], ts[4] - ts[3]);
+                        }
+                    } else if (__ballot(q) && q) {
+                        did = ser_macro<NP>(m, r, cc, fetch_reg, on_dump, [](int) {});
+                    }
+                    if (SER_PROBE && j == 0) {
+                        const uint64_t nh = __ballot(nohave);
+                        if (lane == 0) atomicAdd(&s_cnt[8 + 3], 0ull + __builtin_popcountll(nh));
+                    }
+                    if (SER_PROBE && j == 0) {
+                        const bool nq_ = live && v == SR_RUN && !q;
+                        const uint64_t nq = __ballot(nq_), qn = __ballot(q && !did);
+                        const uint64_t mi = __ballot(nq_ && (r.iss & (r.iss - 1u)) != 0u);
+                        if (lane == 0) {
+                            atomicAdd(&s_cnt[9], (unsigned long long)__builtin_popcountll(nq));
+                            atomicAdd(&s_cnt[10], (unsigned long long)__builtin_popcountll(qn));
+                            (void)mi;
+                        }
+                    }
+                    mac = mac || did;
+                    nmac += did ? 1u : 0u;
+                }
+                if (mac && r.A == 0u) v = SR_DONE;
+                if (SOLO) rest = rest | (taken & mac);
+            }
+            if (SER_PROBE) {
+                const uint64_t gm = __ballot(live && v == SR_RUN && !mac), mm = __ballot(mac);
+                const uint64_t lv = __ballot(live);
+                if (lane == 0) {
+                    atomicAdd(&s_cnt[8], (unsigned long long)__builtin_popcountll(lv));
+                    if (__builtin_popcountll(lv) < 32) atomicAdd(&s_cnt[12], 1ull);
+                    atomicAdd(&s_cnt[0], 1ull);
+                    if (mm) atomicAdd(&s_cnt[1], 1ull);
+                    if (gm) atomicAdd(&s_cnt[2], 1ull);
+                }
+            }
+            if (SER_PROBE >= 2) tp1 = __builtin_amdgcn_s_memtime();
+            if (live && v == SR_RUN && !mac && gen && !rest) {
+                v = ser_step<NP, S_QN, CAP>(m, r, T, fetch, on_dump, lim_rsh, cap);
+                ser_cache_clear(cc);
+            }
+            if (SER_PROBE >= 2) tp2 = __builtin_amdgcn_s_memtime();
+            if (SER_PROBE) {
+                const uint64_t hm = __ballot(live && v != SR_RUN);
+                if (lane == 0 && hm) atomicAdd(&s_cnt[4], 1ull);
+            }
+            bool hgo = false;
+            const uint64_t fin = __ballot(live && v != SR_RUN);
+            if (fin) {
+                hgo = (uint32_t)__builtin_popcountll(fin) >= (uint32_t)SER_HB ||
+                      hwait >= (uint32_t)SER_HT || fin == __ballot(live);
+                hwait = hgo ? 0u : hwait + (gen ? 1u : 0u) + (ran_now ? (uint32_t)SER_SOLO_HW : 0u);
+            }
+            if (hgo && live && v != SR_RUN) {
+                if constexpr (SIM_TAILPROBE == 2) now_it = iters + (uint32_t)k;
+                uint64_t th0 = 0, th1 = 0, th2 = 0;
+                if (SER_PROBE >= 3) th0 = __builtin_amdgcn_s_memtime();
+                wait_vmcnt0();
+                const uint32_t k = claim_next();
+                const bool nl = k < n;
+                const uint32_t ns = nl ? sel(k) : 0u;
+                if (nl && serfmt) load_rec(ns);
+                if (SER_PROBE >= 3) { __builtin_amdgcn_s_waitcnt(0); th1 = __builtin_amdgcn_s_memtime(); }
+                if constexpr (SIM_TAILPROBE == 2) {
+                    const uint64_t dur = now_it > tclaim ? (uint64_t)(now_it - tclaim) : 0u;
+                    const uint64_t a = (dur << 32) | (uint64_t)sys;
+                    const uint64_t b = ((uint64_t)now_it << 32) | ((uint64_t)lone0 << 31) | dur;
+                    pr_long = a > pr_long ? a : pr_long;
+                    pr_last = b > pr_last ? b : pr_last;
+                    pr_n4k += dur > 4000u ? 1u : 0u;
+                    pr_nl_it += lone0 ? 0u : dur;
+                    pr_it += dur;
+                    pr_nl_n += lone0 ? 0u : 1u;
+                    tclaim = now_it;
+                    lone0 = nl && serfmt && (rr[30].y & 0x100u);
+                }
+                finish(v);
+                if (SER_PROBE >= 3) { __builtin_amdgcn_s_waitcnt(0); th2 = __builtin_amdgcn_s_memtime(); }
+                live = nl;
+                sys = ns;
+                rest = false;
+                v = live ? start() : SR_RUN;
+                if (SER_PROBE >= 3) {
+                    __builtin_amdgcn_s_waitcnt(0);
+                    const uint64_t th3 = __builtin_amdgcn_s_memtime();
+                    const uint64_t fl = __ballot(true);
+                    if (lane == (uint32_t)__builtin_ctzll(fl)) {
+                        atomicAdd(&s_cnt[13], th1 - th0);
+                        atomicAdd(&s_cnt[14], th2 - th1);
+                        atomicAdd(&s_cnt[15], th3 - th2);
+                    }
+                }
+            }
+            if (SER_PROBE >= 2 && lane == 0) {
+                const uint64_t tp3 = __builtin_amdgcn_s_memtime();
+                atomicAdd(&s_cnt[5], tp1 - tp0);
+                atomicAdd(&s_cnt[6], tp2 - tp1);
+                atomicAdd(&s_cnt[7], tp3 - tp2);
+            }
+            if (!gen) break;
+        }
+        uint64_t tr0 = 0;
+        if (SER_PROBE >= 2) tr0 = __builtin_amdgcn_s_memtime();
+        refill();
+        (void)tr0;
+        if (!SOLO) iters += SER_RF;
+        if (__ballot(live) == 0) break;
+    }
+    [[maybe_unused]] bool pr_wave_nl = false;
+#if SIM_TAILPROBE == 2
+    {
+        uint64_t v6[6] = {pr_long, pr_last, pr_n4k, pr_nl_it, pr_it, pr_nl_n};
+#pragma unroll
+        for (int q = 0; q < 6; ++q) {
+            uint64_t x = v6[q];
+            for (int o = 1; o < 64; o <<= 1) {
+                const uint32_t lo = __shfl_xor((uint32_t)x, o, 64), hi = __shfl_xor((uint32_t)(x >> 32), o, 64);
+                const uint64_t y = ((uint64_t)hi << 32) | lo;
+                x = q < 2 ? (y > x ? y : x) : x + y;
+            }
+            if (q == 5) pr_wave_nl = x != 0;
+            if (lane == 0) {
+                if (q < 2) atomicMax(&Ap->counters[q], (unsigned long long)x);
+                else atomicAdd(&Ap->counters[q], (unsigned long long)x);
+            }
+        }
+    }
+#endif
+    if (lane == 0) {
+        atomicAdd(&s_cnt[K_WROUNDS], (unsigned long long)iters);
+        atomicAdd(&Ap->counters[K_SERIT], (unsigned long long)iters);
+        if (SER_PROBE && SOLO && !SIM_TAILPROBE) {
+            atomicAdd(&Ap->counters[K_SERPROBE], (unsigned long long)pb_runs);
+            atomicAdd(&Ap->counters[K_SERPROBE + 1], (unsigned long long)pb_steps);
+            atomicAdd(&Ap->counters[K_SERPROBE + 2], (unsigned long long)pb_idle);
+            atomicAdd(&Ap->counters[K_SERPROBE + 3], (unsigned long long)pb_cyc);
+        }
+#if SIM_TAILPROBE
+        const uint64_t ticks = __builtin_amdgcn_s_memrealtime() - tprobe0, ms = ticks / 100000u;
+        atomicAdd(&Ap->counters[K_SERPROBE + (ms < 11u ? 0u : (ms - 10u < 5u ? ms - 10u : 5u))], 1ull);
+        if constexpr (SIM_TAILPROBE == 2) {
+            atomicMax(&Ap->counters[pr_wave_nl ? 6 : 7], (unsigned long long)ticks);
+            if (pr_wave_nl) atomicAdd(&Ap->counters[8], 1ull);
+            if (ms >= 2u && ms < 6u) atomicAdd(&Ap->counters[7u + ms], 1ull);
+        }
+#endif
+    }
+    if (!CAP) {
+        uint32_t t = nmac;
+        for (int o = 1; o < 64; o <<= 1) t += __shfl_xor(t, o, 64);
+        if (lane == 0 && t) atomicAdd(&Ap->counters[K_SERMAC], (unsigned long long)t);
+    }
+    __syncthreads();
+    if (threadIdx.x < K_N) {
+        const unsigned long long x = s_cnt[threadIdx.x];
+        if (x) {
+            if (threadIdx.x == K_MAXR) atomicMax(&Ap->counters[K_MAXR], x);
+            else atomicAdd(&Ap->counters[threadIdx.x], x);
+        }
+    }
diff --git a/hp-assignment-2_amd/pydsm.py b/hp-assignment-2_amd/pydsm.py
--- a/hp-assignment-2_amd/pydsm.py
+++ b/hp-assignment-2_amd/pydsm.py
@@ -200,6 +200,7 @@
             "dsm_debug_exscan_device": (i32, [vp, vp, u64, vp, vp]),
             "dsm_debug_order_state": (i32, [vp, vp, vp, vp, u64, u64, vp, u32, ctypes.POINTER(u32),
                                             ctypes.POINTER(i32)]),
+            "dsm_debug_ser_claims": (i32, [vp, vp]),
         }
         for name, (res, args) in sig.items():
             if os.environ.get("DSM_LIB") and not hasattr(L, name):
@@ -1368,6 +1369,11 @@
             d["order_short"] = order[:ns][::-1].copy()
         return d
 
+    def ser_claims(self):
+        out = np.zeros(4, dtype=np.uint32)
+        _check(lib().dsm_debug_ser_claims(self.ctx, _ptr(out)), "dsm_debug_ser_claims")
+        return dict(zip(("took", "plain", "rest", "multi"), (int(x) for x in out)))
+
     def launch_info(self):
         li = LaunchInfo()
         _check(lib().dsm_launch_info_get(self.ctx, ctypes.byref(li)), "dsm_launch_info_get")
```

After: 116.6 billion (median of 6 runs). +10.3%, better.
